# SelennLamson/AntsRL

Measured on AMD Instinct MI355X. Metric: ant-steps/sec (ants x envs x steps/s), 256^2 grid, higher is better.
Workload: dtype f64 ant kinematics / f32 grids

## Files before the change

### antsrl_amd/_lib.py

```python
from __future__ import annotations

import ctypes as C
import os

from .config import AntsCfg, AntsGen, AntsInit

LIB_PATH = os.environ.get("ANTSRL_LIB") or os.path.join(os.path.dirname(os.path.abspath(__file__)), "lib",
                                                        "libantsrl_hip.so")

EXPORTS = ("antsrl_abi_version", "antsrl_cfg_size", "antsrl_last_error", "antsrl_workspace_bytes", "antsrl_create",
           "antsrl_workspace_map",
           "antsrl_destroy", "antsrl_reset", "antsrl_generate", "antsrl_step", "antsrl_observe", "antsrl_update", "antsrl_flush",
           "antsrl_step_update", "antsrl_set_timing_events", "antsrl_set_activation", "antsrl_policy_mlp", "antsrl_read_state", "antsrl_state_bytes",
           "antsrl_set_obs_format", "antsrl_query", "antsrl_bench_copy", "antsrl_set_inloop_policy", "antsrl_set_obs_row_stride", "antsrl_set_perceive_path", "antsrl_mem_alloc", "antsrl_mem_free",
           "antsrl_mem_trim", "antsrl_mem_stats", "antsrl_update_phase",
           "antsrl_perceptive_field", "antsrl_memnet_packed_bytes", "antsrl_memnet_pack", "antsrl_policy_memory",
           "antsrl_memtrain_sizes", "antsrl_memtrain_init", "antsrl_memtrain_unpack", "antsrl_memtrain_copy",
           "antsrl_memtrain_grad", "antsrl_memtrain_apply", "antsrl_memnet_packed_bytes_ex", "antsrl_memnet_pack_ex",
           "antsrl_policy_memory_ex", "antsrl_agent_select", "antsrl_replay_record_pre", "antsrl_replay_record_post",
           "antsrl_policy_memory_tiles", "antsrl_agent_plan", "antsrl_agent_select_actions",
           "antsrl_replay_record_pre_plain", "antsrl_replay_record_post_plain", "antsrl_lintrain_sizes",
           "antsrl_lintrain_grad", "antsrl_lintrain_apply", "antsrl_lintrain_step", "antsrl_exptrain_sizes",
           "antsrl_exptrain_grad", "antsrl_exptrain_apply", "antsrl_exptrain_step", "antsrl_rework_collapsed_bytes",
           "antsrl_rework_collapse", "antsrl_policy_rework", "antsrl_reworktrain_sizes", "antsrl_reworktrain_grad",
           "antsrl_reworktrain_apply", "antsrl_reworktrain_step", "antsrl_policy_rework_select", "antsrl_monitor_sizes",
           "antsrl_monitor_init", "antsrl_monitor_step", "antsrl_monitor_end_episode", "antsrl_recorder_sizes",
           "antsrl_recorder_begin", "antsrl_recorder_frame", "antsrl_render_sizes", "antsrl_render_frames")

_lib = None


class AntsMemNetShape(C.Structure):
    _fields_ = [(n, C.c_int32) for n in ("n_features", "agent_dim", "mem_size", "h1", "h2", "h3", "n_rot", "n_ph")]


class AntsReworkShape(C.Structure):
    _fields_ = [(n, C.c_int32) for n in ("n_features", "agent_dim", "g1", "g2", "g3", "r1", "r2", "r3", "p1", "n_rot", "n_ph")]


class AntsRecordSpec(C.Structure):
    _fields_ = [(n, C.c_int32) for n in ("n_envs", "n_ants", "env_id_base", "n_features", "agent_dim", "mem_size", "n_rot",
                                         "obs_format", "obs_pitch", "reserved")] + [
        (n, C.c_int64) for n in ("K", "head", "max_len")] + [(n, C.c_uint64) for n in ("seed", "step")]


class AntsRenderOpts(C.Structure):
    _fields_ = [(n, C.c_int32) for n in ("zoom", "view_mask", "ant_radius", "layer_only")] + [
        ("phero_max_val", C.c_double), ("phero_colors", (C.c_uint8 * 3) * 4)]


class AntsWsArray(C.Structure):
    _fields_ = [("name", C.c_char * 24), ("block", C.c_int32), ("_pad", C.c_int32), ("offset", C.c_uint64), ("bytes", C.c_uint64)]


class AntsrlError(RuntimeError):
    pass


def load() -> C.CDLL:
    global _lib
    if _lib is not None:
        return _lib
    if not os.path.exists(LIB_PATH):
        raise AntsrlError(
            "libantsrl_hip.so is missing (%s): build it with `python -m antsrl_amd.build` "
            "(hipcc, gfx950).  There is no CPU fallback." % LIB_PATH)
    import torch
    lib = C.CDLL(LIB_PATH)
    vp, i32 = C.c_void_p, C.c_int
    lib.antsrl_abi_version.restype = i32
    lib.antsrl_last_error.restype = C.c_char_p
    lib.antsrl_workspace_bytes.argtypes = [C.POINTER(AntsCfg), C.POINTER(C.c_size_t)]
    lib.antsrl_create.argtypes = [C.POINTER(AntsCfg), vp, C.c_size_t, C.POINTER(vp)]
    lib.antsrl_workspace_bytes2.argtypes = [C.POINTER(AntsCfg), C.POINTER(C.c_size_t), C.POINTER(C.c_size_t)]
    lib.antsrl_create2.argtypes = [C.POINTER(AntsCfg), vp, C.c_size_t, vp, C.c_size_t, C.POINTER(vp)]
    lib.antsrl_workspace_map.argtypes = [C.POINTER(AntsCfg), i32, C.POINTER(AntsWsArray), C.c_int32, C.POINTER(C.c_int32)]
    lib.antsrl_destroy.argtypes = [vp]
    lib.antsrl_destroy.restype = None
    lib.antsrl_reset.argtypes = [vp, C.POINTER(AntsInit), vp]
    lib.antsrl_generate.argtypes = [vp, C.POINTER(AntsGen), C.c_uint64, vp]
    lib.antsrl_step.argtypes = [vp, vp, vp, vp, vp, vp, vp, vp]
    lib.antsrl_observe.argtypes = [vp, vp, vp, vp, vp]
    lib.antsrl_update.argtypes = [vp, vp, vp]
    lib.antsrl_flush.argtypes = [vp, vp]
    lib.antsrl_update_phase.argtypes = [vp, i32, vp, vp]
    lib.antsrl_perceptive_field.argtypes = [vp, vp, vp]
    lib.antsrl_step_update.argtypes = [vp, vp, vp, vp, vp, vp, vp, vp, vp]
    lib.antsrl_set_timing_events.argtypes = [vp, C.POINTER(vp)]
    lib.antsrl_set_activation.argtypes = [vp, vp, C.c_double, vp]
    lib.antsrl_policy_mlp.argtypes = [vp, vp, vp, C.c_int64, C.c_int32, vp, vp, vp, vp, vp, vp, vp, vp, vp, vp]
    lib.antsrl_read_state.argtypes = [vp, i32, vp, vp]
    lib.antsrl_state_bytes.argtypes = [vp, i32, C.POINTER(C.c_size_t)]
    lib.antsrl_query.argtypes = [vp, i32, C.POINTER(C.c_longlong)]
    lib.antsrl_set_inloop_policy.argtypes = [vp, i32] + [vp] * 9
    lib.antsrl_bench_copy.argtypes = [vp, vp, C.c_size_t, vp]
    lib.antsrl_set_obs_row_stride.argtypes = [vp, i32]
    lib.antsrl_set_perceive_path.argtypes = [vp, i32]
    lib.antsrl_mem_alloc.argtypes = [C.c_size_t, i32, C.POINTER(vp)]
    lib.antsrl_mem_free.argtypes = [vp]
    lib.antsrl_mem_trim.argtypes = []
    lib.antsrl_mem_stats.argtypes = [C.POINTER(C.c_size_t)] * 4
    lib.antsrl_memnet_packed_bytes.argtypes = [C.POINTER(AntsMemNetShape), C.POINTER(C.c_size_t)]
    lib.antsrl_memnet_pack.argtypes = [C.POINTER(AntsMemNetShape), C.POINTER(vp), vp, vp]
    lib.antsrl_policy_memory.argtypes = [C.POINTER(AntsMemNetShape), vp, vp, i32, vp, vp, C.c_int64, vp, vp, vp, vp, vp]
    lib.antsrl_memnet_packed_bytes_ex.argtypes = [C.POINTER(AntsMemNetShape), i32, C.POINTER(C.c_size_t)]
    lib.antsrl_memnet_pack_ex.argtypes = [C.POINTER(AntsMemNetShape), i32, C.POINTER(vp), vp, vp]
    lib.antsrl_policy_memory_ex.argtypes = [C.POINTER(AntsMemNetShape), i32, vp, vp, i32, vp, vp, C.c_int64, vp, vp, vp,
                                            vp, vp]
    lib.antsrl_policy_memory_tiles.argtypes = [C.POINTER(AntsMemNetShape), i32, vp, vp, i32, vp, vp, C.c_int64, vp, vp, vp,
                                               vp, vp, vp, vp]
    sz = C.POINTER(C.c_size_t)
    lib.antsrl_memtrain_sizes.argtypes = [C.POINTER(AntsMemNetShape), C.c_int64, sz, sz, sz, sz]
    lib.antsrl_memtrain_init.argtypes = [C.POINTER(AntsMemNetShape), C.POINTER(vp), vp, vp]
    lib.antsrl_memtrain_unpack.argtypes = [C.POINTER(AntsMemNetShape), vp, C.POINTER(vp), vp]
    lib.antsrl_memtrain_copy.argtypes = [C.POINTER(AntsMemNetShape), vp, vp, vp]
    lib.antsrl_memtrain_grad.argtypes = [C.POINTER(AntsMemNetShape), vp, vp, vp, vp, vp, vp, vp, vp, vp, vp, C.c_int64,
                                         C.c_float, vp, vp, vp, vp]
    lib.antsrl_memtrain_apply.argtypes = [C.POINTER(AntsMemNetShape), vp, vp, C.c_int64, C.c_double, C.c_double,
                                          C.c_double, C.c_double, vp]
    lib.antsrl_agent_select.argtypes = [C.c_uint64, C.c_uint64, i32, i32, i32, C.c_double, i32, i32, i32, vp, vp, vp, vp,
                                        vp, vp]
    lib.antsrl_agent_plan.argtypes = [C.c_uint64, C.c_uint64, i32, i32, i32, C.c_double, vp, vp, vp]
    lib.antsrl_replay_record_pre.argtypes = [C.POINTER(AntsRecordSpec)] + [vp] * 9
    lib.antsrl_replay_record_post.argtypes = [C.POINTER(AntsRecordSpec)] + [vp] * 10
    lib.antsrl_agent_select_actions.argtypes = [C.c_uint64, C.c_uint64, i32, i32, i32, C.c_double, i32, i32, vp, vp, vp, vp]
    lib.antsrl_replay_record_pre_plain.argtypes = [C.POINTER(AntsRecordSpec)] + [vp] * 8
    lib.antsrl_replay_record_post_plain.argtypes = [C.POINTER(AntsRecordSpec)] + [vp] * 9
    lib.antsrl_lintrain_sizes.argtypes = [i32, C.c_int64, sz, sz, C.POINTER(C.c_int32)]
    lib.antsrl_lintrain_grad.argtypes = [i32] + [vp] * 11 + [C.c_int64, vp, C.c_int64, C.c_float, vp, vp, vp, vp]
    lib.antsrl_lintrain_apply.argtypes = [vp, vp, vp, vp, C.c_int64, C.c_double, C.c_double, C.c_double, C.c_double, vp]
    lib.antsrl_lintrain_step.argtypes = [i32] + [vp] * 13 + [C.c_int64, vp, C.c_int64, C.c_float, C.c_int64, C.c_double,
                                                             C.c_double, C.c_double, C.c_double, vp, vp, vp, vp]
    lib.antsrl_exptrain_sizes.argtypes = [i32, C.c_int64, sz, sz, C.POINTER(C.c_int32)]
    lib.antsrl_exptrain_grad.argtypes = [i32] + [vp] * 9 + [C.c_int64, vp, C.c_int64, C.c_float, vp, vp, vp, vp]
    lib.antsrl_exptrain_apply.argtypes = [i32, vp, vp, vp, vp, C.c_int64, C.c_double, C.c_double, C.c_double, C.c_double, vp]
    lib.antsrl_exptrain_step.argtypes = [i32] + [vp] * 11 + [C.c_int64, vp, C.c_int64, C.c_float, C.c_int64, C.c_double,
                                                             C.c_double, C.c_double, C.c_double, vp, vp, vp, vp]
    lib.antsrl_rework_collapsed_bytes.argtypes = [C.POINTER(AntsReworkShape), sz]
    lib.antsrl_rework_collapse.argtypes = [C.POINTER(AntsReworkShape), C.POINTER(vp), vp, vp]
    lib.antsrl_policy_rework.argtypes = [C.POINTER(AntsReworkShape), vp, vp, i32, vp, C.c_int64, vp, vp, vp, vp]
    rs = C.POINTER(AntsReworkShape)
    lib.antsrl_policy_rework_select.argtypes = [rs, vp, vp, i32, vp, C.c_uint64, C.c_uint64, i32, i32, i32, C.c_double, vp, vp,
                                                vp, vp, vp]
    lib.antsrl_reworktrain_sizes.argtypes = [rs, C.c_int64, sz, sz, C.POINTER(C.c_int32)]
    lib.antsrl_reworktrain_grad.argtypes = [rs] + [vp] * 9 + [C.c_int64, vp, C.c_int64, C.c_float, vp, vp, vp, vp]
    lib.antsrl_reworktrain_apply.argtypes = [rs, vp, vp, vp, vp, C.c_int64, C.c_double, C.c_double, C.c_double, C.c_double, vp]
    lib.antsrl_reworktrain_step.argtypes = [rs] + [vp] * 11 + [C.c_int64, vp, C.c_int64, C.c_float, C.c_int64, C.c_double,
                                                               C.c_double, C.c_double, C.c_double, vp, vp, vp, vp]
    lib.antsrl_monitor_sizes.argtypes = [i32, i32, i32, i32, sz]
    lib.antsrl_monitor_init.argtypes = [vp, i32, i32, i32, i32, vp]
    lib.antsrl_monitor_step.argtypes = [vp, i32, i32, i32, i32, vp, vp, C.c_double, i32, i32, vp]
    lib.antsrl_monitor_end_episode.argtypes = [vp, i32, i32, i32, i32, i32, i32, vp]
    lib.antsrl_recorder_sizes.argtypes = [vp, i32, i32, i32, sz, sz, sz]
    lib.antsrl_recorder_begin.argtypes = [vp, vp, C.POINTER(C.c_int32), i32, i32, i32, vp]
    lib.antsrl_recorder_frame.argtypes = [vp, vp, C.POINTER(C.c_int32), i32, i32, i32, i32, vp]
    lib.antsrl_render_sizes.argtypes = [vp, i32, C.POINTER(AntsRenderOpts), sz, sz]
    lib.antsrl_render_frames.argtypes = [vp, vp, i32, i32, i32, i32, i32, C.POINTER(AntsRenderOpts), vp, vp, vp]
    for name in EXPORTS:
        getattr(lib, name)
    lib.antsrl_cfg_size.restype = C.c_size_t
    from .config import ABI_VERSION
    if lib.antsrl_abi_version() != ABI_VERSION:
        raise AntsrlError("ABI version mismatch: library %d, binding %d" % (lib.antsrl_abi_version(), ABI_VERSION))
    if lib.antsrl_cfg_size() != C.sizeof(AntsCfg):
        raise AntsrlError("AntsCfg layout mismatch: library %d bytes, binding %d" % (
            lib.antsrl_cfg_size(), C.sizeof(AntsCfg)))
    _lib = lib
    return lib


def hip_runtime() -> C.CDLL:
    load()
    for line in open("/proc/self/maps"):
        path = line.split()[-1]
        if "libamdhip64" in path:
            return C.CDLL(path)
    raise AntsrlError("no libamdhip64 mapped in this process")


def check(rc: int, what: str = "antsrl") -> None:
    if rc != 0:
        msg = load().antsrl_last_error().decode("utf-8", "replace")
        raise AntsrlError("%s failed (%d): %s" % (what, rc, msg))


def ptr(t):
    return None if t is None else C.c_void_p(t.data_ptr())


def stream(device):
    import torch
    return C.c_void_p(torch.cuda.current_stream(device).cuda_stream)


class HipEvents:

    def __init__(self, n):
        self.hip = hip_runtime()
        self.ev = []
        for _ in range(n):
            e = C.c_void_p()
            rc = self.hip.hipEventCreate(C.byref(e))
            assert rc == 0, "hipEventCreate failed: %d" % rc
            self.ev.append(e)

    def elapsed_ms(self, a, b):
        ms = C.c_float()
        rc = self.hip.hipEventElapsedTime(C.byref(ms), self.ev[a], self.ev[b])
        assert rc == 0, "hipEventElapsedTime failed: %d" % rc
        return ms.value

    def destroy(self):
        for e in self.ev:
            self.hip.hipEventDestroy(e)
```

### antsrl_amd/batched.py

```python
from __future__ import annotations

import ctypes as C
from typing import Dict, Optional

import numpy as np
import torch

from . import _lib
from . import config as cfgmod
from . import vmm
from .config import AntsCfg, AntsInit

_STATE_DTYPES = {
    cfgmod.S_ANTS_XYT: torch.float64, cfgmod.S_PREV_XY: torch.float64, cfgmod.S_HOLDING: torch.float32,
    cfgmod.S_MANDIBLES: torch.uint8, cfgmod.S_ACTIVATION: torch.float32, cfgmod.S_PHERO: torch.float32,
    cfgmod.S_FOOD: torch.float32, cfgmod.S_EXPLORED: torch.uint8, cfgmod.S_ANTHILL_FOOD: torch.float64,
    cfgmod.S_ROCK_CENTERS: torch.float64, cfgmod.S_TIMESTEP: torch.int32, cfgmod.S_REWARD_STATE: torch.uint8,
    cfgmod.S_WALLS: torch.uint8, cfgmod.S_ANTHILL_AREA: torch.uint8, cfgmod.S_SEED: torch.float32,
    cfgmod.S_ANTHILL_XYR: torch.int32, cfgmod.S_ROCK_RW: torch.float64,
    cfgmod.S_PHERO_C0: torch.float32, cfgmod.S_PHERO_C1: torch.float32, cfgmod.S_PHERO_C2: torch.float32,
    cfgmod.S_PHERO_C3: torch.float32,
}


import contextlib

_NULL_CTX = contextlib.nullcontext()
_RAW_STREAM = getattr(torch._C, "_cuda_getCurrentRawStream", None)


def _ptr(t: Optional[torch.Tensor]):
    return None if t is None else C.c_void_p(t.data_ptr())


def placement_levels_seen(times) -> bool:
    ok = [t for t in times if t < 1.25 * min(times)]
    return max(ok) >= 1.06 * min(ok)


class BatchedAntsEnv:
    def __init__(self, cfg: AntsCfg, device: Optional[torch.device] = None, obs_dtype: torch.dtype = torch.float32,
                 obs_row_stride=None, pieced_memory: bool = True, split_workspace: bool = True):
        if obs_dtype not in (torch.float32, torch.bfloat16):
            raise ValueError("obs_dtype must be torch.float32 or torch.bfloat16")
        if not torch.cuda.is_available():
            raise _lib.AntsrlError("BatchedAntsEnv needs an MI355X (torch.cuda.is_available() is False); "
                                   "there is no CPU fallback")
        self.lib = _lib.load()
        self.cfg = cfg.copy()
        self.device = torch.device(device if device is not None else "cuda:%d" % torch.cuda.current_device())
        self._dev_index = self.device.index if self.device.index is not None else torch.cuda.current_device()
        need = C.c_size_t()
        _lib.check(self.lib.antsrl_workspace_bytes(C.byref(self.cfg), C.byref(need)), "workspace_bytes")
        self.workspace_bytes = need.value
        nst, nrec = C.c_size_t(), C.c_size_t()
        _lib.check(self.lib.antsrl_workspace_bytes2(C.byref(self.cfg), C.byref(nst), C.byref(nrec)), "workspace_bytes2")
        self.state_bytes, self.record_bytes = nst.value, nrec.value
        self._split = bool(split_workspace)
        if not self._split:
            self.state_bytes, self.record_bytes = 0, self.workspace_bytes
        with torch.cuda.device(self.device):
            big = (lambda n: vmm.empty_u8(n, self.device)) if pieced_memory else (lambda n: torch.empty(n, dtype=torch.uint8, device=self.device))
            self._pieced = bool(pieced_memory)
            self._h = None
            self._state = None
            self._make_handle(torch.empty(self.record_bytes + 256, dtype=torch.uint8, device=self.device))
            E, N, P, K = cfg.n_envs, cfg.n_ants, cfg.pside, cfg.n_channels
            esz = 4 if obs_dtype == torch.float32 else 2
            row = P * P * K
            if obs_row_stride not in (None, "line"):
                raise ValueError("obs_row_stride must be None or 'line'")
            pitch = row if obs_row_stride is None else (row * esz + 127) // 128 * 128 // esz
            sizes = [("agent_state", E * N * 2 * 4), ("reward", E * N * 4), ("done", E), ("obs", E * N * pitch * esz)]
            offs, total = {}, 0
            for name, nbytes in sizes:
                offs[name] = total
                total += (nbytes + 255) // 256 * 256
            self._out_sizes, self._out_offs, self._out_total, self._small_bytes = sizes, offs, total, offs["obs"]
            self._obs_dtype, self._obs_pitch_row = obs_dtype, (pitch, row)
            if obs_dtype == torch.bfloat16:
                _lib.check(self.lib.antsrl_set_obs_format(self._h, 1), "set_obs_format")
            if pitch != row:
                _lib.check(self.lib.antsrl_set_obs_row_stride(self._h, pitch), "set_obs_row_stride")
            self.obs_row_pitch = pitch
            self._bind_outputs(big(total + 256).zero_())
        self._keep = None
        self._loaded = None
        self._host_out = None
        self._host_act = None
        self._act_event = None

    def __del__(self):
        h = getattr(self, "_h", None)
        if h:
            self.lib.antsrl_destroy(h)
            self._h = None

    def _bind_outputs(self, flat: torch.Tensor) -> None:
        c = self.cfg
        E, N, P, K = c.n_envs, c.n_ants, c.pside, c.n_channels
        sizes, offs, total = self._out_sizes, self._out_offs, self._out_total
        pitch, row = self._obs_pitch_row
        base = (-flat.data_ptr()) % 256
        self._out_flat = flat[base:base + total]

        def piece(name, nbytes, dtype, shape):
            return self._out_flat[offs[name]:offs[name] + nbytes].view(dtype).view(shape)
        if pitch == row:
            self.obs = piece("obs", sizes[3][1], self._obs_dtype, (E, N, P, P, K))
            self.obs_padded = None
        else:
            self.obs_padded = piece("obs", sizes[3][1], self._obs_dtype, (E, N, pitch))
            self.obs = self.obs_padded[..., :row].unflatten(-1, (P, P, K))
        self.agent_state = piece("agent_state", sizes[0][1], torch.float32, (E, N, 2))
        self.reward = piece("reward", sizes[1][1], torch.float32, (E, N))
        self.done = piece("done", sizes[2][1], torch.uint8, (E,))
        self._host_out = None

    def _make_handle(self, ws: torch.Tensor, state: Optional[torch.Tensor] = None) -> None:
        if getattr(self, "_h", None):
            self.lib.antsrl_destroy(self._h)
            self._h = None
        if ws.numel() < self.record_bytes + (-ws.data_ptr()) % 256:
            raise _lib.AntsrlError("record block too small: %d bytes for %d" % (ws.numel(), self.record_bytes))
        self._ws_ptr = ws.data_ptr() + (-ws.data_ptr()) % 256
        self._h = C.c_void_p()
        if not self._split:
            self._ws, self._state = ws, None
            _lib.check(self.lib.antsrl_create(C.byref(self.cfg), C.c_void_p(self._ws_ptr), self.workspace_bytes, C.byref(self._h)), "create")
        else:
            if state is None:
                state = self._state if self._state is not None else torch.empty(self.state_bytes + 256, dtype=torch.uint8, device=self.device)
            if state.numel() < self.state_bytes + (-state.data_ptr()) % 256:
                raise _lib.AntsrlError("state block too small: %d bytes for %d" % (state.numel(), self.state_bytes))
            self._ws, self._state = ws, state
            self._state_ptr = state.data_ptr() + (-state.data_ptr()) % 256
            _lib.check(self.lib.antsrl_create2(C.byref(self.cfg), C.c_void_p(self._state_ptr), self.state_bytes,
                                               C.c_void_p(self._ws_ptr), self.record_bytes, C.byref(self._h)), "create2")
        if getattr(self, "_obs_dtype", torch.float32) == torch.bfloat16:
            _lib.check(self.lib.antsrl_set_obs_format(self._h, 1), "set_obs_format")
        pitch, row = getattr(self, "_obs_pitch_row", (0, 0))
        if pitch != row:
            _lib.check(self.lib.antsrl_set_obs_row_stride(self._h, pitch), "set_obs_row_stride")

    def tune_placement(self, age: int = 150, steps: int = 30, verbose: bool = False, extra_outputs: int = 4,
                       walk_spacers: int = 3, spacer_gib: float = 24.0, force_walk: bool = False, state_stage: bool = True):
        if self._out_total < vmm.SMALL_BYTES:
            return None
        if self._loaded:
            raise _lib.AntsrlError("tune_placement() must run right after construction: this handle has already been %s" % self._loaded)
        c = self.cfg
        E, N = c.n_envs, c.n_ants
        dev = self.device

        def torch_u8(n):
            return torch.empty(n, dtype=torch.uint8, device=dev)
        with torch.cuda.device(dev):
            g = torch.Generator(device=dev)
            g.manual_seed(7)
            rot = torch.randint(-1, 2, (4, E, N), generator=g, device=dev, dtype=torch.int8)
            ph = torch.randint(0, 3, (4, E, N), generator=g, device=dev, dtype=torch.int8) if c.n_phero == 2 else [None] * 4
            e0, e1 = torch.cuda.Event(enable_timing=True), torch.cuda.Event(enable_timing=True)

            def scratch_episode():
                self.generate(cfgmod.make_gen(), episode_seed=0x7A11)
                for t in range(age):
                    self.step_update(rot[t % 4], ph[t % 4], None)

            NEV, PSTEPS, PSTEPS_STATE = cfgmod.TIMING_EVENTS, 8, 24
            evs = _lib.HipEvents(NEV * PSTEPS_STATE)
            prc_times = []
            upd_times = []

            def measure(psteps=PSTEPS):
                for t in range(4):
                    self.step_update(rot[t % 4], ph[t % 4], None)
                e0.record()
                for t in range(steps):
                    self.step_update(rot[t % 4], ph[t % 4], None)
                e1.record()
                for t in range(psteps):
                    self.set_timing_events([evs.ev[NEV * t + i].value for i in range(NEV)])
                    self.step_update(rot[t % 4], ph[t % 4], None)
                torch.cuda.current_stream(dev).synchronize()
                prc_times.append(float(np.mean([evs.elapsed_ms(NEV * t + 2, NEV * t + 3) for t in range(psteps)])))
                upd_times.append(float(np.mean([evs.elapsed_ms(NEV * t + 1, NEV * t + 2) for t in range(psteps)])))
                return e0.elapsed_time(e1) / steps
            own_ws, own_out, own_state = self._ws, self._out_flat, self._state
            n_ws, n_out, n_state = self.record_bytes + 256, self._out_total + 256, self.state_bytes + 256
            pairs, times = [], []
            for ws_kind in ("own", "other"):
                if ws_kind == "other":
                    self._make_handle(vmm.empty_u8(n_ws, dev))
                scratch_episode()
                for out_kind in ("own", "other"):
                    if out_kind == "other":
                        self._bind_outputs((torch_u8(n_out) if self._pieced else vmm.empty_u8(n_out, dev)).zero_())
                    elif ws_kind == "other":
                        self._bind_outputs(own_out)
                    pairs.append((self._ws, self._out_flat))
                    times.append(measure())
            labels = ["ws torch / out %s" % ("pieced" if self._pieced else "torch"),
                      "ws torch / out %s" % ("torch" if self._pieced else "pieced"),
                      "ws pieced / out %s" % ("pieced" if self._pieced else "torch"),
                      "ws pieced / out %s" % ("torch" if self._pieced else "pieced")]
            if extra_outputs > 0 and self._pieced:
                self._make_handle(own_ws)
                scratch_episode()
                for k in range(int(extra_outputs)):
                    self._bind_outputs(vmm.empty_u8(n_out, dev).zero_())
                    pairs.append((self._ws, self._out_flat))
                    times.append(measure())
                    labels.append("ws torch / out pieced (draw %d)" % (k + 2))
            spacers = []
            walked = 0
            both_levels = placement_levels_seen
            while self._pieced and walked < int(walk_spacers) and (force_walk or not both_levels(prc_times)):
                free_b = torch.cuda.mem_get_info(dev)[0]
                want = int(min(spacer_gib * 2 ** 30, free_b / 5))
                if want < (4 << 30):
                    break
                try:
                    spacers.append(torch_u8(want))
                    spacers.append(vmm.empty_u8(want, dev))
                except (RuntimeError, _lib.AntsrlError):
                    break
                walked += 1
                depth = sum(x.numel() for x in spacers) / 2 ** 30
                if self._ws.data_ptr() != own_ws.data_ptr():
                    self._make_handle(own_ws)
                scratch_episode()
                for kind, mk in (("pieced", lambda: vmm.empty_u8(n_out, dev)), ("torch", lambda: torch_u8(n_out))):
                    self._bind_outputs(mk().zero_())
                    pairs.append((self._ws, self._out_flat))
                    times.append(measure())
                    labels.append("ws torch / out %s (walk %d: +%.0f GiB)" % (kind, walked, depth))
                self._make_handle(torch_u8(n_ws))
                scratch_episode()
                self._bind_outputs(own_out)
                pairs.append((self._ws, self._out_flat))
                times.append(measure())
                labels.append("ws torch (walk %d: +%.0f GiB) / out %s" % (walked, depth, "pieced" if self._pieced else "torch"))
            best = min(range(len(times)), key=prc_times.__getitem__)
            if verbose:
                print("tune_placement: ms/step per (workspace, outputs) pair %s -> %d" % (["%.4f" % t for t in times], best))
            ws, out = pairs[best]
            n_stage1 = len(times)
            state_cands = [("state torch (default)", own_state)]
            if state_stage and self._split:
                try:
                    state_cands.append(("state pieced", vmm.pieced_u8(n_state, dev)))
                except _lib.AntsrlError:
                    pass
                seen = {ws.data_ptr()}
                for (w2, _o), lab in zip(pairs, labels):
                    if w2.data_ptr() not in seen and w2.numel() >= n_state and len(state_cands) < 4:
                        seen.add(w2.data_ptr())
                        state_cands.append(("state in spare record block (%s)" % lab.split(" / ")[0], w2[:n_state]))
            for lab, st in state_cands if len(state_cands) > 1 else []:
                self._make_handle(ws, st)
                self._bind_outputs(out)
                scratch_episode()
                times.append(measure(PSTEPS_STATE))
            evs.destroy()
            s_upd, s_prc = upd_times[n_stage1:], prc_times[n_stage1:]
            times, prc_times, upd_times = times[:n_stage1], prc_times[:n_stage1], upd_times[:n_stage1]
            s_best = 0
            if s_upd:
                def fast(k, by):
                    return s_upd[k] <= (1.0 - by) * s_upd[0] and s_upd[k] + s_prc[k] < s_upd[0] + s_prc[0]
                own = [k for k in range(1, len(s_upd)) if state_cands[k][0] == "state pieced" and fast(k, 0.03)]
                corners = [k for k in range(1, len(s_upd)) if state_cands[k][0] != "state pieced" and fast(k, 0.05)]
                if own or corners:
                    s_best = min(own or corners, key=s_upd.__getitem__)
            state = state_cands[s_best][1]
            state_labels = [lab for lab, _ in state_cands]
            del pairs, spacers, state_cands
            if ws.data_ptr() != self._ws.data_ptr() or (state is not None and state.data_ptr() != self._state.data_ptr()):
                self._make_handle(ws, state)
            self._bind_outputs(out)
            if walked:
                vmm.trim()
            torch.cuda.empty_cache()
            self._out_flat.zero_()
            del own_ws, own_out, own_state, ws, out, state
        self.placement_trials = dict(ms_per_step=[round(t, 5) for t in times], observation_kernel_ms=[round(t, 5) for t in prc_times],
                                     chosen=best, pairs=labels, both_levels_seen=bool(both_levels(prc_times)), walk_steps=walked,
                                     state_stage=dict(candidates=state_labels, update_move_kernel_ms=[round(t, 5) for t in s_upd],
                                                      observation_kernel_ms=[round(t, 5) for t in s_prc], chosen=s_best))
        self._loaded = None
        return times

    @property
    def _obs_buf(self):
        return self.obs if self.obs_padded is None else self.obs_padded

    def _stream(self):
        if _RAW_STREAM is not None:
            return C.c_void_p(_RAW_STREAM(self._dev_index))
        return C.c_void_p(torch.cuda.current_stream(self.device).cuda_stream)

    def _on_device(self):
        return _NULL_CTX if torch.cuda.current_device() == self._dev_index else torch.cuda.device(self.device)

    def _dev(self, a, dtype, shape=None):
        if a is None:
            return None
        t = torch.as_tensor(np.ascontiguousarray(a) if isinstance(a, np.ndarray) else a)
        t = t.to(device=self.device, dtype=dtype).contiguous()
        if shape is not None:
            assert tuple(t.shape) == tuple(shape), "expected shape %s, got %s" % (shape, tuple(t.shape))
        return t

    def reset(self, init: Dict[str, object]) -> None:
        c = self.cfg
        E, N, W, H, Cn, R = c.n_envs, c.n_ants, c.w, c.h, c.n_phero, c.n_rocks
        t = dict(
            ants_xyt=self._dev(init["ants_xyt"], torch.float64, (E, N, 3)),
            seed=self._dev(init["seed"], torch.float64, (E, N)),
            walls=self._dev(init["walls"], torch.uint8, (E, W, H)),
            food=self._dev(init["food"], torch.float32, (E, W, H)),
            anthill_xyr=self._dev(init["anthill_xyr"], torch.int32, (E, 3)),
            rocks=self._dev(init.get("rocks"), torch.float64, (E, R, 4)) if R > 0 else None,
            phero=self._dev(init.get("phero"), torch.float32, (E, Cn, W, H)),
        )
        ai = AntsInit(*[None if t[k] is None else t[k].data_ptr()
                        for k in ("ants_xyt", "seed", "walls", "food", "anthill_xyr", "rocks", "phero")])
        with torch.cuda.device(self.device):
            _lib.check(self.lib.antsrl_reset(self._h, C.byref(ai), self._stream()), "reset")
        self._loaded = "reset"
        self._keep = t

    def generate(self, gen=None, episode_seed: int = 0, walls=None) -> None:
        g = gen if gen is not None else cfgmod.make_gen()
        if walls is not None:
            c = self.cfg
            self._gen_walls = self._dev(np.asarray(walls).astype(np.uint8) if not torch.is_tensor(walls) else walls,
                                        torch.uint8, (c.n_envs, c.w, c.h))
            g.walls_input = self._gen_walls.data_ptr()
        with torch.cuda.device(self.device):
            _lib.check(self.lib.antsrl_generate(self._h, C.byref(g), int(episode_seed), self._stream()), "generate")
        self._loaded = "given an episode (generate)"

    def _actions(self, rotation, phero):
        c = self.cfg
        if isinstance(rotation, np.ndarray) and isinstance(phero, np.ndarray):
            n = c.n_envs * c.n_ants
            if self._host_act is None:
                self._host_act = torch.empty((2, c.n_envs, c.n_ants), dtype=torch.int8, pin_memory=True)
                self._dev_act = torch.empty((2, c.n_envs, c.n_ants), dtype=torch.int8, device=self.device)
                self._act_event = torch.cuda.Event()
            else:
                self._act_event.synchronize()
            assert rotation.size == n and phero.size == n, "expected %d actions per array" % n
            h = self._host_act.numpy()
            h[0] = self._integral(rotation, "rotation").reshape(c.n_envs, c.n_ants)
            h[1] = self._integral(phero, "pheromone").reshape(c.n_envs, c.n_ants)
            with torch.cuda.device(self.device):
                self._dev_act.copy_(self._host_act, non_blocking=True)
                self._act_event.record()
            return self._dev_act[0], self._dev_act[1]
        rot = self._dev(self._integral(rotation, "rotation"), torch.int8, (c.n_envs, c.n_ants))
        ph = self._dev(self._integral(phero, "pheromone"), torch.int8, (c.n_envs, c.n_ants))
        return rot, ph

    validate_actions = True

    def _integral(self, a, what):
        if a is None:
            return None
        if torch.is_tensor(a):
            if a.dtype == torch.int8 or a.numel() == 0:
                return a
            if self.validate_actions:
                fl = a.is_floating_point()
                frac = (a != a.round()).any() if fl else torch.zeros((), dtype=torch.bool, device=a.device)
                lo, hi, bad = torch.stack([a.min().to(torch.float64), a.max().to(torch.float64), frac.to(torch.float64)]).tolist()
                if bad:
                    raise ValueError("%s actions must be whole numbers (the kernels take them as int8)" % what)
                if lo < -128 or hi > 127:
                    raise ValueError("%s actions out of the int8 range" % what)
            return a.to(torch.int8) if a.is_floating_point() else a
        arr = np.asarray(a)
        if arr.dtype.kind == "f":
            if not np.array_equal(arr, np.rint(arr)):
                raise ValueError("%s actions must be whole numbers (the kernels take them as int8)" % what)
            arr = arr.astype(np.int64)
        if arr.size and (arr.min() < -128 or arr.max() > 127):
            raise ValueError("%s actions out of the int8 range" % what)
        return arr

    def outputs_to_host(self, want_obs: bool = True):
        if self.obs.dtype != torch.float32 and want_obs:
            raise _lib.AntsrlError("outputs_to_host: bfloat16 observations have no numpy dtype; use the device tensors")
        base, o = self._out_flat.data_ptr(), self._out_offs
        if any(t.data_ptr() != base + o[k] for k, t in (("obs", self._obs_buf), ("agent_state", self.agent_state),
                                                         ("reward", self.reward), ("done", self.done))):
            return (self.obs.cpu().numpy() if want_obs else None, self.agent_state.cpu().numpy(),
                    self.reward.cpu().numpy(), self.done.cpu().numpy())
        if self._host_out is None:
            self._host_out = torch.empty((self._out_flat.numel(),), dtype=torch.uint8, pin_memory=True)
        n = self._out_flat.numel() if want_obs else self._small_bytes
        with torch.cuda.device(self.device):
            self._host_out[:n].copy_(self._out_flat[:n], non_blocking=True)
            torch.cuda.current_stream(self.device).synchronize()
        hb, o = self._host_out.numpy(), self._out_offs

        def piece(name, t):
            nb = t.numel() * t.element_size()
            return hb[o[name]:o[name] + nb].view(np.float32 if t.dtype == torch.float32 else np.uint8).reshape(tuple(t.shape)).copy()
        obs_h = None
        if want_obs:
            obs_h = piece("obs", self._obs_buf)
            if self.obs_padded is not None:
                c = self.cfg
                obs_h = np.ascontiguousarray(obs_h[..., :c.pside * c.pside * c.n_channels]).reshape(tuple(self.obs.shape))
        return (obs_h, piece("agent_state", self.agent_state),
                piece("reward", self.reward), piece("done", self.done))

    def step(self, rotation, phero, want_obs: bool = True):
        rot, ph = self._actions(rotation, phero)
        with self._on_device():
            _lib.check(self.lib.antsrl_step(self._h, _ptr(rot), _ptr(ph), _ptr(self._obs_buf if want_obs else None),
                                            _ptr(self.agent_state), _ptr(self.reward), _ptr(self.done),
                                            self._stream()), "step")
        return self.obs, self.agent_state, self.reward, self.done

    def observe(self, want_obs: bool = True):
        with self._on_device():
            _lib.check(self.lib.antsrl_observe(self._h, _ptr(self._obs_buf if want_obs else None),
                                               _ptr(self.agent_state), _ptr(self.reward), self._stream()),
                       "observe")
        return self.obs, self.agent_state, self.reward

    def update(self, wall_jitter=None) -> None:
        c = self.cfg
        j = self._dev(wall_jitter, torch.float64, (c.n_envs, c.n_ants))
        with self._on_device():
            _lib.check(self.lib.antsrl_update(self._h, _ptr(j), self._stream()), "update")

    def update_phase(self, phase: int, wall_jitter=None) -> None:
        c = self.cfg
        j = self._dev(wall_jitter, torch.float64, (c.n_envs, c.n_ants)) if phase == cfgmod.PHASE_WALLS else None
        with self._on_device():
            _lib.check(self.lib.antsrl_update_phase(self._h, int(phase), _ptr(j), self._stream()), "update_phase")

    def flush(self) -> None:
        with self._on_device():
            _lib.check(self.lib.antsrl_flush(self._h, self._stream()), "flush")

    def step_update(self, rotation, phero, wall_jitter=None, want_obs: bool = True):
        c = self.cfg
        rot, ph = self._actions(rotation, phero)
        j = self._dev(wall_jitter, torch.float64, (c.n_envs, c.n_ants))
        with self._on_device():
            _lib.check(self.lib.antsrl_step_update(self._h, _ptr(rot), _ptr(ph), _ptr(j),
                                                   _ptr(self._obs_buf if want_obs else None), _ptr(self.agent_state),
                                                   _ptr(self.reward), _ptr(self.done), self._stream()),
                       "step_update")
        return self.obs, self.agent_state, self.reward, self.done

    def set_timing_events(self, events) -> None:
        if events is None:
            _lib.check(self.lib.antsrl_set_timing_events(self._h, None), "set_timing_events")
        else:
            n = cfgmod.TIMING_EVENTS
            assert len(events) == n, "antsrl_set_timing_events takes %d events" % n
            arr = (C.c_void_p * n)(*[C.c_void_p(int(e)) for e in events])
            _lib.check(self.lib.antsrl_set_timing_events(self._h, arr), "set_timing_events")

    def query(self, what: int) -> int:
        v = C.c_longlong()
        _lib.check(self.lib.antsrl_query(self._h, int(what), C.byref(v)), "query")
        return int(v.value)

    def set_perceive_path(self, path: int) -> None:
        _lib.check(self.lib.antsrl_set_perceive_path(self._h, int(path)), "set_perceive_path")

    def set_activation(self, act, new_deposit_strength: float = 0.0) -> None:
        c = self.cfg
        a = self._dev(act, torch.float32, (c.n_envs, c.n_ants, c.n_phero))
        with torch.cuda.device(self.device):
            _lib.check(self.lib.antsrl_set_activation(self._h, _ptr(a), float(new_deposit_strength),
                                                      self._stream()), "set_activation")
        self._loaded = "given an activation matrix"

    def perceptive_field(self) -> torch.Tensor:
        c = self.cfg
        out = torch.empty((c.n_envs, c.w, c.h), dtype=torch.uint8, device=self.device)
        with self._on_device():
            _lib.check(self.lib.antsrl_perceptive_field(self._h, _ptr(out), self._stream()), "perceptive_field")
        return out.to(torch.bool)

    def read_state(self, which: int) -> torch.Tensor:
        c = self.cfg
        E, N, W, H, Cn, R = c.n_envs, c.n_ants, c.w, c.h, c.n_phero, c.n_rocks
        shapes = {
            cfgmod.S_ANTS_XYT: (E, N, 3), cfgmod.S_PREV_XY: (E, N, 2), cfgmod.S_HOLDING: (E, N),
            cfgmod.S_MANDIBLES: (E, N), cfgmod.S_ACTIVATION: (E, N, Cn), cfgmod.S_PHERO: (E, Cn, W, H),
            cfgmod.S_FOOD: (E, W, H), cfgmod.S_EXPLORED: (E, W, H), cfgmod.S_ANTHILL_FOOD: (E,),
            cfgmod.S_ROCK_CENTERS: (E, R, 2), cfgmod.S_TIMESTEP: (E,), cfgmod.S_REWARD_STATE: (E, N),
            cfgmod.S_WALLS: (E, W, H), cfgmod.S_ANTHILL_AREA: (E, W, H), cfgmod.S_SEED: (E, N),
            cfgmod.S_ANTHILL_XYR: (E, 3), cfgmod.S_ROCK_RW: (E, R, 2),
            cfgmod.S_PHERO_C0: (E, W, H), cfgmod.S_PHERO_C1: (E, W, H), cfgmod.S_PHERO_C2: (E, W, H),
            cfgmod.S_PHERO_C3: (E, W, H),
        }
        if cfgmod.S_PHERO_C0 <= which <= cfgmod.S_PHERO_C3 and which - cfgmod.S_PHERO_C0 >= Cn:
            raise _lib.AntsrlError("pheromone channel %d of %d" % (which - cfgmod.S_PHERO_C0, Cn))
        out = torch.empty(shapes[which], dtype=_STATE_DTYPES[which], device=self.device)
        if out.numel():
            with torch.cuda.device(self.device):
                _lib.check(self.lib.antsrl_read_state(self._h, which, _ptr(out), self._stream()), "read_state")
        return out
```

### antsrl_amd/config.py

```python
from __future__ import annotations

import ctypes as C
import math
from typing import Optional, Sequence

import numpy as np

ABI_VERSION = 5
MAX_CHANNELS = 16
MAX_PSIDE = 15
MAX_PCELLS = MAX_PSIDE * MAX_PSIDE
MAX_FILTER_RADIUS = 3
MAX_FILTER_TAPS = 49
MAX_PHERO = 4

CH_ANTS, CH_PHERO, CH_ANTHILL, CH_WALLS, CH_FOOD, CH_ROCKS = range(6)
REWARD_NONE, REWARD_EXPLORATION, REWARD_FOOD, REWARD_ALL = range(4)
PHERO_AUTO, PHERO_EXPLICIT_SWEEP = 0, 1
ACT_AUTO, ACT_CELL_META, ACT_SINGLE_KERNEL = 0, 1, 2
TIMING_EVENTS = 5
Q_CELL_META, Q_SCALED_UNITS, Q_INTERLEAVED, Q_FILTER_SEPARABLE, Q_PERCEIVE_RUN, Q_TIMESTEP, Q_DEFERRED_UPDATE, Q_PERCEIVE_FAST = range(8)
PERCEIVE_AUTO, PERCEIVE_GENERIC = 0, 1

(S_ANTS_XYT, S_PREV_XY, S_HOLDING, S_MANDIBLES, S_ACTIVATION, S_PHERO, S_FOOD, S_EXPLORED,
 S_ANTHILL_FOOD, S_ROCK_CENTERS, S_TIMESTEP, S_REWARD_STATE, S_WALLS, S_ANTHILL_AREA,
 S_SEED, S_ANTHILL_XYR, S_ROCK_RW, S_PHERO_C0, S_PHERO_C1, S_PHERO_C2, S_PHERO_C3) = range(21)


class AntsCfg(C.Structure):
    _fields_ = [
        ("abi_version", C.c_int32),
        ("n_envs", C.c_int32),
        ("n_ants", C.c_int32),
        ("w", C.c_int32),
        ("h", C.c_int32),
        ("n_phero", C.c_int32),
        ("n_rocks", C.c_int32),
        ("max_time", C.c_int32),
        ("perception_radius", C.c_int32),
        ("n_channels", C.c_int32),
        ("channel_kind", C.c_int32 * MAX_CHANNELS),
        ("channel_arg", C.c_int32 * MAX_CHANNELS),
        ("has_mask", C.c_int32),
        ("mask", C.c_uint8 * MAX_PCELLS),
        ("_pad0", C.c_uint8 * 7),
        ("delta", C.c_double),
        ("fwd_delta", C.c_double),
        ("max_speed", C.c_double),
        ("max_rot_speed", C.c_double),
        ("carry_speed_reduction", C.c_double),
        ("backward_speed_reduction", C.c_double),
        ("max_hold", C.c_double),
        ("has_max_val", C.c_int32),
        ("filter_radius", C.c_int32),
        ("phero_max_val", C.c_double),
        ("deposit_strength", C.c_double),
        ("phero_threshold", C.c_double),
        ("filter", C.c_double * MAX_FILTER_TAPS),
        ("reward_kind", C.c_int32),
        ("phero_mode", C.c_int32),
        ("reward_threshold", C.c_double),
        ("fct_explore", C.c_double),
        ("fct_food", C.c_double),
        ("fct_anthill", C.c_double),
        ("fct_explore_holding", C.c_double),
        ("fct_headinganthill", C.c_double),
        ("rng_seed", C.c_uint64),
        ("act_path", C.c_int32),
        ("env_id_base", C.c_int32),
        ("n_envs_total", C.c_int32),
        ("_pad1", C.c_int32),
    ]

    @property
    def pside(self) -> int:
        return 2 * self.perception_radius + 1

    def copy(self) -> "AntsCfg":
        out = AntsCfg()
        C.memmove(C.byref(out), C.byref(self), C.sizeof(AntsCfg))
        return out

    def obs_shape(self):
        p = self.pside
        return (self.n_envs, self.n_ants, p, p, self.n_channels)


class AntsGen(C.Structure):
    _fields_ = [("wall_density", C.c_double), ("n_food_discs", C.c_int32), ("food_rmin", C.c_int32),
                ("food_rmax", C.c_int32), ("auto_reset", C.c_int32), ("wall_kind", C.c_int32),
                ("perlin_octaves", C.c_int32), ("perlin_scale", C.c_double), ("perlin_persistence", C.c_double),
                ("perlin_lacunarity", C.c_double), ("rng_kind", C.c_int32), ("_pad", C.c_int32),
                ("walls_input", C.c_void_p)]


WALLS_BERNOULLI, WALLS_PERLIN, WALLS_INPUT = 0, 1, 2
PHASE_WALLS, PHASE_ROCKS_PHEROMONE, PHASE_ANTS, PHASE_ANTHILL = 0, 1, 2, 3
RNG_COUNTER, RNG_REFERENCE = 0, 1


def make_gen(wall_density=0.05, n_food_discs=20, food_rmin=5, food_rmax=10, auto_reset=False, walls="bernoulli",
             perlin_scale=22.0, perlin_octaves=2, perlin_persistence=0.5, perlin_lacunarity=2.0, rng="counter",
             walls_input_ptr=None) -> AntsGen:
    kind = {"bernoulli": WALLS_BERNOULLI, "perlin": WALLS_PERLIN, "input": WALLS_INPUT}[walls]
    return AntsGen(wall_density, n_food_discs, food_rmin, food_rmax, 1 if auto_reset else 0, kind,
                   int(perlin_octaves), float(perlin_scale), float(perlin_persistence), float(perlin_lacunarity),
                   {"counter": RNG_COUNTER, "reference": RNG_REFERENCE}[rng], 0, walls_input_ptr)


class AntsInit(C.Structure):
    _fields_ = [
        ("ants_xyt", C.c_void_p),
        ("seed", C.c_void_p),
        ("walls", C.c_void_p),
        ("food", C.c_void_p),
        ("anthill_xyr", C.c_void_p),
        ("rocks", C.c_void_p),
        ("phero", C.c_void_p),
    ]


DEFAULT_MASK = np.array([[0, 0, 1, 1, 1, 0, 0],
                         [0, 1, 1, 1, 1, 1, 0],
                         [1, 1, 1, 1, 1, 1, 1],
                         [1, 1, 1, 1, 1, 1, 1],
                         [1, 1, 1, 1, 1, 1, 1],
                         [0, 1, 1, 1, 1, 1, 0],
                         [0, 0, 1, 1, 1, 0, 0]], dtype=np.uint8)


def diffuse_filter(diffuse_factor: float = 0.0, evap_factor: float = 0.001) -> np.ndarray:
    f = np.ones((3, 3)) * diffuse_factor
    f[1, 1] = 1 - 8 * diffuse_factor
    f *= 1 - evap_factor
    return f


def default_channels(n_phero: int, n_rocks: int):
    kinds = [CH_ANTS] + [CH_PHERO] * n_phero + [CH_ANTHILL, CH_WALLS, CH_FOOD]
    args = [0] + list(range(n_phero)) + [0, 0, 0]
    if n_rocks > 0:
        kinds.append(CH_ROCKS)
        args.append(0)
    return kinds, args


def make_cfg(n_envs: int, n_ants: int, w: int, h: int, *, n_phero: int = 2, n_rocks: int = 0,
             max_time: int = 2000, mask: Optional[np.ndarray] = DEFAULT_MASK,
             perception_radius: Optional[int] = None, fwd_delta: float = 4.0, delta: float = 1.1,
             channels: Optional[Sequence] = None,
             max_speed: float = 1.0, max_rot_speed: float = 40 / 180 * np.pi,
             carry_speed_reduction: float = 0.05, backward_speed_reduction: float = 0.5,
             max_hold: float = 5.0, phero_max_val: Optional[float] = 255.0,
             deposit_strength: float = 1.0, phero_threshold: float = 0.01,
             filt: Optional[np.ndarray] = None, reward_kind: int = REWARD_EXPLORATION,
             reward_threshold: float = 1.0, fct_explore: float = 1.0, fct_food: float = 1.0,
             fct_anthill: float = 5.0, fct_explore_holding: float = 0.0,
             fct_headinganthill: float = 1.0, rng_seed: int = 0x5EED,
             phero_mode: int = PHERO_AUTO, act_path: int = ACT_AUTO, env_id_base: int = 0,
             n_envs_total: int = 0) -> AntsCfg:
    c = AntsCfg()
    c.abi_version = ABI_VERSION
    c.n_envs, c.n_ants, c.w, c.h = n_envs, n_ants, w, h
    c.n_phero, c.n_rocks, c.max_time = n_phero, n_rocks, max_time
    if mask is not None:
        mask = np.asarray(mask)
        assert mask.ndim == 2 and mask.shape[0] == mask.shape[1] and mask.shape[0] % 2 == 1
        r = mask.shape[0] // 2 if perception_radius is None else perception_radius
        assert mask.shape[0] == 2 * r + 1
        c.has_mask = 1
        flat = mask.astype(np.uint8).reshape(-1)
        for i, v in enumerate(flat):
            c.mask[i] = int(v)
    else:
        r = 3 if perception_radius is None else perception_radius
        c.has_mask = 0
    assert 2 * r + 1 <= MAX_PSIDE
    c.perception_radius = r
    if channels is None:
        kinds, args = default_channels(n_phero, n_rocks)
    else:
        kinds = [k if isinstance(k, int) else k[0] for k in channels]
        args = [0 if isinstance(k, int) else k[1] for k in channels]
    assert len(kinds) <= MAX_CHANNELS
    c.n_channels = len(kinds)
    for i, (k, a) in enumerate(zip(kinds, args)):
        c.channel_kind[i] = k
        c.channel_arg[i] = a
    c.delta, c.fwd_delta = delta, fwd_delta
    c.max_speed, c.max_rot_speed = max_speed, max_rot_speed
    c.carry_speed_reduction, c.backward_speed_reduction = carry_speed_reduction, backward_speed_reduction
    c.max_hold = max_hold
    c.has_max_val = 0 if phero_max_val is None else 1
    c.phero_max_val = 0.0 if phero_max_val is None else phero_max_val
    c.deposit_strength = deposit_strength
    c.phero_threshold = phero_threshold
    if filt is None:
        filt = diffuse_filter()
    filt = np.asarray(filt, dtype=np.float64)
    assert filt.ndim == 2 and filt.shape[0] == filt.shape[1] and filt.shape[0] % 2 == 1
    fr = filt.shape[0] // 2
    off = filt.copy()
    off[fr, fr] = 0.0
    if not off.any():
        filt = filt[fr:fr + 1, fr:fr + 1]
        fr = 0
    assert fr <= MAX_FILTER_RADIUS
    c.filter_radius = fr
    for i, v in enumerate(filt.reshape(-1)):
        c.filter[i] = float(v)
    c.reward_kind = reward_kind
    c.reward_threshold = reward_threshold
    c.fct_explore, c.fct_food, c.fct_anthill = fct_explore, fct_food, fct_anthill
    c.fct_explore_holding, c.fct_headinganthill = fct_explore_holding, fct_headinganthill
    c.rng_seed = rng_seed
    c.phero_mode = phero_mode
    c.act_path = act_path
    c.env_id_base = env_id_base
    c.n_envs_total = n_envs_total
    return c


def mask_array(cfg: AntsCfg) -> Optional[np.ndarray]:
    if not cfg.has_mask:
        return None
    p = cfg.pside
    return np.array(list(cfg.mask[: p * p]), dtype=bool).reshape(p, p)


__all__ = [n for n in dir() if n.isupper() or n in (
    "AntsCfg", "AntsInit", "AntsGen", "make_gen", "make_cfg", "diffuse_filter", "default_channels", "mask_array")]
_ = math


def uses_scaled_units(cfg: AntsCfg) -> bool:
    return (cfg.phero_mode == PHERO_AUTO and cfg.filter_radius == 0 and 0.5 < cfg.filter[0] <= 1.0
            and cfg.phero_threshold >= 0.0)
```

### antsrl_amd/csrc/antsrl_capi.hip

```cpp
#include <hip/hip_runtime.h>
#include <stdarg.h>
#include <stdio.h>
#include <math.h>
#include <stdlib.h>
#include <string.h>
#include <new>

#include "antsrl_device.h"
#include "antsrl_fail.h"
#include "antsrl_recorder.h"
#include "antsrl_render.h"

hipError_t antsrl_launch_act(const KP &p, const int8_t *rot, const int8_t *ph, int cur, float *obs,
                             float *agent_state, float *reward, uint8_t *done, int flags, hipStream_t st);
bool antsrl_act_fits(const KP &p);
bool antsrl_act_needs_hbm_maps(const KP &p);
hipError_t antsrl_launch_sweep(const KP &p, int cur, hipStream_t st);
hipError_t antsrl_launch_update(const KP &p, const double *jitter, int out_buf, hipStream_t st, int phases = 15);
hipError_t antsrl_launch_collect_full(const KP &p, hipStream_t st);
hipError_t antsrl_launch_reset(const KP &p, const AntsInit *in, hipStream_t st);
hipError_t antsrl_launch_set_activation(const KP &p, const float *act, hipStream_t st);
hipError_t antsrl_launch_read_state(const KP &p, int which, int cur, void *dst, hipStream_t st);
hipError_t antsrl_launch_perceptive_field(const KP &p, uint8_t *dst, hipStream_t st);
hipError_t antsrl_launch_generate(const KP &p, const AntsGen &g, uint64_t seed, hipStream_t st);
hipError_t antsrl_launch_phero_wall_clear(const KP &p, hipStream_t st, int buf = 0);
hipError_t antsrl_launch_phero_renorm(const KP &p, hipStream_t st);
bool antsrl_meta_supported(const KP &p);
hipError_t antsrl_launch_move(const KP &p, const int8_t *rot, const int8_t *ph, uint8_t *done, int do_step, uint32_t seq,
                              hipStream_t st);
hipError_t antsrl_launch_perceive(const KP &p, int cur, float *obs, float *agent_state, float *reward, int flags,
                                  uint32_t seq, hipStream_t st, const PolArgs *pol, uint32_t obs_pitch, bool generic);
bool antsrl_perceive_fast(const KP &p);
bool antsrl_inloop_policy_supported(const KP &p);
hipError_t antsrl_launch_policy_pack(unsigned char *pack, const float *w1, const float *b1, const float *w2, const float *b2,
                                     const float *w3, const float *b3, int F, hipStream_t st);
hipError_t antsrl_launch_meta_rebase(const KP &p, hipStream_t st);
bool antsrl_update_move_supported(const KP &p);
hipError_t antsrl_launch_update_move(const KP &p, int out_buf, double g_dep, double inv_g_dep, const int8_t *rot,
                                     const int8_t *ph, uint8_t *done, uint32_t seq, hipStream_t st, bool with_frames);
int antsrl_perceive_run(const KP &p);
hipError_t antsrl_launch_copy16(void *dst, const void *src, size_t bytes, hipStream_t st);

struct AntsHandle {
    AntsCfg cfg;
    KP p;
    int cur;
    int steps_since_update;
    bool need_full_collect;
    bool is_reset;
    bool episode_over;
    size_t ws_bytes[2];
    AntsGen gen;
    bool has_gen;
    uint64_t episode_seed;
    int host_timestep;
    long long sweeps;
    bool obs_bf16;
    uint32_t obs_pitch;
    bool prc_generic;
    bool need_wall_clear;
    hipEvent_t ev[ANTSRL_TIMING_EVENTS];
    bool ev_armed;
    uint32_t obs_seq;
    PolArgs pol;
    bool pend_update;
    KP pend_p;
    int pend_out_buf;
    int phase_next;
};

static thread_local char g_err[512] = "";

int fail(int code, const char *fmt, ...)
{
    va_list ap;
    va_start(ap, fmt);
    vsnprintf(g_err, sizeof(g_err), fmt, ap);
    va_end(ap);
    return code;
}

int hip_fail(hipError_t e, const char *what)
{
    return fail(ANTSRL_E_DEVICE, "%s: %s", what, hipGetErrorString(e));
}

extern "C" int antsrl_abi_version(void) { return ANTSRL_ABI_VERSION; }
extern "C" size_t antsrl_cfg_size(void) { return sizeof(AntsCfg); }
extern "C" const char *antsrl_last_error(void) { return g_err; }

static void fill_kp(const AntsCfg *c, KP *p);

static int validate(const AntsCfg *c)
{
    if (!c) return fail(ANTSRL_E_INVALID, "cfg is NULL");
    if (c->abi_version != ANTSRL_ABI_VERSION)
        return fail(ANTSRL_E_INVALID, "AntsCfg.abi_version %d != library %d", c->abi_version, ANTSRL_ABI_VERSION);
    if (c->n_envs < 1 || c->n_ants < 1 || c->w < 1 || c->h < 1)
        return fail(ANTSRL_E_INVALID, "n_envs, n_ants, w, h must be >= 1");
    if ((long long)c->w * c->h > (1ll << 30)) return fail(ANTSRL_E_INVALID, "grid too large");
    if (c->n_envs > 65535)
        return fail(ANTSRL_E_INVALID, "n_envs must be <= 65535 per handle (shard larger batches over handles / GPUs)");
    if (c->n_phero < 1 || c->n_phero > ANTSRL_MAX_PHERO)
        return fail(ANTSRL_E_INVALID, "n_phero must be in 1..%d", ANTSRL_MAX_PHERO);
    if (c->n_rocks < 0 || c->n_rocks > 32) return fail(ANTSRL_E_INVALID, "n_rocks must be in 0..32");
    if (c->perception_radius < 0 || 2 * c->perception_radius + 1 > ANTSRL_MAX_PSIDE)
        return fail(ANTSRL_E_INVALID, "perception side must be <= %d", ANTSRL_MAX_PSIDE);
    if (c->n_channels < 1 || c->n_channels > ANTSRL_MAX_CHANNELS)
        return fail(ANTSRL_E_INVALID, "n_channels must be in 1..%d", ANTSRL_MAX_CHANNELS);
    for (int k = 0; k < c->n_channels; ++k) {
        const int kind = c->channel_kind[k];
        if (kind < ANTSRL_CH_ANTS || kind > ANTSRL_CH_ROCKS) return fail(ANTSRL_E_INVALID, "bad channel kind");
        if (kind == ANTSRL_CH_PHERO && (c->channel_arg[k] < 0 || c->channel_arg[k] >= c->n_phero))
            return fail(ANTSRL_E_INVALID, "pheromone channel index out of range");
        if (kind == ANTSRL_CH_PHERO && !c->has_max_val)
            return fail(ANTSRL_E_INVALID, "a perceived pheromone needs max_val (RL_api.py:125 divides by it)");
        if (kind == ANTSRL_CH_ROCKS && c->n_rocks == 0)
            return fail(ANTSRL_E_INVALID, "rocks perceived but n_rocks == 0");
    }
    if (c->filter_radius < 0 || c->filter_radius > ANTSRL_MAX_FILTER_RADIUS)
        return fail(ANTSRL_E_INVALID, "filter_radius must be in 0..%d", ANTSRL_MAX_FILTER_RADIUS);
    if (c->reward_kind < ANTSRL_REWARD_NONE || c->reward_kind > ANTSRL_REWARD_ALL)
        return fail(ANTSRL_E_INVALID, "bad reward_kind");
    if (c->has_max_val && !(c->phero_max_val > 0)) return fail(ANTSRL_E_INVALID, "phero_max_val must be > 0");
    if (c->act_path < ANTSRL_ACT_AUTO || c->act_path > ANTSRL_ACT_SINGLE_KERNEL) return fail(ANTSRL_E_INVALID, "bad act_path");
    if (c->env_id_base < 0 || (long long)c->env_id_base + c->n_envs > 0x7fffffffll)
        return fail(ANTSRL_E_INVALID, "env_id_base must be >= 0 and env_id_base + n_envs must fit 31 bits");
    if (c->n_envs_total != 0 && (long long)c->n_envs_total < (long long)c->env_id_base + c->n_envs)
        return fail(ANTSRL_E_INVALID, "n_envs_total %d < env_id_base + n_envs = %lld (0 = that sum)", c->n_envs_total,
                    (long long)c->env_id_base + c->n_envs);
    if (c->act_path == ANTSRL_ACT_CELL_META) {
        KP kp;
        fill_kp(c, &kp);
        if (!kp.meta)
            return fail(ANTSRL_E_UNSUPPORTED, "ANTSRL_ACT_CELL_META needs 2 pheromone channels, the generator's channel order "
                                              "([Ants, Phero0, Phero1, Anthill, Walls, Food(, Rocks)]), a perception of 128..368 values "
                                              "per ant over at most 64 cells, and at most 4096 ants per env");
    }
    return ANTSRL_OK;
}

static bool use_scaled(const AntsCfg *c)
{
    return c->phero_mode == ANTSRL_PHERO_AUTO && c->filter_radius == 0 && c->filter[0] > 0.5 &&
           c->filter[0] <= 1.0 && c->phero_threshold >= 0.0;
}

static bool use_interleaved(const AntsCfg *c)
{
    return use_scaled(c) && c->n_phero == 2;
}

static void carve(const AntsCfg *c, DState *s, unsigned char *base, unsigned char *rec_base, bool split, size_t bytes[2],
                  AntsWsArray *map = nullptr, int32_t cap = 0, int32_t *count = nullptr)
{
    const size_t E = c->n_envs, N = c->n_ants, G = (size_t)c->w * c->h, Cn = c->n_phero, R = c->n_rocks;
    const size_t words = (G + 31) / 32;
    size_t off[2] = {0, 0};
    int32_t n_arrays = 0;
    auto take_from = [&](int block, const char *name, size_t nbytes) -> unsigned char * {
        unsigned char *b = block ? rec_base : base;
        size_t &o = off[split ? block : 0];
        unsigned char *ptr = b ? b + o : nullptr;
        if (map && n_arrays < cap) {
            AntsWsArray &a = map[n_arrays];
            memset(&a, 0, sizeof(a));
            strncpy(a.name, name, sizeof(a.name) - 1);
            a.block = split ? block : 0; a.offset = o; a.bytes = nbytes;
        }
        ++n_arrays;
        o = (o + nbytes + 255) / 256 * 256;
        return ptr;
    };
    auto take = [&](const char *name, size_t nbytes) { return take_from(0, name, nbytes); };
    auto take_rec = [&](const char *name, size_t nbytes) { return take_from(1, name, nbytes); };
    KP kp;
    fill_kp(c, &kp);
    DState d;
    d.x = (double *)take("x", 8 * E * N); d.y = (double *)take("y", 8 * E * N); d.theta = (double *)take("theta", 8 * E * N);
    d.prev_x = (double *)take("prev_x", 8 * E * N); d.prev_y = (double *)take("prev_y", 8 * E * N);
    d.prev_dist = (double *)take("prev_dist", 8 * E * N);
    d.holding = (float *)take("holding", 4 * E * N); d.seed = (float *)take("seed", 4 * E * N);
    d.prev_holding = (float *)take("prev_holding", 4 * E * N);
    d.activation = (float *)take("activation", 4 * E * N * Cn);
    d.mandibles = (uint8_t *)take("mandibles", E * N); d.reward_state = (uint8_t *)take("reward_state", E * N);
    d.dirty_cell = (int32_t *)take("dirty_cell", 4 * E * N);
    d.walldep_cell = (int32_t *)take("walldep_cell", 4 * E * N);
    if (use_interleaved(c)) {
        d.phero[0] = d.phero[1] = (float *)take_rec("records", 16 * E * G);
        d.food = d.phero[0] ? d.phero[0] + 2 : nullptr;
    } else {
        d.phero[0] = (float *)take_rec("phero0", 4 * E * G * Cn);
        d.phero[1] = use_scaled(c) ? d.phero[0] : (float *)take_rec("phero1", 4 * E * G * Cn);
        d.food = (float *)take_rec("food", 4 * E * G * (size_t)kp.fs);
    }
    d.walls_bits = (uint32_t *)take("walls_bits", 4 * E * words); d.area_bits = (uint32_t *)take("area_bits", 4 * E * words);
    d.explored_bits = (uint32_t *)take("explored_bits", 4 * E * words);
    d.big_pres = d.big_old = nullptr;
    if (!kp.meta && antsrl_act_needs_hbm_maps(kp)) {
        d.big_pres = (uint32_t *)take("big_pres", 4 * E * words);
        d.big_old = (uint32_t *)take("big_old", 4 * E * words);
    }
    d.primed_cur = kp.meta ? (uint8_t *)take("primed_cur", E) : nullptr;
    d.frames = kp.meta ? (AntFrame *)take("frames", sizeof(AntFrame) * E * N) : nullptr;
    d.anthill_xyr = (int32_t *)take("anthill_xyr", 4 * E * 3);
    d.anthill_food = (double *)take("anthill_food", 8 * E);
    d.rock_cx = (double *)take("rock_cx", 8 * E * (R ? R : 1)); d.rock_cy = (double *)take("rock_cy", 8 * E * (R ? R : 1));
    d.rock_r = (double *)take("rock_r", 8 * E * (R ? R : 1)); d.rock_w = (double *)take("rock_w", 8 * E * (R ? R : 1));
    d.timestep = (int32_t *)take("timestep", 4 * E);
    d.reward_primed = (uint8_t *)take("reward_primed", E);
    d.gen_discs = (int32_t *)take("gen_discs", 4 * E * ANTSRL_MAX_FOOD_DISCS * 3);
    d.gen_perlin = (int32_t *)take("gen_perlin", 4 * E * 2);
    d.pol_pack = (unsigned char *)take("pol_pack", ANTSRL_POL_PACK_BYTES);
    if (s) *s = d;
    if (count) *count = n_arrays;
    bytes[0] = off[0]; bytes[1] = off[1];
}

static void fill_kp(const AntsCfg *c, KP *p)
{
    memset(p, 0, sizeof(*p));
    p->E = c->n_envs; p->N = c->n_ants; p->W = c->w; p->H = c->h; p->C = c->n_phero; p->R = c->n_rocks;
    p->K = c->n_channels; p->r = c->perception_radius; p->P = 2 * p->r + 1; p->PP = p->P * p->P;
    p->words = (int)(((size_t)c->w * c->h + 31) / 32);
    int ht = 64;
    while (ht < 2 * c->n_ants) ht <<= 1;
    p->HT = ht;
    p->has_mask = c->has_mask; p->has_max_val = c->has_max_val; p->reward_kind = c->reward_kind;
    p->max_time = c->max_time; p->filter_radius = c->filter_radius;
    p->explore_on = c->reward_kind == ANTSRL_REWARD_EXPLORATION ||
                    (c->reward_kind == ANTSRL_REWARD_ALL &&
                     (c->fct_explore != 0.0 || c->fct_explore_holding != 0.0));
    for (int k = 0; k < ANTSRL_MAX_CHANNELS; ++k) {
        p->ch_kind[k] = c->channel_kind[k];
        p->ch_arg[k] = c->channel_arg[k];
    }
    p->mand_first = p->mand_last = 0;
    for (int k = 0; k < c->n_channels; ++k) {
        const int op = c->channel_kind[k] == ANTSRL_CH_FOOD ? 1 : c->channel_kind[k] == ANTSRL_CH_ANTHILL ? 2 : 0;
        if (op && op != p->mand_last) {
            p->mand_first = p->mand_last;
            p->mand_last = op;
        }
    }
    memcpy(p->mask, c->mask, ANTSRL_MAX_PCELLS);
    p->delta = c->delta; p->fwd_delta = c->fwd_delta; p->max_speed = c->max_speed;
    p->max_rot_speed = c->max_rot_speed; p->carry = c->carry_speed_reduction;
    p->backward = c->backward_speed_reduction; p->max_hold = c->max_hold;
    p->max_val = c->phero_max_val; p->deposit_strength = c->deposit_strength;
    p->threshold = c->phero_threshold; p->reward_threshold = c->reward_threshold;
    p->fct_explore = c->fct_explore; p->fct_food = c->fct_food; p->fct_anthill = c->fct_anthill;
    p->fct_explore_holding = c->fct_explore_holding; p->fct_heading = c->fct_headinganthill;
    memcpy(p->filter, c->filter, sizeof(p->filter));
    {
        const int S = 2 * c->filter_radius + 1;
        for (int a = 0; a < S; ++a)
            for (int b = 0; b < S; ++b) {
                const double f = c->filter[a * S + b];
                const float hi = (float)f;
                p->ftap[(b * S + a) * 2 + 0] = hi;
                p->ftap[(b * S + a) * 2 + 1] = (float)(f - (double)hi);
            }
    }
    {
        const int S = 2 * c->filter_radius + 1;
        p->filter_sep = 0;
        if (S > 1) {
            int i0 = 0, j0 = 0;
            double big = 0.0;
            for (int a = 0; a < S; ++a)
                for (int b = 0; b < S; ++b)
                    if (fabs(c->filter[a * S + b]) > big) { big = fabs(c->filter[a * S + b]); i0 = a; j0 = b; }
            bool sep = big > 0.0;
            double u[2 * ANTSRL_MAX_FILTER_RADIUS + 1], v[2 * ANTSRL_MAX_FILTER_RADIUS + 1];
            for (int a = 0; a < S && sep; ++a) u[a] = c->filter[a * S + j0];
            for (int b = 0; b < S && sep; ++b) v[b] = c->filter[i0 * S + b] / c->filter[i0 * S + j0];
            for (int a = 0; a < S && sep; ++a)
                for (int b = 0; b < S; ++b)
                    if (fabs(u[a] * v[b] - c->filter[a * S + b]) > 1e-15 * big) sep = false;
            if (sep) {
                p->filter_sep = 1;
                for (int k = 0; k < S; ++k) {
                    const float uh = (float)u[k], vh = (float)v[k];
                    p->fsep_u[2 * k] = uh; p->fsep_u[2 * k + 1] = (float)(u[k] - (double)uh);
                    p->fsep_v[2 * k] = vh; p->fsep_v[2 * k + 1] = (float)(v[k] - (double)vh);
                }
            }
        }
    }
    p->rng_seed = c->rng_seed;
    p->env_id_base = (uint32_t)c->env_id_base;
    p->scaled = use_scaled(c) ? 1 : 0;
    p->ps = use_interleaved(c) ? 4 : c->n_phero;
    p->fs = use_interleaved(c) ? 4 : 1;
    p->g_now = p->g_dep = p->inv_g_dep = 1.0;
    p->meta = antsrl_meta_supported(*p) && c->act_path != ANTSRL_ACT_SINGLE_KERNEL ? 1 : 0;
    if (p->meta && p->fs == 1) p->fs = 2;
    p->tiled = (p->meta && p->ps == 4 && p->fs == 4 && (c->w & 1) == 0 && (c->h & 3) == 0) ? 1 : 0;
    p->ftile = (p->meta && p->fs == 2 && (c->w & 3) == 0 && (c->h & 3) == 0) ? 1 : 0;
}

static void set_decay(AntsHandle *h)
{
    if (!h->p.scaled) return;
    const double f0 = h->cfg.filter[0];
    h->p.g_now = pow(f0, (double)h->sweeps);
    h->p.g_dep = pow(f0, (double)(h->sweeps + 1));
    h->p.inv_g_dep = 1.0 / h->p.g_dep;
}

extern "C" int antsrl_workspace_bytes(const AntsCfg *cfg, size_t *bytes)
{
    int rc = validate(cfg);
    if (rc) return rc;
    if (!bytes) return fail(ANTSRL_E_INVALID, "bytes is NULL");
    size_t b[2];
    carve(cfg, nullptr, nullptr, nullptr, false, b);
    *bytes = b[0];
    return ANTSRL_OK;
}

extern "C" int antsrl_workspace_bytes2(const AntsCfg *cfg, size_t *state_bytes, size_t *record_bytes)
{
    int rc = validate(cfg);
    if (rc) return rc;
    size_t b[2];
    carve(cfg, nullptr, nullptr, nullptr, true, b);
    if (state_bytes) *state_bytes = b[0];
    if (record_bytes) *record_bytes = b[1];
    return ANTSRL_OK;
}

extern "C" int antsrl_workspace_map(const AntsCfg *cfg, int split, AntsWsArray *entries, int32_t cap, int32_t *count)
{
    int rc = validate(cfg);
    if (rc) return rc;
    if (!count) return fail(ANTSRL_E_INVALID, "count is NULL");
    if (cap < 0 || (cap > 0 && !entries)) return fail(ANTSRL_E_INVALID, "entries is NULL or cap < 0");
    size_t b[2];
    carve(cfg, nullptr, nullptr, nullptr, split != 0, b, entries, cap, count);
    return ANTSRL_OK;
}

static int create_handle(const AntsCfg *cfg, void *state_ws, void *record_ws, bool split, const size_t need[2], AntsHandle **out)
{
    AntsHandle *h = new (std::nothrow) AntsHandle();
    if (!h) return fail(ANTSRL_E_NOMEM, "out of host memory");
    h->cfg = *cfg;
    fill_kp(cfg, &h->p);
    size_t b[2];
    carve(cfg, &h->p.s, (unsigned char *)state_ws, (unsigned char *)record_ws, split, b);
    h->cur = 0; h->steps_since_update = 0; h->need_full_collect = true; h->is_reset = false; h->episode_over = false; h->pend_update = false;
    h->phase_next = 0;
    h->pol = PolArgs{};
    h->sweeps = 0; h->need_wall_clear = false;
    h->has_gen = false; h->episode_seed = 0; h->host_timestep = 1; h->obs_bf16 = false; h->obs_pitch = 0;
    h->prc_generic = false;
    h->ws_bytes[0] = need[0]; h->ws_bytes[1] = need[1];
    h->ev_armed = false;
    h->obs_seq = 0;
    if (!h->p.meta && !antsrl_act_fits(h->p)) {
        delete h;
        return fail(ANTSRL_E_UNSUPPORTED,
                    "%d ants with a %dx%d perception need more than 160 KiB of LDS per workgroup "
                    "(per-ant frames, the collision hash and the row staging are kept in LDS)", cfg->n_ants,
                    2 * cfg->perception_radius + 1, 2 * cfg->perception_radius + 1);
    }
    *out = h;
    return ANTSRL_OK;
}

extern "C" int antsrl_create(const AntsCfg *cfg, void *workspace, size_t workspace_bytes, AntsHandle **out)
{
    int rc = validate(cfg);
    if (rc) return rc;
    if (!out) return fail(ANTSRL_E_INVALID, "out is NULL");
    if (!workspace) return fail(ANTSRL_E_INVALID, "workspace is NULL");
    if (((uintptr_t)workspace & 255) != 0) return fail(ANTSRL_E_INVALID, "workspace must be 256-byte aligned");
    size_t need[2];
    carve(cfg, nullptr, nullptr, nullptr, false, need);
    if (workspace_bytes < need[0])
        return fail(ANTSRL_E_NOMEM, "workspace too small: %zu < %zu bytes", workspace_bytes, need[0]);
    return create_handle(cfg, workspace, workspace, false, need, out);
}

extern "C" int antsrl_create2(const AntsCfg *cfg, void *state_ws, size_t state_bytes, void *record_ws, size_t record_bytes,
                              AntsHandle **out)
{
    int rc = validate(cfg);
    if (rc) return rc;
    if (!out) return fail(ANTSRL_E_INVALID, "out is NULL");
    if (!state_ws || !record_ws) return fail(ANTSRL_E_INVALID, "state_ws or record_ws is NULL");
    if ((((uintptr_t)state_ws | (uintptr_t)record_ws) & 255) != 0)
        return fail(ANTSRL_E_INVALID, "state_ws and record_ws must be 256-byte aligned");
    size_t need[2];
    carve(cfg, nullptr, nullptr, nullptr, true, need);
    if (state_bytes < need[0])
        return fail(ANTSRL_E_NOMEM, "state block too small: %zu < %zu bytes", state_bytes, need[0]);
    if (record_bytes < need[1])
        return fail(ANTSRL_E_NOMEM, "record block too small: %zu < %zu bytes", record_bytes, need[1]);
    const uintptr_t s0 = (uintptr_t)state_ws, r0 = (uintptr_t)record_ws;
    if (s0 < r0 + need[1] && r0 < s0 + need[0])
        return fail(ANTSRL_E_INVALID, "the state block and the record block overlap");
    return create_handle(cfg, state_ws, record_ws, true, need, out);
}

extern "C" void antsrl_destroy(AntsHandle *h) { delete h; }

extern "C" int antsrl_reset(AntsHandle *h, const AntsInit *init, void *stream)
{
    if (!h || !init) return fail(ANTSRL_E_INVALID, "NULL handle or init");
    if (!init->ants_xyt || !init->seed || !init->walls || !init->food || !init->anthill_xyr)
        return fail(ANTSRL_E_INVALID, "AntsInit: ants_xyt, seed, walls, food, anthill_xyr are required");
    if (h->p.R > 0 && !init->rocks) return fail(ANTSRL_E_INVALID, "AntsInit.rocks is NULL but n_rocks > 0");
    h->pend_update = false;
    h->phase_next = 0;
    hipError_t e = antsrl_launch_reset(h->p, init, (hipStream_t)stream);
    if (e != hipSuccess) return hip_fail(e, "reset");
    h->p.deposit_strength = h->cfg.deposit_strength;
    h->cur = 0; h->steps_since_update = 0; h->need_full_collect = true; h->is_reset = true; h->episode_over = false;
    h->sweeps = 0; h->need_wall_clear = h->p.scaled && init->phero != nullptr;
    h->host_timestep = 1; h->obs_seq = 0;
    set_decay(h);
    return ANTSRL_OK;
}

static int check_gen_seed(const AntsHandle *h, const AntsGen &g, uint64_t seed)
{
    const uint64_t top = (uint64_t)h->p.env_id_base + (uint64_t)h->p.E;
    const uint64_t lim = 0xFFFFFFFFull / 5u;
    if (g.rng_kind == ANTSRL_RNG_REFERENCE && (top > lim || seed > lim - top))
        return fail(ANTSRL_E_INVALID, "ANTSRL_RNG_REFERENCE: (episode_seed + env_id_base + n_envs) * 5 must stay below 2^32 (np.random.seed)");
    return ANTSRL_OK;
}

static int do_generate(AntsHandle *h, uint64_t seed, hipStream_t st)
{
    int rc = check_gen_seed(h, h->gen, seed);
    if (rc) return rc;
    h->pend_update = false;
    h->phase_next = 0;
    hipError_t e = antsrl_launch_generate(h->p, h->gen, seed, st);
    if (e != hipSuccess) return hip_fail(e, "generate");
    h->p.deposit_strength = h->cfg.deposit_strength;
    h->cur = 0; h->steps_since_update = 0; h->need_full_collect = true; h->is_reset = true; h->episode_over = false;
    h->sweeps = 0; h->need_wall_clear = false; h->host_timestep = 1; h->obs_seq = 0;
    h->episode_seed = seed;
    set_decay(h);
    return ANTSRL_OK;
}

extern "C" int antsrl_generate(AntsHandle *h, const AntsGen *gen, uint64_t episode_seed, void *stream)
{
    if (!h || !gen) return fail(ANTSRL_E_INVALID, "NULL handle or gen");
    if (gen->n_food_discs < 0 || gen->n_food_discs > ANTSRL_MAX_FOOD_DISCS)
        return fail(ANTSRL_E_INVALID, "n_food_discs must be in 0..%d", ANTSRL_MAX_FOOD_DISCS);
    if (gen->food_rmin < 0 || gen->food_rmax < gen->food_rmin) return fail(ANTSRL_E_INVALID, "bad food radii");
    if (gen->wall_kind == ANTSRL_WALLS_BERNOULLI) {
        if (!(gen->wall_density >= 0.0 && gen->wall_density <= 1.0)) return fail(ANTSRL_E_INVALID, "bad wall_density");
    } else if (gen->wall_kind == ANTSRL_WALLS_PERLIN) {
        if (!(gen->wall_density >= -1.0 && gen->wall_density <= 1.0) || gen->perlin_octaves < 1 || gen->perlin_octaves > 8 ||
            !(gen->perlin_scale > 0.0) || !(gen->perlin_persistence > 0.0) || !(gen->perlin_lacunarity > 0.0))
            return fail(ANTSRL_E_INVALID, "bad Perlin wall parameters (density in [-1, 1], 1..8 octaves, positive "
                                          "scale / persistence / lacunarity)");
    } else if (gen->wall_kind == ANTSRL_WALLS_INPUT) {
        if (!gen->walls_input) return fail(ANTSRL_E_INVALID, "ANTSRL_WALLS_INPUT needs AntsGen.walls_input");
    } else {
        return fail(ANTSRL_E_INVALID, "bad wall_kind %d", gen->wall_kind);
    }
    if (gen->rng_kind != ANTSRL_RNG_COUNTER && gen->rng_kind != ANTSRL_RNG_REFERENCE)
        return fail(ANTSRL_E_INVALID, "bad rng_kind %d", gen->rng_kind);
    if (gen->rng_kind == ANTSRL_RNG_REFERENCE) {
        if (gen->wall_kind == ANTSRL_WALLS_BERNOULLI && gen->wall_density != 0.0)
            return fail(ANTSRL_E_UNSUPPORTED, "the reference has no Bernoulli walls generator: with ANTSRL_RNG_REFERENCE use "
                                              "ANTSRL_WALLS_PERLIN, ANTSRL_WALLS_INPUT or wall_density 0");
    }
    int rc = check_gen_seed(h, *gen, episode_seed);
    if (rc) return rc;
    h->gen = *gen;
    h->has_gen = true;
    return do_generate(h, episode_seed, (hipStream_t)stream);
}

static int bf16_unsupported()
{
    return fail(ANTSRL_E_UNSUPPORTED, "bfloat16 observations on the single-kernel path (k_act) need 2 pheromone channels, the "
                                      "generator's channel order ([Ants, Phero0, Phero1, Anthill, Walls, Food(, Rocks)]), a perception of "
                                      "at most 64 cells and a grid whose bit maps fit LDS (up to ~600k cells); the cell-meta path "
                                      "(ANTSRL_Q_CELL_META) has no grid limit");
}

extern "C" int antsrl_set_obs_format(AntsHandle *h, int format)
{
    if (!h) return fail(ANTSRL_E_INVALID, "NULL handle");
    if (format != ANTSRL_OBS_F32 && format != ANTSRL_OBS_BF16) return fail(ANTSRL_E_INVALID, "bad observation format %d", format);
    if ((format == ANTSRL_OBS_BF16) != h->obs_bf16) h->obs_pitch = 0;
    h->obs_bf16 = format == ANTSRL_OBS_BF16;
    if (!h->obs_bf16) h->pol = PolArgs{};
    return ANTSRL_OK;
}

extern "C" int antsrl_set_obs_row_stride(AntsHandle *h, int32_t stride_elems)
{
    if (!h) return fail(ANTSRL_E_INVALID, "NULL handle");
    const int32_t row = h->p.PP * h->p.K, esz = h->obs_bf16 ? 2 : 4;
    if (stride_elems == 0 || stride_elems == row) {
        h->obs_pitch = 0;
        return ANTSRL_OK;
    }
    if (stride_elems < row || ((long long)stride_elems * esz) % 128 != 0 || stride_elems > row + 128 / esz)
        return fail(ANTSRL_E_INVALID, "obs row stride %d: 0 (dense) or the row's %d elements rounded up to whole 128-byte lines (%d)",
                    stride_elems, row, (row * esz + 127) / 128 * 128 / esz);
    if (!h->p.meta) return fail(ANTSRL_E_UNSUPPORTED, "antsrl_set_obs_row_stride needs the cell-meta path (ANTSRL_Q_CELL_META)");
    if (h->pol.pack)
        return fail(ANTSRL_E_UNSUPPORTED, "a padded observation row stride and the in-loop policy exclude each other (the net reads a "
                                          "dense tile image): switch the policy off first (antsrl_set_inloop_policy with w1 == NULL)");
    h->obs_pitch = (uint32_t)stride_elems;
    return ANTSRL_OK;
}

extern "C" int antsrl_set_perceive_path(AntsHandle *h, int path)
{
    if (!h) return fail(ANTSRL_E_INVALID, "NULL handle");
    if (path != ANTSRL_PERCEIVE_AUTO && path != ANTSRL_PERCEIVE_GENERIC) return fail(ANTSRL_E_INVALID, "bad perceive path %d", path);
    h->prc_generic = path == ANTSRL_PERCEIVE_GENERIC;
    return ANTSRL_OK;
}

static int flush_pending(AntsHandle *h, hipStream_t st)
{
    if (!h->pend_update) return ANTSRL_OK;
    h->pend_update = false;
    hipError_t e = antsrl_launch_update(h->pend_p, nullptr, h->pend_out_buf, st);
    if (e != hipSuccess) return hip_fail(e, "deferred update");
    return ANTSRL_OK;
}

static int not_reset(const AntsHandle *h)
{
    if (h->episode_over)
        return fail(ANTSRL_E_INVALID, "the episode is over and its auto-reset was refused (episode seed past np.random.seed's 32 bits): "
                                      "call antsrl_reset or antsrl_generate");
    return fail(ANTSRL_E_INVALID, "antsrl_reset has not been called on this handle");
}

static int mid_update(const AntsHandle *h)
{
    return fail(ANTSRL_E_INVALID, "an Environment.update is in progress (antsrl_update_phase %d of 4 is next): finish it first", h->phase_next);
}

static int meta_observe(AntsHandle *h, const int8_t *rot, const int8_t *ph, float *obs, float *agent_state,
                        float *reward, uint8_t *done, bool stepping, hipStream_t st, bool timed)
{
    hipError_t e;
    if (obs && h->obs_pitch != 0 && h->obs_pitch != (uint32_t)(h->p.PP * h->p.K) && h->pol.pack && h->obs_bf16)
        return fail(ANTSRL_E_UNSUPPORTED, "a padded observation row stride and the in-loop policy exclude each other");
    if (h->obs_seq >= META_NEVER - 2) {
        e = antsrl_launch_meta_rebase(h->p, st);
        if (e != hipSuccess) return hip_fail(e, "explored-stamp rebase");
        h->obs_seq = 0;
    }
    h->obs_seq++;
    bool frames = false;
    if (h->pend_update && stepping) {
        h->pend_update = false;
        frames = h->pol.pack != nullptr;
        e = antsrl_launch_update_move(h->p, h->pend_out_buf, h->pend_p.g_dep, h->pend_p.inv_g_dep, rot, ph, done, h->obs_seq, st, frames);
        if (e != hipSuccess) return hip_fail(e, "update + move");
    } else {
        int rc = flush_pending(h, st);
        if (rc) return rc;
        e = antsrl_launch_move(h->p, rot, ph, done, stepping ? 1 : 0, h->obs_seq, st);
        if (e != hipSuccess) return hip_fail(e, "move");
    }
    if (timed) (void)hipEventRecord(h->ev[2], st);
    e = antsrl_launch_perceive(h->p, h->cur, obs, agent_state, reward,
                               (stepping ? ACT_STEP : 0) | (obs ? ACT_HAS_OBS : 0) | (frames ? ACT_FRAMES : 0) |
                                   ((obs || h->pol.pack) && h->obs_bf16 ? ACT_OBS_BF16 : 0),
                               h->obs_seq, st, &h->pol, h->obs_pitch, h->prc_generic);
    if (e == hipErrorNotSupported)
        return fail(ANTSRL_E_UNSUPPORTED, "a padded observation row stride and the in-loop policy exclude each other (the net reads a dense tile image)");
    if (e != hipSuccess) return hip_fail(e, "perceive");
    return ANTSRL_OK;
}

static int do_step(AntsHandle *h, const int8_t *rot, const int8_t *ph, float *obs, float *agent_state,
                   float *reward, uint8_t *done, hipStream_t st, bool timed = false)
{
    if (ph && h->p.C != 2)
        return fail(ANTSRL_E_INVALID, "pheromone actions need exactly 2 pheromone channels (ants.py:89-96)");
    if (h->steps_since_update > 0) h->need_full_collect = true;
    if (h->p.meta) {
        int rc = meta_observe(h, rot, ph, obs, agent_state, reward, done, true, st, timed);
        if (rc) return rc;
        h->steps_since_update++;
        return ANTSRL_OK;
    }
    if (obs && h->obs_pitch) return fail(ANTSRL_E_UNSUPPORTED, "antsrl_set_obs_row_stride needs the cell-meta path (ANTSRL_Q_CELL_META)");
    if (timed) (void)hipEventRecord(h->ev[2], st);
    hipError_t e = antsrl_launch_act(h->p, rot, ph, h->cur, obs, agent_state, reward, done,
                                     ACT_STEP | (obs ? ACT_HAS_OBS : 0) | (obs && h->obs_bf16 ? ACT_OBS_BF16 : 0), st);
    if (e == hipErrorNotSupported) return bf16_unsupported();
    if (e != hipSuccess) return hip_fail(e, "step");
    h->steps_since_update++;
    return ANTSRL_OK;
}

static int do_update(AntsHandle *h, const double *jitter, hipStream_t st, bool sweep_done, bool may_defer)
{
    hipError_t e;
    int frc = flush_pending(h, st);
    if (frc) return frc;
    if (h->p.scaled) {
        if (h->p.g_dep < 1e-20) {
            e = antsrl_launch_phero_renorm(h->p, st);
            if (e != hipSuccess) return hip_fail(e, "pheromone renorm");
            h->sweeps = 0;
            set_decay(h);
        }
        if (h->need_wall_clear) {
            e = antsrl_launch_phero_wall_clear(h->p, st);
            if (e != hipSuccess) return hip_fail(e, "pheromone wall clear");
            h->need_wall_clear = false;
        }
    } else if (!sweep_done) {
        e = antsrl_launch_sweep(h->p, h->cur, st);
        if (e != hipSuccess) return hip_fail(e, "pheromone sweep");
    }
    if (may_defer && !jitter && !h->need_full_collect && antsrl_update_move_supported(h->p)) {
        h->pend_update = true;
        h->pend_p = h->p;
        h->pend_out_buf = h->p.scaled ? 0 : h->cur ^ 1;
    } else {
        e = antsrl_launch_update(h->p, jitter, h->p.scaled ? 0 : h->cur ^ 1, st);
        if (e != hipSuccess) return hip_fail(e, "update");
    }
    if (h->p.scaled) {
        h->sweeps++;
        set_decay(h);
    }
    if (h->need_full_collect) {
        e = antsrl_launch_collect_full(h->p, st);
        if (e != hipSuccess) return hip_fail(e, "anthill collect");
        h->need_full_collect = false;
    }
    if (!h->p.scaled) h->cur ^= 1;
    h->steps_since_update = 0;
    h->host_timestep++;
    return ANTSRL_OK;
}

extern "C" int antsrl_step(AntsHandle *h, const int8_t *rotation, const int8_t *phero, float *obs,
                           float *agent_state, float *reward, uint8_t *done, void *stream)
{
    if (!h) return fail(ANTSRL_E_INVALID, "NULL handle");
    if (!h->is_reset) return not_reset(h);
    if (h->phase_next) return mid_update(h);
    if (!agent_state || !reward || !done) return fail(ANTSRL_E_INVALID, "agent_state, reward, done are required");
    return do_step(h, rotation, phero, obs, agent_state, reward, done, (hipStream_t)stream);
}

extern "C" int antsrl_observe(AntsHandle *h, float *obs, float *agent_state, float *reward, void *stream)
{
    if (!h) return fail(ANTSRL_E_INVALID, "NULL handle");
    if (!h->is_reset) return not_reset(h);
    if (h->phase_next) return mid_update(h);
    if (h->p.meta)
        return meta_observe(h, nullptr, nullptr, obs, agent_state, reward, nullptr, false, (hipStream_t)stream, false);
    if (obs && h->obs_pitch) return fail(ANTSRL_E_UNSUPPORTED, "antsrl_set_obs_row_stride needs the cell-meta path (ANTSRL_Q_CELL_META)");
    hipError_t e = antsrl_launch_act(h->p, nullptr, nullptr, h->cur, obs, agent_state, reward, nullptr,
                                     obs ? ACT_HAS_OBS | (h->obs_bf16 ? ACT_OBS_BF16 : 0) : 0, (hipStream_t)stream);
    if (e == hipErrorNotSupported) return bf16_unsupported();
    if (e != hipSuccess) return hip_fail(e, "observe");
    return ANTSRL_OK;
}

extern "C" int antsrl_update(AntsHandle *h, const double *wall_jitter, void *stream)
{
    if (!h) return fail(ANTSRL_E_INVALID, "NULL handle");
    if (!h->is_reset) return not_reset(h);
    if (h->phase_next) return mid_update(h);
    return do_update(h, wall_jitter, (hipStream_t)stream, false, true);
}

extern "C" int antsrl_update_phase(AntsHandle *h, int phase, const double *wall_jitter, void *stream)
{
    if (!h) return fail(ANTSRL_E_INVALID, "NULL handle");
    if (!h->is_reset) return not_reset(h);
    if (phase < ANTSRL_PHASE_WALLS || phase > ANTSRL_PHASE_ANTHILL) return fail(ANTSRL_E_INVALID, "bad phase %d", phase);
    if (phase != h->phase_next)
        return fail(ANTSRL_E_INVALID, "antsrl_update_phase: phase %d is next, got %d (WALLS, ROCKS_PHEROMONE, ANTS, ANTHILL in order)", h->phase_next, phase);
    hipStream_t st = (hipStream_t)stream;
    hipError_t e;
    if (phase == ANTSRL_PHASE_WALLS) {
        int frc = flush_pending(h, st);
        if (frc) return frc;
        if (h->p.scaled) {
            if (h->p.g_dep < 1e-20) {
                e = antsrl_launch_phero_renorm(h->p, st);
                if (e != hipSuccess) return hip_fail(e, "pheromone renorm");
                h->sweeps = 0;
                set_decay(h);
            }
            if (h->need_wall_clear) {
                e = antsrl_launch_phero_wall_clear(h->p, st);
                if (e != hipSuccess) return hip_fail(e, "pheromone wall clear");
                h->need_wall_clear = false;
            }
        } else {
            e = antsrl_launch_phero_wall_clear(h->p, st, h->cur);
            if (e != hipSuccess) return hip_fail(e, "pheromone wall clear");
        }
        e = antsrl_launch_update(h->p, wall_jitter, h->p.scaled ? 0 : h->cur, st, 1 );
        if (e != hipSuccess) return hip_fail(e, "update: walls");
    } else if (phase == ANTSRL_PHASE_ROCKS_PHEROMONE) {
        e = antsrl_launch_update(h->p, nullptr, h->p.scaled ? 0 : h->cur, st, 2 );
        if (e != hipSuccess) return hip_fail(e, "update: rocks");
        if (h->p.scaled) {
            h->sweeps++;
            set_decay(h);
        } else {
            e = antsrl_launch_sweep(h->p, h->cur, st);
            if (e != hipSuccess) return hip_fail(e, "pheromone sweep");
            h->cur ^= 1;
        }
    } else if (phase == ANTSRL_PHASE_ANTS) {
        KP kp = h->p;
        if (kp.scaled) {
            kp.g_dep = kp.g_now;
            kp.inv_g_dep = 1.0 / kp.g_dep;
        }
        e = antsrl_launch_update(kp, nullptr, kp.scaled ? 0 : h->cur, st, 4 );
        if (e != hipSuccess) return hip_fail(e, "update: ants");
    } else {
        e = antsrl_launch_update(h->p, nullptr, h->p.scaled ? 0 : h->cur, st, 8 );
        if (e != hipSuccess) return hip_fail(e, "update: anthill");
        if (h->need_full_collect) {
            e = antsrl_launch_collect_full(h->p, st);
            if (e != hipSuccess) return hip_fail(e, "anthill collect");
            h->need_full_collect = false;
        }
        h->steps_since_update = 0;
        h->host_timestep++;
    }
    h->phase_next = (phase + 1) % 4;
    return ANTSRL_OK;
}

extern "C" int antsrl_flush(AntsHandle *h, void *stream)
{
    if (!h) return fail(ANTSRL_E_INVALID, "NULL handle");
    return flush_pending(h, (hipStream_t)stream);
}

extern "C" int antsrl_step_update(AntsHandle *h, const int8_t *rotation, const int8_t *phero,
                                  const double *wall_jitter, float *obs, float *agent_state, float *reward,
                                  uint8_t *done, void *stream)
{
    if (!h) return fail(ANTSRL_E_INVALID, "NULL handle");
    if (!h->is_reset) return not_reset(h);
    if (h->phase_next) return mid_update(h);
    if (!agent_state || !reward || !done) return fail(ANTSRL_E_INVALID, "agent_state, reward, done are required");
    hipStream_t st = (hipStream_t)stream;
    const bool timed = h->ev_armed;
    h->ev_armed = false;
    if (timed) (void)hipEventRecord(h->ev[0], st);
    const bool sweep_late = !h->p.scaled && h->pend_update;
    if (!h->p.scaled && !sweep_late) {
        hipError_t e = antsrl_launch_sweep(h->p, h->cur, st);
        if (e != hipSuccess) return hip_fail(e, "pheromone sweep");
    }
    if (timed) (void)hipEventRecord(h->ev[1], st);
    int rc = do_step(h, rotation, phero, obs, agent_state, reward, done, st, timed);
    if (rc) return rc;
    if (timed) (void)hipEventRecord(h->ev[3], st);
    if (sweep_late) {
        hipError_t e = antsrl_launch_sweep(h->p, h->cur, st);
        if (e != hipSuccess) return hip_fail(e, "pheromone sweep");
    }
    const bool was_done = h->host_timestep == h->cfg.max_time;
    const bool regen = was_done && h->has_gen && h->gen.auto_reset;
    rc = do_update(h, wall_jitter, st, true, !regen);
    if (timed) (void)hipEventRecord(h->ev[4], st);
    if (rc == ANTSRL_OK && regen) {
        const uint64_t total = h->cfg.n_envs_total ? (uint64_t)h->cfg.n_envs_total : (uint64_t)h->p.env_id_base + (uint64_t)h->p.E;
        rc = do_generate(h, h->episode_seed + (h->gen.rng_kind == ANTSRL_RNG_REFERENCE ? total : 1u), st);
        if (rc != ANTSRL_OK) {
            h->is_reset = false;
            h->episode_over = true;
        }
    }
    return rc;
}

extern "C" int antsrl_query(const AntsHandle *h, int what, long long *value)
{
    if (!h || !value) return fail(ANTSRL_E_INVALID, "NULL handle or value");
    switch (what) {
    case ANTSRL_Q_CELL_META: *value = h->p.meta; break;
    case ANTSRL_Q_SCALED_UNITS: *value = h->p.scaled; break;
    case ANTSRL_Q_INTERLEAVED: *value = h->p.ps == 4 && h->p.fs == 4; break;
    case ANTSRL_Q_FILTER_SEPARABLE: *value = h->p.filter_sep; break;
    case ANTSRL_Q_PERCEIVE_RUN: *value = h->p.meta ? antsrl_perceive_run(h->p) : 0; break;
    case ANTSRL_Q_TIMESTEP: *value = h->host_timestep; break;
    case ANTSRL_Q_DEFERRED_UPDATE: *value = antsrl_update_move_supported(h->p); break;
    case ANTSRL_Q_PERCEIVE_FAST: *value = h->p.meta && !h->prc_generic && antsrl_perceive_fast(h->p); break;
    default: return fail(ANTSRL_E_INVALID, "bad query selector %d", what);
    }
    return ANTSRL_OK;
}

extern "C" int antsrl_bench_copy(void *dst, const void *src, size_t bytes, void *stream)
{
    if (!dst || !src || (bytes & 15) || ((uintptr_t)dst & 15) || ((uintptr_t)src & 15))
        return fail(ANTSRL_E_INVALID, "bench_copy: 16-byte aligned pointers and a multiple of 16 bytes");
    hipError_t e = antsrl_launch_copy16(dst, src, bytes, (hipStream_t)stream);
    if (e != hipSuccess) return hip_fail(e, "bench_copy");
    return ANTSRL_OK;
}

extern "C" int antsrl_set_timing_events(AntsHandle *h, void *const *events)
{
    if (!h) return fail(ANTSRL_E_INVALID, "NULL handle");
    h->ev_armed = events != nullptr;
    if (events)
        for (int i = 0; i < ANTSRL_TIMING_EVENTS; ++i) h->ev[i] = (hipEvent_t)events[i];
    return ANTSRL_OK;
}

extern "C" int antsrl_set_activation(AntsHandle *h, const float *act, double new_deposit_strength, void *stream)
{
    if (!h || !act) return fail(ANTSRL_E_INVALID, "NULL handle or act");
    if (!h->is_reset) return not_reset(h);
    if (h->phase_next) return mid_update(h);
    int frc = flush_pending(h, (hipStream_t)stream);
    if (frc) return frc;
    hipError_t e = antsrl_launch_set_activation(h->p, act, (hipStream_t)stream);
    if (e != hipSuccess) return hip_fail(e, "set_activation");
    if (new_deposit_strength > 0) h->p.deposit_strength = new_deposit_strength;
    return ANTSRL_OK;
}

hipError_t antsrl_launch_policy(const float *obs, const float *agent_state, const float *w1, const float *b1,
                                const float *w2, const float *b2, const float *w3, const float *b3, int8_t *rot,
                                int8_t *ph, float *logits, int M, int F, hipStream_t st, bool obs_bf16);

extern "C" int antsrl_policy_mlp(AntsHandle *h, const float *obs, const float *agent_state, int64_t n_ants,
                                 int32_t n_features, const float *w1, const float *b1, const float *w2,
                                 const float *b2, const float *w3, const float *b3, int8_t *rotation,
                                 int8_t *pheromone, float *logits, void *stream)
{
    if (!obs || !agent_state || !w1 || !b1 || !w2 || !b2 || !rotation)
        return fail(ANTSRL_E_INVALID, "policy_mlp: obs, agent_state, w1, b1, w2, b2, rotation are required");
    if ((w3 == nullptr) != (b3 == nullptr) || (pheromone && !w3))
        return fail(ANTSRL_E_INVALID, "policy_mlp: w3/b3 go together and are needed for a pheromone output");
    if (n_ants < 1 || n_ants > 0x7fffffff || n_features < 1 || n_features + 2 > 1024)
        return fail(ANTSRL_E_INVALID, "policy_mlp: n_ants >= 1 and 1 <= n_features <= 1022");
    hipError_t e = antsrl_launch_policy(obs, agent_state, w1, b1, w2, b2, w3, b3, rotation, pheromone, logits,
                                        (int)n_ants, n_features, (hipStream_t)stream, h && h->obs_bf16);
    if (e != hipSuccess) return hip_fail(e, "policy_mlp");
    return ANTSRL_OK;
}

extern "C" int antsrl_set_inloop_policy(AntsHandle *h, int32_t n_features, const float *w1, const float *b1, const float *w2,
                                        const float *b2, const float *w3, const float *b3, int8_t *rotation_next,
                                        int8_t *pheromone_next, void *stream)
{
    if (!h) return fail(ANTSRL_E_INVALID, "NULL handle");
    if (!w1) {
        h->pol = PolArgs{};
        return ANTSRL_OK;
    }
    if (!b1 || !w2 || !b2 || !rotation_next)
        return fail(ANTSRL_E_INVALID, "inloop_policy: w1, b1, w2, b2, rotation_next are required");
    if ((w3 == nullptr) != (b3 == nullptr) || (pheromone_next && !w3))
        return fail(ANTSRL_E_INVALID, "inloop_policy: w3/b3 go together and are needed for a pheromone output");
    if (n_features != h->p.PP * h->p.K)
        return fail(ANTSRL_E_INVALID, "inloop_policy: n_features must be P*P*K = %d", h->p.PP * h->p.K);
    if (!h->obs_bf16 || !antsrl_inloop_policy_supported(h->p))
        return fail(ANTSRL_E_UNSUPPORTED, "inloop_policy needs the cell-meta path (ANTSRL_Q_CELL_META) with bfloat16 "
                                          "observations (antsrl_set_obs_format) — use antsrl_policy_mlp otherwise");
    if (h->obs_pitch != 0 && h->obs_pitch != (uint32_t)(h->p.PP * h->p.K))
        return fail(ANTSRL_E_UNSUPPORTED, "the in-loop policy and a padded observation row stride exclude each other (the net reads a "
                                          "dense tile image): antsrl_set_obs_row_stride(h, 0) first");
    hipError_t e = antsrl_launch_policy_pack(h->p.s.pol_pack, w1, b1, w2, b2, w3, b3, n_features, (hipStream_t)stream);
    if (e != hipSuccess) return hip_fail(e, "inloop_policy pack");
    h->pol.pack = h->p.s.pol_pack;
    h->pol.rot = rotation_next;
    h->pol.ph = pheromone_next;
    h->pol.ks = (n_features + 15) / 16;
    return ANTSRL_OK;
}

static size_t state_bytes(const AntsHandle *h, int which)
{
    const size_t E = h->p.E, N = h->p.N, G = (size_t)h->p.W * h->p.H, C = h->p.C, R = h->p.R;
    switch (which) {
    case ANTSRL_S_ANTS_XYT: return 8 * E * N * 3;
    case ANTSRL_S_PREV_XY: return 8 * E * N * 2;
    case ANTSRL_S_HOLDING: case ANTSRL_S_SEED: return 4 * E * N;
    case ANTSRL_S_MANDIBLES: case ANTSRL_S_REWARD_STATE: return E * N;
    case ANTSRL_S_ACTIVATION: return 4 * E * N * C;
    case ANTSRL_S_PHERO: return 4 * E * C * G;
    case ANTSRL_S_FOOD: return 4 * E * G;
    case ANTSRL_S_EXPLORED: case ANTSRL_S_WALLS: case ANTSRL_S_ANTHILL_AREA: return E * G;
    case ANTSRL_S_ANTHILL_FOOD: return 8 * E;
    case ANTSRL_S_ROCK_CENTERS: return 8 * E * R * 2;
    case ANTSRL_S_TIMESTEP: return 4 * E;
    case ANTSRL_S_ANTHILL_XYR: return 4 * E * 3;
    case ANTSRL_S_ROCK_RW: return 8 * E * R * 2;
    case ANTSRL_S_PHERO_C0: case ANTSRL_S_PHERO_C1: case ANTSRL_S_PHERO_C2: case ANTSRL_S_PHERO_C3:
        return (size_t)(which - ANTSRL_S_PHERO_C0) < C ? 4 * E * G : 0;
    default: return 0;
    }
}

extern "C" int antsrl_state_bytes(const AntsHandle *h, int which, size_t *bytes)
{
    if (!h || !bytes) return fail(ANTSRL_E_INVALID, "NULL handle or bytes");
    if (which < 0 || which >= ANTSRL_S_COUNT_) return fail(ANTSRL_E_INVALID, "bad state selector %d", which);
    *bytes = state_bytes(h, which);
    return ANTSRL_OK;
}

extern "C" int antsrl_perceptive_field(AntsHandle *h, uint8_t *dst, void *stream)
{
    if (!h || !dst) return fail(ANTSRL_E_INVALID, "NULL handle or dst");
    if (!h->is_reset) return not_reset(h);
    hipError_t e = antsrl_launch_perceptive_field(h->p, dst, (hipStream_t)stream);
    if (e != hipSuccess) return hip_fail(e, "perceptive_field");
    return ANTSRL_OK;
}

static int recorder_layout(const char *who, const AntsHandle *h, int32_t n_sel, int32_t max_frames, int32_t with_heatmap,
                           RecorderLayout *L)
{
    if (!h) return fail(ANTSRL_E_INVALID, "%s: NULL handle", who);
    if (n_sel < 1 || n_sel > ANTSRL_RECORDER_MAX_ENVS)
        return fail(ANTSRL_E_INVALID, "%s: n_sel %d is not in 1..%d", who, n_sel, ANTSRL_RECORDER_MAX_ENVS);
    if (max_frames < 1) return fail(ANTSRL_E_INVALID, "%s: max_frames must be >= 1 (%d)", who, max_frames);
    const bool keeps_map = h->cfg.reward_kind == ANTSRL_REWARD_EXPLORATION || h->cfg.reward_kind == ANTSRL_REWARD_ALL;
    *L = antsrl_recorder_layout(n_sel, h->p.N, h->p.R, h->p.C, (size_t)h->p.W * h->p.H, with_heatmap && keeps_map ? 1 : 0);
    return ANTSRL_OK;
}

static int recorder_check(const char *who, const AntsHandle *h, const void *block, const int32_t *env_indices, int32_t n_sel,
                          int32_t max_frames, int32_t with_heatmap, bool has_frame, int32_t frame, RecorderLayout *L, RecorderSel *sel)
{
    int rc = recorder_layout(who, h, n_sel, max_frames, with_heatmap, L);
    if (rc) return rc;
    if (!block) return fail(ANTSRL_E_INVALID, "%s: NULL block", who);
    if ((uintptr_t)block & 15) return fail(ANTSRL_E_INVALID, "%s: block must be 16-byte aligned", who);
    if (!env_indices) return fail(ANTSRL_E_INVALID, "%s: NULL env_indices", who);
    memset(sel, 0, sizeof(*sel));
    for (int s = 0; s < n_sel; ++s) {
        const int32_t e = env_indices[s];
        if (e < 0 || e >= h->p.E)
            return fail(ANTSRL_E_INVALID, "%s: env_indices[%d] = %d is not in [0, n_envs = %d)", who, s, e, h->p.E);
        for (int t = 0; t < s; ++t)
            if (sel->env[t] == e) return fail(ANTSRL_E_INVALID, "%s: env_indices[%d] repeats environment %d", who, s, e);
        sel->env[s] = e;
    }
    if (has_frame && (frame < 0 || frame >= max_frames))
        return fail(ANTSRL_E_INVALID, "%s: frame %d is not in [0, max_frames = %d)", who, frame, max_frames);
    if (!h->is_reset) return not_reset(h);
    if (h->phase_next) return mid_update(h);
    return ANTSRL_OK;
}

extern "C" int antsrl_recorder_sizes(const AntsHandle *h, int32_t n_sel, int32_t max_frames, int32_t with_heatmap,
                                     size_t *static_bytes, size_t *frame_bytes, size_t *bytes)
{
    RecorderLayout L;
    int rc = recorder_layout("recorder_sizes", h, n_sel, max_frames, with_heatmap, &L);
    if (rc) return rc;
    if (static_bytes) *static_bytes = L.static_bytes;
    if (frame_bytes) *frame_bytes = L.frame_bytes;
    if (bytes) *bytes = L.static_bytes + (size_t)max_frames * L.frame_bytes;
    return ANTSRL_OK;
}

extern "C" int antsrl_recorder_begin(AntsHandle *h, void *block, const int32_t *env_indices, int32_t n_sel,
                                     int32_t max_frames, int32_t with_heatmap, void *stream)
{
    RecorderLayout L;
    RecorderSel sel;
    int rc = recorder_check("recorder_begin", h, block, env_indices, n_sel, max_frames, with_heatmap, false, 0, &L, &sel);
    if (rc) return rc;
    rc = flush_pending(h, (hipStream_t)stream);
    if (rc) return rc;
    hipError_t e = antsrl_launch_record_static(h->p, L, sel, (unsigned char *)block, (hipStream_t)stream);
    if (e != hipSuccess) return hip_fail(e, "recorder_begin");
    return ANTSRL_OK;
}

extern "C" int antsrl_recorder_frame(AntsHandle *h, void *block, const int32_t *env_indices, int32_t n_sel,
                                     int32_t max_frames, int32_t with_heatmap, int32_t frame, void *stream)
{
    RecorderLayout L;
    RecorderSel sel;
    int rc = recorder_check("recorder_frame", h, block, env_indices, n_sel, max_frames, with_heatmap, true, frame, &L, &sel);
    if (rc) return rc;
    rc = flush_pending(h, (hipStream_t)stream);
    if (rc) return rc;
    hipError_t e = antsrl_launch_record_frame(h->p, h->cur, L, sel,
                                              (unsigned char *)block + L.static_bytes + (size_t)frame * L.frame_bytes,
                                              (hipStream_t)stream);
    if (e != hipSuccess) return hip_fail(e, "recorder_frame");
    return ANTSRL_OK;
}

static int render_opts(const char *who, const AntsHandle *h, int32_t n_sel, const AntsRenderOpts *o)
{
    if (!h) return fail(ANTSRL_E_INVALID, "%s: NULL handle", who);
    if (!o) return fail(ANTSRL_E_INVALID, "%s: NULL opts", who);
    if (n_sel < 1 || n_sel > ANTSRL_RECORDER_MAX_ENVS)
        return fail(ANTSRL_E_INVALID, "%s: n_sel %d is not in 1..%d", who, n_sel, ANTSRL_RECORDER_MAX_ENVS);
    if (o->zoom < 1 || o->zoom > ANTSRL_RENDER_MAX_ZOOM)
        return fail(ANTSRL_E_INVALID, "%s: zoom %d is not in 1..%d", who, o->zoom, ANTSRL_RENDER_MAX_ZOOM);
    if (o->ant_radius < 0 || o->ant_radius > ANTSRL_RENDER_MAX_ANT_RADIUS)
        return fail(ANTSRL_E_INVALID, "%s: ant_radius %d is not in 0..%d", who, o->ant_radius, ANTSRL_RENDER_MAX_ANT_RADIUS);
    if (!(o->phero_max_val > 0.0)) return fail(ANTSRL_E_INVALID, "%s: phero_max_val must be > 0 (%g)", who, o->phero_max_val);
    if (o->view_mask & ~ANTSRL_RENDER_VIEW_ALL)
        return fail(ANTSRL_E_INVALID, "%s: view_mask 0x%x has bits outside 0x%x", who, (unsigned)o->view_mask, ANTSRL_RENDER_VIEW_ALL);
    return ANTSRL_OK;
}

extern "C" int antsrl_render_sizes(const AntsHandle *h, int32_t n_sel, const AntsRenderOpts *o, size_t *frame_env_bytes,
                                   size_t *scratch_bytes_per_frame)
{
    int rc = render_opts("render_sizes", h, n_sel, o);
    if (rc) return rc;
    const size_t W = (size_t)h->p.W, H = (size_t)h->p.H, Z = (size_t)o->zoom;
    if (frame_env_bytes) *frame_env_bytes = o->layer_only ? 4 * W * H : 3 * (W * Z) * (H * Z);
    if (scratch_bytes_per_frame) *scratch_bytes_per_frame = 4 * (size_t)n_sel;
    return ANTSRL_OK;
}

extern "C" int antsrl_render_frames(AntsHandle *h, const void *block, int32_t n_sel, int32_t max_frames, int32_t with_heatmap,
                                    int32_t first, int32_t count, const AntsRenderOpts *o, void *out, void *scratch, void *stream)
{
    const char *who = "render_frames";
    int rc = render_opts(who, h, n_sel, o);
    if (rc) return rc;
    RenderArgs a;
    memset(&a, 0, sizeof(a));
    rc = recorder_layout(who, h, n_sel, max_frames, with_heatmap, &a.L);
    if (rc) return rc;
    if (!block) return fail(ANTSRL_E_INVALID, "%s: NULL block", who);
    if (!out) return fail(ANTSRL_E_INVALID, "%s: NULL out", who);
    if (!scratch) return fail(ANTSRL_E_INVALID, "%s: NULL scratch", who);
    if ((uintptr_t)block & 15) return fail(ANTSRL_E_INVALID, "%s: block must be 16-byte aligned", who);
    if ((uintptr_t)out & 15) return fail(ANTSRL_E_INVALID, "%s: out must be 16-byte aligned", who);
    if ((uintptr_t)scratch & 15) return fail(ANTSRL_E_INVALID, "%s: scratch must be 16-byte aligned", who);
    if (first < 0 || count < 1 || (long long)first + count > max_frames)
        return fail(ANTSRL_E_INVALID, "%s: frames %d .. %d + %d are not inside [0, max_frames = %d)", who, first, first, count, max_frames);
    const size_t groups = o->layer_only ? render_layer_groups(a.L.G) : render_tiles(h->p.W, h->p.H, o->zoom);
    if (count > 65535 || groups * (size_t)n_sel * (size_t)count >= ANTSRL_RENDER_MAX_GROUPS)
        return fail(ANTSRL_E_INVALID, "%s: count %d is past the launch limits (65535 frames, %zu workgroups per frame of 2^24): split the call",
                    who, count, groups * (size_t)n_sel);
    if (!h->is_reset) return not_reset(h);
    a.block = (const unsigned char *)block;
    a.out = (unsigned char *)out;
    a.fmax = (int32_t *)scratch;
    a.W = h->p.W; a.H = h->p.H; a.Z = o->zoom; a.TY = render_ty(o->zoom); a.view = o->view_mask; a.ra = o->ant_radius; a.first = first; a.count = count;
    a.phero_den = o->phero_max_val + 0.0001;
    memcpy(a.col, o->phero_colors, sizeof(a.col));
    hipError_t e = antsrl_launch_render(a, o->layer_only != 0, (hipStream_t)stream);
    if (e != hipSuccess) return hip_fail(e, who);
    return ANTSRL_OK;
}

extern "C" int antsrl_read_state(AntsHandle *h, int which, void *dst, void *stream)
{
    if (!h || !dst) return fail(ANTSRL_E_INVALID, "NULL handle or dst");
    if (!h->is_reset) return not_reset(h);
    if (which < 0 || which >= ANTSRL_S_COUNT_) return fail(ANTSRL_E_INVALID, "bad state selector %d", which);
    if (state_bytes(h, which) == 0) return ANTSRL_OK;
    int frc = flush_pending(h, (hipStream_t)stream);
    if (frc) return frc;
    hipError_t e = antsrl_launch_read_state(h->p, which, h->cur, dst, (hipStream_t)stream);
    if (e != hipSuccess) return hip_fail(e, "read_state");
    return ANTSRL_OK;
}
```

### antsrl_amd/csrc/antsrl_device.h

```cpp
#pragma once
#include <stdint.h>
#include "../../include/antsrl.h"

#define META_PRES_MASK 0xFFFFu
#define META_WALL 0x10000u
#define META_AREA 0x20000u
#define META_STAMP_SHIFT 18
#define META_NEVER 0x3FFFu

struct __align__(16) AntFrame { double cx, cy, ct, st; };
#define UMFWD_WIN 0x100
struct UmFwd {
    double x, y, th;
    double th_new, sn, cs;
    float food, hold;
    uint32_t meta;
    int m, rot, pa;
    int rec;
    int pre;
    int has_rot;
    int ts;
    uint8_t primed;
    uint32_t frm_off;
};

struct DState {
    double *x, *y, *theta, *prev_x, *prev_y;
    double *prev_dist;
    float *holding, *seed, *prev_holding;
    float *activation;
    uint8_t *mandibles, *reward_state;
    int32_t *dirty_cell;
    int32_t *walldep_cell;
    float *phero[2];
    float *food;
    uint32_t *walls_bits, *area_bits, *explored_bits;
    uint32_t *big_pres, *big_old;
    int32_t *anthill_xyr;
    double *anthill_food;
    double *rock_cx, *rock_cy, *rock_r, *rock_w;
    int32_t *timestep;
    uint8_t *reward_primed;
    int32_t *gen_discs;
    int32_t *gen_perlin;
    uint8_t *primed_cur;
    AntFrame *frames;
    unsigned char *pol_pack;
};

#define ANTSRL_POL_MAX_KSTEPS 64
#define ANTSRL_POL_WPACK_BYTES (ANTSRL_POL_MAX_KSTEPS * 64 * 16)
#define ANTSRL_POL_A2PACK_BYTES (2 * 64 * 16)
#define ANTSRL_POL_LANEPACK_FLOATS (48 * 64 + 8)
#define ANTSRL_POL_PACK_BYTES (ANTSRL_POL_WPACK_BYTES + ANTSRL_POL_A2PACK_BYTES + 4 * ANTSRL_POL_LANEPACK_FLOATS)
struct PolArgs {
    const unsigned char *pack;
    int8_t *rot, *ph;
    int ks;
    int _pad;
};

struct KP {
    DState s;
    int32_t E, N, W, H, C, R, K, P, PP, r, words;
    int32_t HT;
    int32_t has_mask, has_max_val, reward_kind, max_time, filter_radius, explore_on;
    int32_t ch_kind[ANTSRL_MAX_CHANNELS], ch_arg[ANTSRL_MAX_CHANNELS];
    int32_t mand_first, mand_last;
    uint8_t mask[ANTSRL_MAX_PCELLS + 7];
    double delta, fwd_delta, max_speed, max_rot_speed, carry, backward, max_hold;
    double max_val, deposit_strength, threshold, reward_threshold;
    double fct_explore, fct_food, fct_anthill, fct_explore_holding, fct_heading;
    double filter[ANTSRL_MAX_FILTER_TAPS];
    uint64_t rng_seed;
    uint32_t env_id_base, _pad0;
    int32_t scaled, _pad;
    int32_t ps, fs;
    int32_t meta;
    int32_t tiled;
    int32_t ftile;
    int32_t _pad3;
    double g_now;
    double g_dep;
    double inv_g_dep;
    float ftap[2 * ANTSRL_MAX_FILTER_TAPS];
    int32_t filter_sep, _pad2;
    float fsep_u[2 * (2 * ANTSRL_MAX_FILTER_RADIUS + 1)], fsep_v[2 * (2 * ANTSRL_MAX_FILTER_RADIUS + 1)];
};

#define ACT_STEP 1
#define ACT_HAS_OBS 2
#define ACT_OBS_BF16 8
#define ACT_FRAMES 16
```

### antsrl_amd/csrc/antsrl_perceive.hip

```cpp
#include "antsrl_util.h"
#include "antsrl_flush.h"
#include "antsrl_update_one.h"
#include <type_traits>

#define PRC_UNROLL 2

#define PLAYOUT_DEFAULT 1
#define PLAYOUT_DEFAULT_ROCKS 2

__host__ __device__ inline size_t move_lds_bytes(int HT, int N)
{
    return align_up(8 * (size_t)HT + 12 * (size_t)N, 16);
}

template <int C>
__device__ __forceinline__ void move_body(const KP &p, const int e, const int8_t *__restrict__ rotation,
                                          const int8_t *__restrict__ phero_act, uint8_t *__restrict__ done, const int do_step,
                                          const uint32_t seq, unsigned char *smem, const UmFwd *fw = nullptr)
{
    const int tid = threadIdx.x, T = blockDim.x;
    const int N = p.N, W = p.W, H = p.H;
    const size_t G = (size_t)W * H, eN = (size_t)e * N;
    uint32_t *hkeys = (uint32_t *)smem, *hvals = hkeys + p.HT;
    float *tmp_q = (float *)(hvals + p.HT), *tmp_d = tmp_q + N;
    uint32_t *cprevs = (uint32_t *)(tmp_d + N);

    const uint32_t *area = p.s.area_bits + (size_t)e * p.words;
    const FoodView food{p.s.food + (size_t)e * G * p.fs, p.fs};
    uint16_t *pres = reinterpret_cast<uint16_t *>(p.s.food + (size_t)e * G * p.fs) + 2;
    const size_t FS2 = 2 * (size_t)p.fs;

    const bool one = fw ? true : N <= T;
    const size_t a1 = eN + (tid < N ? tid : 0);
    double h_x = 0.0, h_y = 0.0, h_th = 0.0;
    float h_hold = 0.0f, h_q = 0.0f;
    int h_m = 0, h_rot = 0, h_pa = 0;
    uint32_t h_cprev = 0u;
    if (one) {
        if (fw) {
            h_x = fw->x; h_y = fw->y; h_th = fw->th;
            h_hold = fw->hold; h_m = fw->m & 1; h_rot = fw->rot; h_pa = fw->pa;
            h_cprev = frec_xy(p, (int)fw->x, (int)fw->y);
            if (fw->rec) h_q = (fw->meta & META_AREA) ? 0.0f : fw->food;
            else h_q = food[h_cprev];
        } else {
            h_x = p.s.x[a1]; h_y = p.s.y[a1]; h_th = p.s.theta[a1];
            h_hold = p.s.holding[a1];
            if (do_step) {
                const double ppx = STP_LD(p.s.prev_x[a1]), ppy = STP_LD(p.s.prev_y[a1]);
                h_m = STP_LD(p.s.mandibles[a1]);
                if (rotation) h_rot = STP_LD(rotation[a1]);
                if (phero_act) h_pa = STP_LD(phero_act[a1]);
                h_cprev = frec_xy(p, (int)ppx, (int)ppy);
                h_q = food[h_cprev];
            }
        }
    }
    if (do_step && !fw)
        for (int h = tid; h < p.HT; h += T) {
            hkeys[h] = HASH_EMPTY;
            hvals[h] = 0u;
        }
    if (tid == 0) {
        if (p.reward_kind != ANTSRL_REWARD_NONE) {
            p.s.primed_cur[e] = fw ? fw->primed : p.s.reward_primed[e];
            p.s.reward_primed[e] = 1;
        }
        if (do_step && done) done[e] = (uint8_t)(p.max_time == (fw ? fw->ts : p.s.timestep[e]));
    }
    if (!fw) __syncthreads();
    else __builtin_amdgcn_sched_barrier(0);

    if (do_step) {
        for (int i = tid; i < N; i += T) {
            double x, y;
            uint32_t cprev;
            float q, hold;
            int old_m;
            if (one) {
                x = h_x; y = h_y; cprev = h_cprev; q = h_q; old_m = h_m; hold = h_hold;
            } else {
                x = p.s.x[eN + i]; y = p.s.y[eN + i];
                cprev = frec_xy(p, (int)p.s.prev_x[eN + i], (int)p.s.prev_y[eN + i]);
                q = food[cprev];
                old_m = p.s.mandibles[eN + i];
                hold = p.s.holding[eN + i];
            }
            const uint32_t ccur = (uint32_t)((int)x * H + (int)y);
            int m = old_m;
            {
                const int set = q > 0.0f;
                const int keep = 1 - (int)((fw && fw->rec) ? (fw->meta & META_AREA) != 0 : test_bit(area, ccur));
                if (p.mand_first == 1) m |= set;
                else if (p.mand_first == 2) m &= keep;
                if (p.mand_last == 1) m |= set;
                else if (p.mand_last == 2) m &= keep;
            }
            const int closing = m & (1 - old_m), opening = (1 - m) & old_m;
            const float taken = fminf((float)p.max_hold, fmaxf(0.0f, q)) * (float)closing;
            const float dropped = hold * (float)opening;
            h_hold = hold + (taken - dropped);
            p.s.holding[eN + i] = h_hold;
            STP_ST(p.s.mandibles[eN + i], (uint8_t)m);
            cprevs[i] = cprev;
            tmp_q[i] = q;
            tmp_d[i] = dropped - taken;
            if (fw) break;
            lww_insert(hkeys, hvals, (uint32_t)p.HT - 1, cprev, (uint32_t)i);
        }
        if (!fw) __syncthreads();
        else __builtin_amdgcn_sched_barrier(0);
        for (int i = tid; i < N; i += T) {
            const uint32_t cprev = cprevs[i];
            const float delta = tmp_d[i];
            int32_t dirty = -1;
            if (delta != 0.0f && (fw ? (fw->m & UMFWD_WIN) != 0 : lww_winner(hkeys, hvals, (uint32_t)p.HT - 1, cprev) == (uint32_t)i)) {
                food[cprev] = tmp_q[i] + delta;
                if (__float_as_uint((&food[cprev])[1]) & META_AREA) dirty = (int32_t)cprev;
            }
            STP_ST(p.s.dirty_cell[eN + i], dirty);
            if (fw) break;
        }
    }

    for (int i = tid; i < N; i += T) {
        double x, y, th;
        if (one) {
            x = h_x; y = h_y; th = h_th;
        } else {
            x = p.s.x[eN + i]; y = p.s.y[eN + i]; th = p.s.theta[eN + i];
        }
        if (do_step) {
            if (phero_act) {
                const int a = one ? h_pa : (int)phero_act[eN + i];
                float a0 = 0.0f, a1 = 0.0f;
                if (a == 1) a0 = (float)p.deposit_strength;
                else if (a != 0) a1 = (float)p.deposit_strength;
                STP_ST(p.s.activation[(eN + i) * C + 0], a0);
                if (C > 1) STP_ST(p.s.activation[(eN + i) * C + 1], a1);
            }
            double sn, cs;
            if (fw && fw->pre) {
                th = fw->th_new; sn = fw->sn; cs = fw->cs;
            } else {
                if (rotation)
                    th = np_mod_d(th + (double)(one ? h_rot : (int)rotation[eN + i]) * p.max_rot_speed, 2 * PI_D);
                sincos(th, &sn, &cs);
            }
            double fwd = 1.0 * p.max_speed * (1 - (double)(one ? h_hold : p.s.holding[eN + i]) * p.carry);
            if (fwd < 0) fwd *= p.backward;
            x = warp_coord(x + cs * fwd, (double)W);
            y = warp_coord(y + sn * fwd, (double)H);
            p.s.x[eN + i] = x;
            p.s.y[eN + i] = y;
            p.s.theta[eN + i] = th;
        }
        const uint32_t cell = frec_xy(p, wrap_index((int)x, W), wrap_index((int)y, H));
        pres[(size_t)cell * FS2] = (uint16_t)seq;
        if (fw && fw->frm_off) {
            const double *fs = reinterpret_cast<const double *>(smem + fw->frm_off) + 2 * i;
            AntFrame f;
            const bool shifted = p.fwd_delta != 0.0;
            f.cx = shifted ? x + fw->cs * p.fwd_delta : x;
            f.cy = shifted ? y + fw->sn * p.fwd_delta : y;
            f.ct = fs[0];
            f.st = fs[1];
            p.s.frames[eN + i] = f;
        }
        if (fw) break;
    }
}

template <int C>
__global__ void __launch_bounds__(1024)
k_move(const KP p, const int8_t *__restrict__ rotation, const int8_t *__restrict__ phero_act,
       uint8_t *__restrict__ done, const int do_step, const uint32_t seq)
{
    extern __shared__ __align__(16) unsigned char smem[];
    move_body<C>(p, env_of_block(blockIdx.x, p.E, seq), rotation, phero_act, done, do_step, seq, smem);
}

template <int C, bool ILV>
__global__ void __launch_bounds__(1024, 8)
k_update_move(const KP p, const int out_buf, const double g_dep, const double inv_g_dep, const int8_t *__restrict__ rotation,
              const int8_t *__restrict__ phero_act, uint8_t *__restrict__ done, const uint32_t seq, const int with_frames)
{
    extern __shared__ __align__(16) unsigned char smem[];
    const int e = env_of_block(blockIdx.x, p.E, seq);
    UmFwd fw = {};
    {
        const size_t a = (size_t)e * p.N + (threadIdx.x < (unsigned)p.N ? threadIdx.x : 0);
        fw.hold = p.s.holding[a];
        fw.m = STP_LD(p.s.mandibles[a]);
        if (rotation) fw.rot = STP_LD(rotation[a]);
        if (phero_act) fw.pa = STP_LD(phero_act[a]);
        fw.has_rot = rotation != nullptr;
        fw.primed = p.s.reward_primed[e];
    }
    fw.rec = (ILV && C == 2) ? 1 : 0;
    fw.frm_off = with_frames ? (uint32_t)align_up(max(update_one_lds_bytes(p.HT, p.R, (int)(blockDim.x >> 6), p.N), move_lds_bytes(p.HT, p.N)), 16) : 0u;
    update_one_body<C, ILV>(p, e, nullptr, out_buf, smem, g_dep, inv_g_dep, &fw);
    __syncthreads();
    move_body<C>(p, e, rotation, phero_act, done, 1, seq, smem, &fw);
}

struct PrcOff {
    uint32_t rock, wave0, frame, rm, stage, per_wave, stride;
    size_t total;
};

__host__ __device__ __forceinline__ PrcOff prc_offsets(int run, int PP, int K, int R, int nwaves, bool no_stage = false, uint32_t pitch = 0,
                                                       bool rock_reg = false)
{
    PrcOff o;
    o.rock = 0;
    o.wave0 = (uint32_t)(32 * (size_t)(R > 0 ? R : 1));
    o.frame = 0;
    o.rm = (uint32_t)(sizeof(AntFrame) * (size_t)run);
    o.stage = (uint32_t)align_up(o.rm + ((R > 0 && !rock_reg) ? 4 * (size_t)run : 0), 16);
    const size_t rowf = (size_t)PP * K;
    o.stride = (uint32_t)((2 * rowf + 32 + 3) / 4 * 4);
    if (2 * pitch > o.stride) o.stride = 2 * pitch;
    o.per_wave = (uint32_t)align_up(o.stage + (no_stage ? 0 : 4 * (size_t)o.stride), 16);
    o.total = o.wave0 + (size_t)nwaves * o.per_wave;
    return o;
}

__host__ __device__ __forceinline__ uint32_t prc_policy_img_elems(int row) { return (uint32_t)((32 * row + 8 + 32 + 7) / 8 * 8); }

#define PRC_TPB 256

__device__ __forceinline__ int prc_tile_ant(const int w, const int j, const int run, const int nwaves)
{
    (void)nwaves;
    return w * run + j;
}

typedef __attribute__((ext_vector_type(8))) __bf16 prc_bf16x8;
typedef __attribute__((ext_vector_type(16))) float prc_f32x16;
typedef __attribute__((ext_vector_type(4))) uint32_t prc_u4;

__device__ __forceinline__ void policy_tile(const PolArgs &pol, const uint16_t *img, const uint32_t img_shift, const float *as_lds,
                                            const int F, const int rows, const size_t ant0, const int lane)
{
    const int r = lane & 31, h = lane >> 5;
    const prc_u4 *wpack = reinterpret_cast<const prc_u4 *>(pol.pack);
    const prc_u4 *a2pack = reinterpret_cast<const prc_u4 *>(pol.pack + ANTSRL_POL_WPACK_BYTES);
    const float *lanepack = reinterpret_cast<const float *>(pol.pack + ANTSRL_POL_WPACK_BYTES + ANTSRL_POL_A2PACK_BYTES);
    const int rc = min(r, rows - 1);
    const float as0 = (float)(__bf16)as_lds[2 * rc], as1 = (float)(__bf16)as_lds[2 * rc + 1];
    prc_f32x16 acc;
#pragma unroll
    for (int g = 0; g < 16; ++g) acc[g] = 0.0f;
    const uint32_t off0 = img_shift + (uint32_t)r * (uint32_t)F + 8u * h;
    const int ks = pol.ks;
    constexpr int POL_AHEAD = 6;
    prc_u4 a[POL_AHEAD];
#pragma unroll
    for (int i = 0; i < POL_AHEAD; ++i) a[i] = wpack[min(i, ks - 1) * 64 + lane];
    for (int s0 = 0; s0 < ks; s0 += POL_AHEAD) {
#pragma unroll
        for (int i = 0; i < POL_AHEAD; ++i) {
            const int s = s0 + i;
            const prc_u4 a_s = a[i];
            a[i] = wpack[min(s + POL_AHEAD, ks - 1) * 64 + lane];
            if (s < ks) {
                const uint32_t off = off0 + 16u * s, sh = (off & 1u) * 16u;
                const uint32_t *d = reinterpret_cast<const uint32_t *>(img) + (off >> 1);
                const uint32_t d0 = d[0], d1 = d[1], d2 = d[2], d3 = d[3], d4 = d[4];
                const prc_u4 packed = {__builtin_amdgcn_alignbit(d1, d0, sh), __builtin_amdgcn_alignbit(d2, d1, sh),
                                       __builtin_amdgcn_alignbit(d3, d2, sh), __builtin_amdgcn_alignbit(d4, d3, sh)};
                acc = __builtin_amdgcn_mfma_f32_32x32x16_bf16(__builtin_bit_cast(prc_bf16x8, a_s),
                                                              __builtin_bit_cast(prc_bf16x8, packed), acc, 0, 0, 0);
            }
        }
    }
    prc_f32x16 acc2;
#pragma unroll
    for (int g = 0; g < 16; ++g) acc2[g] = 0.0f;
#pragma unroll
    for (int s = 0; s < 2; ++s) {
        prc_bf16x8 hfrag;
#pragma unroll
        for (int j = 0; j < 8; ++j) {
            const int g = 8 * s + j;
            const float bias1 = lanepack[g * 64 + lane], was0 = lanepack[(16 + g) * 64 + lane], was1 = lanepack[(32 + g) * 64 + lane];
            hfrag[j] = (__bf16)(acc[g] + (as0 * was0 + as1 * was1) + bias1);
        }
        acc2 = __builtin_amdgcn_mfma_f32_32x32x16_bf16(__builtin_bit_cast(prc_bf16x8, a2pack[s * 64 + lane]), hfrag, acc2, 0, 0, 0);
    }
    float lg[6];
    lg[0] = acc2[0]; lg[1] = acc2[1]; lg[2] = acc2[2]; lg[3] = acc2[3];
    lg[4] = __shfl(acc2[0], r + 32); lg[5] = __shfl(acc2[1], r + 32);
#pragma unroll
    for (int o = 0; o < 6; ++o) lg[o] += lanepack[48 * 64 + o];
    if (h == 0 && r < rows) {
        int ar = 0, ap = 0;
        if (lg[1] > lg[ar]) ar = 1;
        if (lg[2] > lg[ar]) ar = 2;
        if (lg[4] > lg[3 + ap]) ap = 1;
        if (lg[5] > lg[3 + ap]) ap = 2;
        pol.rot[ant0 + r] = (int8_t)(ar - 1);
        if (pol.ph) pol.ph[ant0 + r] = (int8_t)ap;
    }
}

#ifndef PRC_SGPR_CAP
#define PRC_SGPR_CAP 96
#endif
#ifndef PRC_MIN_WAVES
#define PRC_MIN_WAVES 7
#endif
#define PRC_SGPR_ATTR __attribute__((amdgpu_num_sgpr(PRC_SGPR_CAP)))
template <int LAYOUT, bool OBS16, bool ILV, bool HAS_OBS, bool POLICY = false, bool PAD = false, bool FAST = false>
__global__ void __launch_bounds__(PRC_TPB, PRC_MIN_WAVES) PRC_SGPR_ATTR
k_perceive(const KP p, const float *__restrict__ cells, float *__restrict__ obs, float *__restrict__ agent_state,
           float *__restrict__ reward, const int flags, const uint32_t seq, const int run, const int nseg, const PolArgs pol,
           const uint32_t pitch_arg)
{
    static_assert(!POLICY || OBS16, "the in-loop policy reads bfloat16 rows");
    static_assert(!PAD || (HAS_OBS && !POLICY), "padded rows: an observation tensor, no in-loop policy image");
    static_assert(!FAST || ILV, "the fast path reads interleaved records");
    extern __shared__ __align__(16) unsigned char smem[];
    constexpr int C = 2;
    const int tid = threadIdx.x;
    const int lane = tid & 63, wave = __builtin_amdgcn_readfirstlane(tid >> 6);
    constexpr int nwaves = PRC_TPB / 64;
    const int N = p.N, W = p.W, H = p.H, K = p.K, P = p.P, PP = p.PP, R = p.R;
    const size_t G = (size_t)W * H;
    int e, seg;
    {
        const int b = blockIdx.x;
        if ((p.E & 7) == 0) {
            const int j = b >> 3;
            e = (j / nseg) * 8 + (b & 7);
            seg = j % nseg;
        } else {
            e = b / nseg;
            seg = b % nseg;
        }
        e = env_of_block(e, p.E, seq);
    }
    const PrcOff lo = prc_offsets(run, PP, K, R, nwaves, POLICY, PAD ? pitch_arg : 0u, FAST);
    double *rock = (double *)(smem + lo.rock);
    unsigned char *wbase = smem + lo.wave0 + (size_t)wave * lo.per_wave;
    AntFrame *frames = (AntFrame *)(wbase + lo.frame);
    uint32_t *rmask = (uint32_t *)(wbase + lo.rm);
    (void)rmask;
    float *stage = (float *)(wbase + lo.stage);
    uint16_t *pol_img = reinterpret_cast<uint16_t *>(smem + align_up(lo.total, 16));
    float *pol_as = reinterpret_cast<float *>(pol_img + prc_policy_img_elems(PP * K));
    const size_t tile_elem0 = ((size_t)e * N + (size_t)(seg * nwaves * run)) * (size_t)(PP * K);
    uint16_t *tile0 = pol_img + (uint32_t)((((uintptr_t)obs >> 1) + tile_elem0) & 7);
    (void)tile0;
    if constexpr (POLICY) {
        const uint32_t rowe = (uint32_t)PP * (uint32_t)K, n_img = prc_policy_img_elems(PP * K);
        const int t0_ = seg * nwaves * run;
        for (int j = 0; j < run; ++j) {
            if (t0_ + wave * run + j < N) continue;
            uint16_t *rz = tile0 + (uint32_t)(wave * run + j) * rowe;
            for (uint32_t i = lane; i < rowe; i += 64) rz[i] = 0;
        }
        if (wave == 0) {
            const uint32_t sh = (uint32_t)(tile0 - pol_img), tail0 = sh + (uint32_t)(nwaves * run) * rowe;
            if ((uint32_t)lane < sh) pol_img[lane] = 0;
            for (uint32_t i = tail0 + lane; i < n_img; i += 64) pol_img[i] = 0;
        }
    }

    const size_t eN = (size_t)e * N;
    const int t_begin = seg * nwaves * run;
    int n_run = 0;
    for (int j = 0; j < run; ++j) n_run += (t_begin + prc_tile_ant(wave, j, run, nwaves) < N) ? 1 : 0;
#define PRC_ANT(j) (t_begin + prc_tile_ant(wave, (j), run, nwaves))

    const size_t a_pre = eN + (size_t)min(PRC_ANT(min(lane, max(n_run, 1) - 1)), N - 1);
    const float pre_hold = p.s.holding[a_pre];
    const float pre_seed = (agent_state || POLICY) ? p.s.seed[a_pre] : 0.0f;
    uint32_t rm_lane = 0u;
    {
        const uint32_t wsel = (blockIdx.x >> 3) + (blockIdx.x >> 8);
        const int w_pro = (POLICY && nwaves > 1) ? 1 + (int)(wsel % (nwaves > 1 ? nwaves - 1 : 1)) : (int)(wsel % nwaves);
        const int w_rock = (w_pro + 1) % nwaves;
        const bool have_frames = (flags & ACT_FRAMES) != 0;
        if (have_frames && lane < n_run) frames[lane] = p.s.frames[eN + (size_t)PRC_ANT(lane)];
        if (wave == w_rock) {
            for (int q = lane; q < R; q += 64) {
                const double rad = p.s.rock_r[(size_t)e * R + q];
                rock[4 * q + 0] = p.s.rock_cx[(size_t)e * R + q];
                rock[4 * q + 1] = p.s.rock_cy[(size_t)e * R + q];
                rock[4 * q + 2] = rad;
                rock[4 * q + 3] = sqrt_lt_threshold(rad);
            }
        }
        if (wave == w_pro && !have_frames) {
            const bool fwd = p.fwd_delta != 0.0;
            const int n_slot = nwaves * run, n_task = fwd ? 2 * n_slot : n_slot;
            for (int t = lane; t < n_task; t += 64) {
                const int which = t >= n_slot ? 1 : 0;
                const int sl = which ? t - n_slot : t, w2 = sl / run, j2 = sl - w2 * run;
                const int ant = t_begin + prc_tile_ant(w2, j2, run, nwaves);
                if (ant < N) {
                    const size_t a = eN + (size_t)ant;
                    AntFrame *fr = reinterpret_cast<AntFrame *>(smem + lo.wave0 + (size_t)w2 * lo.per_wave + lo.frame) + j2;
                    const double th = p.s.theta[a], x = p.s.x[a], y = p.s.y[a];
                    double sn, cs;
                    sincos(which ? th : th + PI_D * 0.5, &sn, &cs);
                    if (which) {
                        fr->cx = x + cs * p.fwd_delta;
                        fr->cy = y + sn * p.fwd_delta;
                    } else {
                        fr->ct = cs;
                        fr->st = sn;
                        if (!fwd) {
                            fr->cx = x;
                            fr->cy = y;
                        }
                    }
                }
            }
        }
        if (!have_frames || R > 0) __syncthreads();
        else wave_lds_sync();
        if (lane < n_run) {
            uint32_t rm = 0u;
            if (R > 0) {
                const double xf = frames[lane].cx, yf = frames[lane].cy;
                const double margin = (double)p.r * p.delta * 1.4142135623730951 + 1.5;
                const bool border = xf - margin < 0 || yf - margin < 0 || xf + margin >= W || yf + margin >= H;
                for (int q = 0; q < R; ++q) {
                    const double dx = rock[4 * q + 0] - xf, dy = rock[4 * q + 1] - yf;
                    const double rr = rock[4 * q + 2] + margin;
                    if (border || dx * dx + dy * dy < rr * rr) rm |= 1u << q;
                }
            }
            if constexpr (FAST) rm_lane = rm;
            else if (R > 0) rmask[lane] = rm;
        }
    }
    const bool wave_rocks = FAST && LAYOUT == PLAYOUT_DEFAULT_ROCKS && __ballot(rm_lane != 0u) != 0ull;
    (void)wave_rocks;
    wave_lds_sync();
    if (n_run <= 0) {
        if constexpr (POLICY) __syncthreads();
        return;
    }

    const float *ph = cells + (size_t)e * G * (size_t)p.ps;
    const float *fm = p.s.food + (size_t)e * G * p.fs;
    uint32_t *metaw = reinterpret_cast<uint32_t *>(p.s.food + (size_t)e * G * p.fs) + 1;
    const size_t FS = (size_t)p.fs;
    const bool explore = p.explore_on != 0;
    constexpr bool has_obs = HAS_OBS;
    constexpr bool has_rows = HAS_OBS || POLICY;
    const float inv_max = 1.0f / (float)p.max_val;
    const float g_now = (float)p.g_now;
    const float cut = p.scaled ? (float)p.threshold : 0.0f;
    const uint32_t row = (uint32_t)PP * (uint32_t)K;
    const bool wrap_fast = !FAST && W > 4 * (p.r + 4) && H > 4 * (p.r + 4) && p.fwd_delta < W / 4 && p.fwd_delta < H / 4 &&
                           p.fwd_delta > -W / 4 && p.fwd_delta > -H / 4 && p.delta < 2.0;
    const bool wrap_pow2 = FAST || ((W & (W - 1)) == 0 && (H & (H - 1)) == 0);

    const int q = lane < PP ? lane : PP - 1;
    const double of_px = (double)(q % P - p.r) * p.delta;
    const double of_py = (double)(q / P - p.r) * p.delta;
    const bool mask_q = p.has_mask ? p.mask[q] != 0 : true;
    const uint32_t qK = (uint32_t)q * K;
    const bool own = mask_q || explore;
    const unsigned long long need_mask = __ballot(own);
    const int src_lane = own ? lane : (need_mask ? __builtin_ctzll(need_mask) : 0);

    const bool tiled = FAST || p.tiled != 0, ftile = !FAST && p.ftile != 0;
#define PRC_SLOT(ix, iy) (tiled ? tiled_slot((ix), (iy), H) : ftile ? tiled44_slot((ix), (iy), H) : (uint32_t)((ix) * H + (iy)))
#define PRC_LOAD4(ptr) (*reinterpret_cast<const stream_f4 *>(ptr))
#define PRC_FETCH(G0, GRP, PERM)                                                                            \
    {                                                                                                    \
        _Pragma("unroll") for (int u = 0; u < PRC_UNROLL; ++u)                                           \
        {                                                                                                \
            const int j_ = min((G0) + u, n_run - 1);                                                     \
            const AntFrame fr = frames[j_];                     \
            const double rx = fr.ct * of_px - fr.st * of_py;                      \
            const double ry = fr.st * of_px + fr.ct * of_py;                                             \
            int ix = (int)rint(rx + fr.cx);                                   \
            int iy = (int)rint(ry + fr.cy);                                                              \
            if (wrap_pow2) {     \
                ix &= W - 1; iy &= H - 1;                                                                \
            } else if (wrap_fast) {            \
                ix = (int)min(min((uint32_t)ix, (uint32_t)(ix + W)), (uint32_t)(ix - W));                \
                iy = (int)min(min((uint32_t)iy, (uint32_t)(iy + H)), (uint32_t)(iy - H));                \
            } else {                                                                                     \
                ix = wrap_index(ix, W); iy = wrap_index(iy, H);                                          \
            }                                                                                            \
            GRP.cell[u] = PRC_SLOT(ix, iy);                                                              \
            if (!ILV) GRP.pc[u] = (uint32_t)(ix * H + iy);   \
        }                                                                                                \
        _Pragma("unroll") for (int u = 0; u < PRC_UNROLL; ++u)                                           \
        {                                                                                                \
            const uint32_t gc_ = (PERM) ? (uint32_t)__shfl((int)GRP.cell[u], src_lane) : GRP.cell[u]; \
            if (ILV) {      \
                const stream_f4 t = PRC_LOAD4(ph + (size_t)gc_ * 4);                                     \
                GRP.pv[u][0] = t.x; GRP.pv[u][1] = t.y; GRP.fd[u] = t.z; GRP.mt[u] = __float_as_uint(t.w); \
            } else {                                                                                     \
                const uint32_t pc_ = (PERM) ? (uint32_t)__shfl((int)GRP.pc[u], src_lane) : GRP.pc[u];  \
                const float2 t = *reinterpret_cast<const float2 *>(ph + (size_t)pc_ * 2);                \
                const float2 f = *reinterpret_cast<const float2 *>(fm + (size_t)gc_ * 2);                \
                GRP.pv[u][0] = t.x; GRP.pv[u][1] = t.y; GRP.fd[u] = f.x; GRP.mt[u] = __float_as_uint(f.y); \
            }                                                                                            \
        }                                                                                                \
    }
    struct PrcGrp {
        uint32_t cell[PRC_UNROLL], mt[PRC_UNROLL], pc[ILV ? 1 : PRC_UNROLL];
        float pv[PRC_UNROLL][C], fd[PRC_UNROLL];
    };
    PrcGrp gA, gB, gC;
    uint32_t cntv = 0u;
    constexpr uint32_t LINE = OBS16 ? 64u : 32u, VEC = OBS16 ? 8u : 4u, ESZ = OBS16 ? 2u : 4u;
    const uint32_t pitch = PAD ? pitch_arg : row;
    unsigned char *run0 = reinterpret_cast<unsigned char *>(obs) + ((size_t)e * N + (size_t)PRC_ANT(0)) * pitch * ESZ;
    uint32_t carry = (has_obs && !PAD) ? (uint32_t)(((uintptr_t)run0 & 15) / ESZ) : 0u;
    (void)LINE; (void)VEC;
    if constexpr (PAD) {
        const uint32_t npad = pitch - row;
        if ((uint32_t)lane < npad) {
            if (OBS16) {
                reinterpret_cast<uint16_t *>(stage)[row + lane] = 0;
                reinterpret_cast<uint16_t *>(stage)[pitch + row + lane] = 0;
            } else {
                stage[row + lane] = 0.0f;
                stage[pitch + row + lane] = 0.0f;
            }
        }
    }
    auto process = [&](const PrcGrp &g, const int j0, auto rk) __attribute__((always_inline)) {
        constexpr bool WAVE_ROCKS = decltype(rk)::value;
        (void)WAVE_ROCKS;
#pragma unroll
        for (int u = 0; u < PRC_UNROLL; ++u) {
            const int j = min(j0 + u, n_run - 1);
            const bool real = (j0 + u < n_run) && lane < PP;
            const uint32_t mt = g.mt[u];
            const bool unexp = real && explore && (mt >> META_STAMP_SHIFT) >= seq;
            const uint32_t n_un = (uint32_t)__popcll(__ballot(unexp));
            cntv = (lane == j0 + u) ? n_un : cntv;
            if (unexp)
                reinterpret_cast<uint16_t *>(metaw)[(size_t)g.cell[u] * FS * 2 + 1] = (uint16_t)((seq << 2) | ((mt >> 16) & 3u));
            if (has_rows) {
                float pvs[C];
#pragma unroll
                for (int c = 0; c < C; ++c) {
                    float v = g.pv[u][c];
                    if (p.scaled) {
                        v *= g_now;
                        v = v < cut ? 0.0f : v;
                    }
                    pvs[c] = v * inv_max;
                }
                const float v_ants = (mt & META_PRES_MASK) == seq ? 1.0f : 0.0f;
                const float v_area = (mt & META_AREA) ? 1.0f : 0.0f;
                const float v_wall = (mt & META_WALL) ? 1.0f : 0.0f;
                float v_rock = 0.0f;
                if (LAYOUT == PLAYOUT_DEFAULT_ROCKS) {
                    uint32_t rm = 0u;
                    if constexpr (!FAST) rm = mask_q ? rmask[j] : 0u;
                    else if constexpr (WAVE_ROCKS)
                        rm = mask_q ? (uint32_t)__builtin_amdgcn_readlane((int)rm_lane, j) : 0u;
                    bool any = false;
                    if (rm) {
                        const AntFrame fr = frames[j];
                        int ix = (int)rint((fr.ct * of_px - fr.st * of_py) + fr.cx);
                        int iy = (int)rint((fr.st * of_px + fr.ct * of_py) + fr.cy);
                        if (wrap_pow2) {
                            ix &= W - 1; iy &= H - 1;
                        } else if (wrap_fast) {
                            ix = (int)min(min((uint32_t)ix, (uint32_t)(ix + W)), (uint32_t)(ix - W));
                            iy = (int)min(min((uint32_t)iy, (uint32_t)(iy + H)), (uint32_t)(iy - H));
                        } else {
                            ix = wrap_index(ix, W); iy = wrap_index(iy, H);
                        }
                        while (rm) {
                            const int r = __builtin_ctz(rm);
                            rm &= rm - 1;
                            const double vx = (double)ix - rock[4 * r + 0];
                            const double vy = (double)iy - rock[4 * r + 1];
                            any |= vx * vx + vy * vy < rock[4 * r + 3];
                        }
                    }
                    v_rock = any ? 1.0f : 0.0f;
                }
                const bool m = mask_q;
                if (OBS16) {
                    uint16_t *o16 = POLICY ? tile0 + (uint32_t)prc_tile_ant(wave, min(j0 + u, n_run - 1), run, nwaves) * row + qK
                                           : reinterpret_cast<uint16_t *>(stage) + carry + (uint32_t)u * pitch + qK;
                    o16[0] = bf16_bits(m ? v_ants : -1.0f); o16[1] = bf16_bits(m ? pvs[0] : -1.0f);
                    o16[2] = bf16_bits(m ? pvs[1] : -1.0f); o16[3] = bf16_bits(m ? v_area : -1.0f);
                    o16[4] = bf16_bits(m ? v_wall : -1.0f); o16[5] = bf16_bits(m ? g.fd[u] : -1.0f);
                    if (LAYOUT == PLAYOUT_DEFAULT_ROCKS) o16[6] = bf16_bits(m ? v_rock : -1.0f);
                } else {
                    float *o = stage + carry + (uint32_t)u * pitch + qK;
                    o[0] = m ? v_ants : -1.0f; o[1] = m ? pvs[0] : -1.0f; o[2] = m ? pvs[1] : -1.0f;
                    o[3] = m ? v_area : -1.0f; o[4] = m ? v_wall : -1.0f; o[5] = m ? g.fd[u] : -1.0f;
                    if (LAYOUT == PLAYOUT_DEFAULT_ROCKS) o[6] = m ? v_rock : -1.0f;
                }
            }
        }
        if (has_obs) {
            wave_lds_sync();
            const uint32_t rowp = (j0 + 1 < n_run) ? 2u * row : row;
            if constexpr (PAD) {
                const uint32_t n16 = ((j0 + 1 < n_run) ? 2u : 1u) * pitch / VEC, last = n16 - 1u;
                uint4 *d = reinterpret_cast<uint4 *>(reinterpret_cast<unsigned char *>(obs) + ((size_t)e * N + (size_t)PRC_ANT(j0)) * pitch * ESZ);
                const uint4 *sp = reinterpret_cast<const uint4 *>(stage);
                const uint32_t i1 = min((uint32_t)lane, last), i2 = min((uint32_t)lane + 64u, last), i3 = min((uint32_t)lane + 128u, last);
                const uint4 w1 = sp[i1], w2 = sp[i2];
                uint4 w3 = w2;
                if (!OBS16) w3 = sp[i3];
                store_stream(d + i1, w1);
                store_stream(d + i2, w2);
                if (!OBS16) store_stream(d + i3, w3);
            } else if (OBS16) {
                uint16_t *dst16 = reinterpret_cast<uint16_t *>(obs) + ((size_t)e * N + (size_t)PRC_ANT(j0)) * row;
                const uint32_t mis16 = (uint32_t)(((uintptr_t)dst16 >> 1) & 7);
                uint16_t *d_al = dst16 - mis16;
                uint16_t *st16 = POLICY ? tile0 + (uint32_t)prc_tile_ant(wave, j0, run, nwaves) * row - mis16 : reinterpret_cast<uint16_t *>(stage);
                const FlushPlanB16 f = flush_plan_b16((uint32_t)lane, mis16, rowp, (uint32_t)((uintptr_t)d_al >> 4) & 7u);
                const uint4 w1 = reinterpret_cast<const uint4 *>(st16)[f.g1];
                const uint4 w2 = reinterpret_cast<const uint4 *>(st16)[f.g2];
                const uint16_t we = st16[f.fe];
                store_stream(reinterpret_cast<uint4 *>(d_al) + f.g1, w1);
                store_stream(reinterpret_cast<uint4 *>(d_al) + f.g2, w2);
                store_stream(d_al + f.fe, we);
                carry = (uint32_t)(((uintptr_t)(reinterpret_cast<uint16_t *>(obs) + ((size_t)e * N + (size_t)PRC_ANT(j0 + 2)) * row) >> 1) & 7);
            } else {
                float *dst = reinterpret_cast<float *>(obs) + ((size_t)e * N + (size_t)PRC_ANT(j0)) * row;
                const uint32_t mis = (uint32_t)(((uintptr_t)dst >> 2) & 3);
                float *dst_al = dst - mis;
                const FlushPlanF32 f = flush_plan_f32((uint32_t)lane, mis, rowp, (uint32_t)((uintptr_t)dst_al >> 4) & 7u);
                const float4 v1 = reinterpret_cast<const float4 *>(stage)[f.j1];
                const float4 v2 = reinterpret_cast<const float4 *>(stage)[f.j2];
                const float4 v3 = reinterpret_cast<const float4 *>(stage)[f.j3];
                const float ve = stage[f.fe];
                store_stream(reinterpret_cast<float4 *>(dst_al) + f.j1, v1);
                store_stream(reinterpret_cast<float4 *>(dst_al) + f.j2, v2);
                store_stream(reinterpret_cast<float4 *>(dst_al) + f.j3, v3);
                store_stream(dst_al + f.fe, ve);
                carry = (uint32_t)(((uintptr_t)(reinterpret_cast<float *>(obs) + ((size_t)e * N + (size_t)PRC_ANT(j0 + 2)) * row) >> 2) & 3);
            }
            wave_lds_sync();
        }
    };
#define PRC_CHUNKS(PERM, RK)                                                                  \
    for (int c0 = 0; c0 < n_run; c0 += 4 * PRC_UNROLL) {                                      \
        constexpr std::integral_constant<bool, (RK)> rk_{};                                   \
        PRC_FETCH(min(c0, n_run - 1), gA, PERM)                                               \
        PRC_FETCH(min(c0 + PRC_UNROLL, n_run - 1), gB, PERM)                                  \
        __builtin_amdgcn_s_waitcnt(0x0F70);         \
        PRC_FETCH(min(c0 + 2 * PRC_UNROLL, n_run - 1), gC, PERM)                              \
        process(gA, c0, rk_);                                                                 \
        if (c0 + PRC_UNROLL < n_run) {                                                        \
            PRC_FETCH(min(c0 + 3 * PRC_UNROLL, n_run - 1), gA, PERM)                          \
            process(gB, c0 + PRC_UNROLL, rk_);                                                \
            if (c0 + 2 * PRC_UNROLL < n_run) {                                                \
                process(gC, c0 + 2 * PRC_UNROLL, rk_);                                        \
                if (c0 + 3 * PRC_UNROLL < n_run) {                                            \
                    process(gA, c0 + 3 * PRC_UNROLL, rk_);                                    \
                }                                                                             \
            }                                                                                 \
        }                                                                                     \
    }
#define PRC_CHUNKS_RK(PERM)                                                                   \
    if (LAYOUT == PLAYOUT_DEFAULT_ROCKS && wave_rocks) PRC_CHUNKS(PERM, true)                 \
    else PRC_CHUNKS(PERM, false)
    if constexpr (FAST) {
        if (need_mask == ~0ull) {
            PRC_CHUNKS_RK(false)
        } else {
            PRC_CHUNKS_RK(true)
        }
    } else {
        PRC_CHUNKS(true, false)
    }
#undef PRC_CHUNKS_RK
#undef PRC_CHUNKS
#undef PRC_FETCH

    if (lane < n_run) {
        const size_t a = eN + (size_t)PRC_ANT(lane);
        const float hold = pre_hold, seed = pre_seed;
        if (agent_state) {
            store_stream(agent_state + a * 2 + 0, hold);
            store_stream(agent_state + a * 2 + 1, seed);
        }
        if constexpr (POLICY) {
            pol_as[2 * prc_tile_ant(wave, lane, run, nwaves)] = hold;
            pol_as[2 * prc_tile_ant(wave, lane, run, nwaves) + 1] = seed;
        }
        double rw = 0.0;
        if (p.reward_kind == ANTSRL_REWARD_EXPLORATION) {
            rw = (double)cntv / 10.0;
        } else if (p.reward_kind != ANTSRL_REWARD_NONE) {
            const float prev_h = p.s.primed_cur[e] ? p.s.prev_holding[a] : hold;
            const double dh = (double)hold - (double)prev_h;
            if (p.reward_kind == ANTSRL_REWARD_FOOD) {
                rw = dh < 0 ? 10.0 : dh;
                p.s.prev_holding[a] = hold;
            } else {
                const double r_food = dh < 0 ? 0.0 : dh;
                const double r_anthill = dh < 0 ? 1.0 : 0.0;
                p.s.prev_holding[a] = hold;
                if (explore) {
                    double re = (double)cntv / 10.0;
                    re = (hold == 0.0f) ? re * p.fct_explore : re * p.fct_explore_holding;
                    rw += re;
                }
                const double dx = p.s.x[a] - (double)p.s.anthill_xyr[3 * e + 0];
                const double dy = p.s.y[a] - (double)p.s.anthill_xyr[3 * e + 1];
                const double nd = sqrt(dx * dx + dy * dy);
                const double heading = (double)((p.s.prev_dist[a] > nd) && (hold > 0.0f)) * 0.1;
                p.s.prev_dist[a] = nd;
                rw += r_food * p.fct_food + r_anthill * p.fct_anthill + heading * p.fct_heading;
            }
        }
        if (reward) store_stream(reward + a, (float)rw);
        if ((flags & ACT_STEP) && rw - p.reward_threshold > 0) p.s.reward_state[a] = 255;
    }
#undef PRC_ANT
    if constexpr (POLICY) {
        __syncthreads();
        const int t0 = seg * nwaves * run;
        if (wave == 0) {
            policy_tile(pol, pol_img, (uint32_t)(tile0 - pol_img), pol_as, (int)row, min(nwaves * run, N - t0), eN + (size_t)t0, lane);
        }
    }
}

__global__ void k_meta_rebase(const KP p)
{
    const size_t n = (size_t)p.E * p.W * p.H;
    uint32_t *m = reinterpret_cast<uint32_t *>(p.s.food) + 1;
    for (size_t i = (size_t)blockIdx.x * blockDim.x + threadIdx.x; i < n; i += (size_t)gridDim.x * blockDim.x) {
        const uint32_t v = m[i * p.fs];
        m[i * p.fs] = (v & (META_WALL | META_AREA)) | ((v >> META_STAMP_SHIFT) != META_NEVER ? 0u : META_NEVER << META_STAMP_SHIFT);
    }
}

static int prc_layout(const KP &p)
{
    static const int def[7] = {ANTSRL_CH_ANTS, ANTSRL_CH_PHERO, ANTSRL_CH_PHERO, ANTSRL_CH_ANTHILL,
                               ANTSRL_CH_WALLS, ANTSRL_CH_FOOD, ANTSRL_CH_ROCKS};
    if (p.C != 2 || (p.K != 6 && p.K != 7)) return 0;
    for (int k = 0; k < p.K; ++k)
        if (p.ch_kind[k] != def[k]) return 0;
    if (p.ch_arg[1] != 0 || p.ch_arg[2] != 1) return 0;
    return p.K == 6 ? PLAYOUT_DEFAULT : PLAYOUT_DEFAULT_ROCKS;
}

bool antsrl_meta_supported(const KP &p)
{
    const uint32_t row = (uint32_t)p.PP * p.K;
    return prc_layout(p) != 0 && p.PP <= 64 && row >= 128 && row <= 368 && p.N <= 4096 &&
           move_lds_bytes(p.HT, p.N) <= 160 * 1024;
}

static int n_cus()
{
    static int n[ANTSRL_MAX_DEVICES] = {};
    int dev = 0;
    if (hipGetDevice(&dev) != hipSuccess || dev < 0 || dev >= ANTSRL_MAX_DEVICES) return 256;
    if (!n[dev] && hipDeviceGetAttribute(&n[dev], hipDeviceAttributeMultiprocessorCount, dev) != hipSuccess) n[dev] = 256;
    return n[dev] > 0 ? n[dev] : 256;
}

static int pick_run(const KP &p)
{
    const long total = (long)p.E * p.N, slots = (long)n_cus() * 16;
    int run = 8;
    while (run > 2 && total / run < slots) run >>= 1;
    return run;
}

int antsrl_perceive_run(const KP &p) { return pick_run(p); }

hipError_t antsrl_launch_move(const KP &p, const int8_t *rot, const int8_t *ph, uint8_t *done, int do_step,
                              uint32_t seq, hipStream_t st)
{
    const int T = p.N <= 1024 ? (p.N + 63) / 64 * 64 : 1024;
    const size_t lds = move_lds_bytes(p.HT, p.N);
    static size_t seen[ANTSRL_MAX_DEVICES] = {};
    int dev = 0;
    if (hipGetDevice(&dev) != hipSuccess || dev < 0 || dev >= ANTSRL_MAX_DEVICES) return hipErrorInvalidDevice;
    if (lds > 64 * 1024 && lds > seen[dev]) {
        hipError_t err = hipFuncSetAttribute((const void *)k_move<2>, hipFuncAttributeMaxDynamicSharedMemorySize, (int)lds);
        if (err != hipSuccess) return err;
        seen[dev] = lds;
    }
    hipLaunchKernelGGL((k_move<2>), dim3(p.E), dim3(T), lds, st, p, rot, ph, done, do_step, seq);
    return hipGetLastError();
}

bool antsrl_update_move_supported(const KP &p)
{
    return p.meta && p.C == 2 && p.N <= 1024;
}

hipError_t antsrl_launch_update_move(const KP &p, int out_buf, double g_dep, double inv_g_dep, const int8_t *rot,
                                     const int8_t *ph, uint8_t *done, uint32_t seq, hipStream_t st, bool with_frames)
{
    const int T = (p.N + 63) / 64 * 64;
    const size_t lds = align_up(std::max(update_one_lds_bytes(p.HT, p.R, T / 64, p.N), move_lds_bytes(p.HT, p.N)), 16) +
                 16 * (size_t)T;
    static size_t seen[ANTSRL_MAX_DEVICES] = {};
    int dev = 0;
    if (hipGetDevice(&dev) != hipSuccess || dev < 0 || dev >= ANTSRL_MAX_DEVICES) return hipErrorInvalidDevice;
    const bool ilv = p.ps == 4;
    if (lds > 64 * 1024 && lds > seen[dev]) {
        hipError_t err = hipFuncSetAttribute((const void *)k_update_move<2, true>, hipFuncAttributeMaxDynamicSharedMemorySize, (int)lds);
        if (err == hipSuccess)
            err = hipFuncSetAttribute((const void *)k_update_move<2, false>, hipFuncAttributeMaxDynamicSharedMemorySize, (int)lds);
        if (err != hipSuccess) return err;
        seen[dev] = lds;
    }
    const int wf = with_frames ? 1 : 0;
    if (ilv) hipLaunchKernelGGL((k_update_move<2, true>), dim3(p.E), dim3(T), lds, st, p, out_buf, g_dep, inv_g_dep, rot, ph, done, seq, wf);
    else hipLaunchKernelGGL((k_update_move<2, false>), dim3(p.E), dim3(T), lds, st, p, out_buf, g_dep, inv_g_dep, rot, ph, done, seq, wf);
    return hipGetLastError();
}

template <int LAYOUT, bool OBS16, bool ILV, bool HAS_OBS, bool POLICY = false, bool PAD = false, bool FAST = false>
static hipError_t launch_perceive_t(const KP &p, const float *cells, float *obs, float *agent_state, float *reward,
                                    int flags, uint32_t seq, hipStream_t st, const PolArgs &pol = PolArgs{}, uint32_t pitch = 0)
{
    const int run = pick_run(p), nwaves = PRC_TPB / 64;
    if (POLICY && run * nwaves > 32) return hipErrorInvalidValue;
    const int nseg = (p.N + run * nwaves - 1) / (run * nwaves);
    const PrcOff lo = prc_offsets(run, p.PP, p.K, p.R, nwaves, POLICY, PAD ? pitch : 0u, FAST);
    const size_t lds = POLICY ? align_up(lo.total, 16) + 2 * (size_t)prc_policy_img_elems(p.PP * p.K) + 4 * 64 : lo.total;
    if (lds > 64 * 1024) return hipErrorInvalidValue;
    hipLaunchKernelGGL((k_perceive<LAYOUT, OBS16, ILV, HAS_OBS, POLICY, PAD, FAST>), dim3((unsigned)((size_t)p.E * nseg)), dim3(PRC_TPB), lds, st, p,
                       cells, obs, agent_state, reward, flags, seq, run, nseg, pol, pitch);
    return hipGetLastError();
}

bool antsrl_inloop_policy_supported(const KP &p) { return p.meta && pick_run(p) * (PRC_TPB / 64) <= 32; }

bool antsrl_perceive_fast(const KP &p)
{
    return (p.W & (p.W - 1)) == 0 && (p.H & (p.H - 1)) == 0 && p.tiled != 0 && p.ftile == 0 && p.ps == 4 && p.fs == 4 &&
           p.has_mask != 0;
}

hipError_t antsrl_launch_perceive(const KP &p, int cur, float *obs, float *agent_state, float *reward, int flags,
                                  uint32_t seq, hipStream_t st, const PolArgs *pol, uint32_t obs_pitch, bool generic)
{
    const int layout = prc_layout(p);
    const bool o16 = (flags & ACT_OBS_BF16) != 0, ilv = p.ps == 4 && p.fs == 4;
    const bool fast = !generic && antsrl_perceive_fast(p);
    const float *cells = p.s.phero[cur];
    const bool with_pol = pol && pol->pack && o16;
    const bool padded = obs && obs_pitch != 0 && obs_pitch != (uint32_t)(p.PP * p.K);
    if (padded && with_pol) return hipErrorNotSupported;
#define PRC_GO(LY)                                                                                             \
    {                                                                                                          \
        if (padded && o16) return launch_perceive_t<LY, true, ILVV, true, false, true, FASTV>(p, cells, obs, agent_state, reward, flags, seq, st, PolArgs{}, obs_pitch); \
        if (padded) return launch_perceive_t<LY, false, ILVV, true, false, true, FASTV>(p, cells, obs, agent_state, reward, flags, seq, st, PolArgs{}, obs_pitch); \
        if (with_pol && !obs) return launch_perceive_t<LY, true, ILVV, false, true, false, FASTV>(p, cells, obs, agent_state, reward, flags, seq, st, *pol); \
        if (!obs) return launch_perceive_t<LY, false, ILVV, false, false, false, FASTV>(p, cells, obs, agent_state, reward, flags, seq, st); \
        if (with_pol) return launch_perceive_t<LY, true, ILVV, true, true, false, FASTV>(p, cells, obs, agent_state, reward, flags, seq, st, *pol); \
        if (o16) return launch_perceive_t<LY, true, ILVV, true, false, false, FASTV>(p, cells, obs, agent_state, reward, flags, seq, st);    \
        return launch_perceive_t<LY, false, ILVV, true, false, false, FASTV>(p, cells, obs, agent_state, reward, flags, seq, st);            \
    }
#define PRC_GO2(LY)                                                                           \
    {                                                                                         \
        if (ilv && fast) { constexpr bool ILVV = true, FASTV = true; PRC_GO(LY) }             \
        else if (ilv) { constexpr bool ILVV = true, FASTV = false; PRC_GO(LY) }               \
        else { constexpr bool ILVV = false, FASTV = false; PRC_GO(LY) }                       \
    }
    if (layout == PLAYOUT_DEFAULT) PRC_GO2(PLAYOUT_DEFAULT)
    if (layout == PLAYOUT_DEFAULT_ROCKS) PRC_GO2(PLAYOUT_DEFAULT_ROCKS)
#undef PRC_GO2
#undef PRC_GO
    return hipErrorInvalidValue;
}

hipError_t antsrl_launch_meta_rebase(const KP &p, hipStream_t st)
{
    hipLaunchKernelGGL(k_meta_rebase, dim3(grid_for((size_t)p.E * p.W * p.H)), dim3(256), 0, st, p);
    return hipGetLastError();
}
```

### include/antsrl.h

```cpp
#ifndef ANTSRL_H
#define ANTSRL_H

#include <stddef.h>
#include <stdint.h>

#ifdef __cplusplus
extern "C" {
#endif

#define ANTSRL_ABI_VERSION 5

#define ANTSRL_MAX_CHANNELS 16
#define ANTSRL_MAX_PSIDE 15
#define ANTSRL_MAX_PCELLS (ANTSRL_MAX_PSIDE * ANTSRL_MAX_PSIDE)
#define ANTSRL_MAX_FILTER_RADIUS 3
#define ANTSRL_MAX_FILTER_TAPS 49
#define ANTSRL_MAX_PHERO 4

#define ANTSRL_OK 0
#define ANTSRL_E_INVALID (-1)
#define ANTSRL_E_NOMEM (-2)
#define ANTSRL_E_DEVICE (-3)
#define ANTSRL_E_UNSUPPORTED (-4)

enum {
    ANTSRL_CH_ANTS = 0,
    ANTSRL_CH_PHERO = 1,
    ANTSRL_CH_ANTHILL = 2,
    ANTSRL_CH_WALLS = 3,
    ANTSRL_CH_FOOD = 4,
    ANTSRL_CH_ROCKS = 5
};

enum { ANTSRL_PHERO_AUTO = 0, ANTSRL_PHERO_EXPLICIT_SWEEP = 1 };

enum { ANTSRL_ACT_AUTO = 0, ANTSRL_ACT_CELL_META = 1, ANTSRL_ACT_SINGLE_KERNEL = 2 };

enum {
    ANTSRL_REWARD_NONE = 0,
    ANTSRL_REWARD_EXPLORATION = 1,
    ANTSRL_REWARD_FOOD = 2,
    ANTSRL_REWARD_ALL = 3
};

typedef struct AntsCfg {
    int32_t abi_version;
    int32_t n_envs;
    int32_t n_ants;
    int32_t w, h;
    int32_t n_phero;
    int32_t n_rocks;
    int32_t max_time;

    int32_t perception_radius;
    int32_t n_channels;
    int32_t channel_kind[ANTSRL_MAX_CHANNELS];
    int32_t channel_arg[ANTSRL_MAX_CHANNELS];
    int32_t has_mask;
    uint8_t mask[ANTSRL_MAX_PCELLS];
    uint8_t _pad0[7];
    double delta;
    double fwd_delta;

    double max_speed, max_rot_speed, carry_speed_reduction, backward_speed_reduction;
    double max_hold;

    int32_t has_max_val;
    int32_t filter_radius;
    double phero_max_val;
    double deposit_strength;
    double phero_threshold;
    double filter[ANTSRL_MAX_FILTER_TAPS];

    int32_t reward_kind;
    int32_t phero_mode;
    double reward_threshold;
    double fct_explore, fct_food, fct_anthill, fct_explore_holding, fct_headinganthill;

    uint64_t rng_seed;

    int32_t act_path;

    int32_t env_id_base;
    int32_t n_envs_total;
    int32_t _pad1;
} AntsCfg;

typedef struct AntsInit {
    const double *ants_xyt;
    const double *seed;
    const uint8_t *walls;
    const float *food;
    const int32_t *anthill_xyr;
    const double *rocks;
    const float *phero;
} AntsInit;

#define ANTSRL_MAX_FOOD_DISCS 64
#define ANTSRL_WALLS_BERNOULLI 0
#define ANTSRL_WALLS_PERLIN 1
#define ANTSRL_WALLS_INPUT 2
#define ANTSRL_RNG_COUNTER 0
#define ANTSRL_RNG_REFERENCE 1
typedef struct AntsGen {
    double wall_density;
    int32_t n_food_discs;
    int32_t food_rmin, food_rmax;
    int32_t auto_reset;
    int32_t wall_kind;
    int32_t perlin_octaves;
    double perlin_scale;
    double perlin_persistence;
    double perlin_lacunarity;
    int32_t rng_kind;
    int32_t _pad;
    const uint8_t *walls_input;
} AntsGen;

typedef struct AntsHandle AntsHandle;

enum {
    ANTSRL_S_ANTS_XYT = 0,
    ANTSRL_S_PREV_XY = 1,
    ANTSRL_S_HOLDING = 2,
    ANTSRL_S_MANDIBLES = 3,
    ANTSRL_S_ACTIVATION = 4,
    ANTSRL_S_PHERO = 5,
    ANTSRL_S_FOOD = 6,
    ANTSRL_S_EXPLORED = 7,
    ANTSRL_S_ANTHILL_FOOD = 8,
    ANTSRL_S_ROCK_CENTERS = 9,
    ANTSRL_S_TIMESTEP = 10,
    ANTSRL_S_REWARD_STATE = 11,
    ANTSRL_S_WALLS = 12,
    ANTSRL_S_ANTHILL_AREA = 13,
    ANTSRL_S_SEED = 14,
    ANTSRL_S_ANTHILL_XYR = 15,
    ANTSRL_S_ROCK_RW = 16,
    ANTSRL_S_PHERO_C0 = 17,
    ANTSRL_S_PHERO_C1 = 18,
    ANTSRL_S_PHERO_C2 = 19,
    ANTSRL_S_PHERO_C3 = 20,
    ANTSRL_S_COUNT_
};

int antsrl_abi_version(void);

size_t antsrl_cfg_size(void);

const char *antsrl_last_error(void);

int antsrl_workspace_bytes(const AntsCfg *cfg, size_t *bytes);

int antsrl_create(const AntsCfg *cfg, void *workspace, size_t workspace_bytes, AntsHandle **out);

int antsrl_workspace_bytes2(const AntsCfg *cfg, size_t *state_bytes, size_t *record_bytes);
int antsrl_create2(const AntsCfg *cfg, void *state_ws, size_t state_bytes, void *record_ws, size_t record_bytes,
                   AntsHandle **out);

typedef struct AntsWsArray {
    char name[24];
    int32_t block, _pad;
    uint64_t offset, bytes;
} AntsWsArray;
int antsrl_workspace_map(const AntsCfg *cfg, int split, AntsWsArray *entries, int32_t cap, int32_t *count);

void antsrl_destroy(AntsHandle *h);

int antsrl_reset(AntsHandle *h, const AntsInit *init, void *stream);

int antsrl_generate(AntsHandle *h, const AntsGen *gen, uint64_t episode_seed, void *stream);

int antsrl_step(AntsHandle *h, const int8_t *rotation, const int8_t *phero, float *obs,
                float *agent_state, float *reward, uint8_t *done, void *stream);

int antsrl_observe(AntsHandle *h, float *obs, float *agent_state, float *reward, void *stream);

int antsrl_update(AntsHandle *h, const double *wall_jitter, void *stream);

enum { ANTSRL_PHASE_WALLS = 0, ANTSRL_PHASE_ROCKS_PHEROMONE = 1, ANTSRL_PHASE_ANTS = 2, ANTSRL_PHASE_ANTHILL = 3 };
int antsrl_update_phase(AntsHandle *h, int phase, const double *wall_jitter, void *stream);

int antsrl_flush(AntsHandle *h, void *stream);

int antsrl_step_update(AntsHandle *h, const int8_t *rotation, const int8_t *phero,
                       const double *wall_jitter, float *obs, float *agent_state, float *reward,
                       uint8_t *done, void *stream);

#define ANTSRL_TIMING_EVENTS 5
int antsrl_set_timing_events(AntsHandle *h, void *const *events);

enum {
    ANTSRL_Q_CELL_META = 0,
    ANTSRL_Q_SCALED_UNITS = 1,
    ANTSRL_Q_INTERLEAVED = 2,
    ANTSRL_Q_FILTER_SEPARABLE = 3,
    ANTSRL_Q_PERCEIVE_RUN = 4,
    ANTSRL_Q_TIMESTEP = 5,
    ANTSRL_Q_DEFERRED_UPDATE = 6,
    ANTSRL_Q_PERCEIVE_FAST = 7,
    ANTSRL_Q_COUNT_
};
int antsrl_query(const AntsHandle *h, int what, long long *value);

int antsrl_bench_copy(void *dst, const void *src, size_t bytes, void *stream);

#define ANTSRL_MEM_PIECE_BYTES ((size_t)16 << 20)
int antsrl_mem_alloc(size_t bytes, int device, void **ptr);
int antsrl_mem_free(void *ptr);
int antsrl_mem_trim(void);
int antsrl_mem_stats(size_t *live_bytes, size_t *pooled_bytes, size_t *reserved_va_bytes, size_t *retired_va_bytes);

#define ANTSRL_OBS_F32 0
#define ANTSRL_OBS_BF16 1
int antsrl_set_obs_format(AntsHandle *h, int format);

int antsrl_set_obs_row_stride(AntsHandle *h, int32_t stride_elems);

#define ANTSRL_PERCEIVE_AUTO 0
#define ANTSRL_PERCEIVE_GENERIC 1
int antsrl_set_perceive_path(AntsHandle *h, int path);

int antsrl_set_activation(AntsHandle *h, const float *act, double new_deposit_strength,
                          void *stream);

int antsrl_policy_mlp(AntsHandle *h, const float *obs, const float *agent_state, int64_t n_ants, int32_t n_features,
                      const float *w1, const float *b1, const float *w2, const float *b2, const float *w3,
                      const float *b3, int8_t *rotation, int8_t *pheromone, float *logits, void *stream);

int antsrl_set_inloop_policy(AntsHandle *h, int32_t n_features, const float *w1, const float *b1, const float *w2,
                             const float *b2, const float *w3, const float *b3, int8_t *rotation_next,
                             int8_t *pheromone_next, void *stream);

typedef struct AntsMemNetShape {
    int32_t n_features, agent_dim, mem_size, h1, h2, h3, n_rot, n_ph;
} AntsMemNetShape;

int antsrl_memnet_packed_bytes(const AntsMemNetShape *s, size_t *bytes);

int antsrl_memnet_pack(const AntsMemNetShape *s, const float *const *params, void *packed, void *stream);

int antsrl_policy_memory(const AntsMemNetShape *s, const void *packed, const void *obs, int obs_format,
                         const float *agent_state, const float *mem_in, int64_t n_ants, float *mem_out, int8_t *rotation,
                         int8_t *pheromone, float *q_out, void *stream);

#define ANTSRL_MEMNET_BF16 0
#define ANTSRL_MEMNET_FP32 1

int antsrl_memnet_packed_bytes_ex(const AntsMemNetShape *s, int precision, size_t *bytes);

int antsrl_memnet_pack_ex(const AntsMemNetShape *s, int precision, const float *const *params, void *packed, void *stream);

int antsrl_policy_memory_ex(const AntsMemNetShape *s, int precision, const void *packed, const void *obs, int obs_format,
                            const float *agent_state, const float *mem_in, int64_t n_ants, float *mem_out,
                            int8_t *rotation, int8_t *pheromone, float *q_out, void *stream);

int antsrl_policy_memory_tiles(const AntsMemNetShape *s, int precision, const void *packed, const void *obs, int obs_format,
                               const float *agent_state, const float *mem_in, int64_t n_ants, float *mem_out,
                               int8_t *rotation, int8_t *pheromone, float *q_out, const int32_t *tiles,
                               const int32_t *n_live, void *stream);

int antsrl_memtrain_sizes(const AntsMemNetShape *s, int64_t B, size_t *params_floats, size_t *trained_floats,
                          size_t *state_bytes, size_t *workspace_bytes);

int antsrl_memtrain_init(const AntsMemNetShape *s, const float *const *params, void *state, void *stream);

int antsrl_memtrain_unpack(const AntsMemNetShape *s, const void *state, float *const *params, void *stream);

int antsrl_memtrain_copy(const AntsMemNetShape *s, const void *src_state, void *dst_state, void *stream);

int antsrl_memtrain_grad(const AntsMemNetShape *s, const void *state, const void *target_state, const float *states,
                         const float *agent_states, const int64_t *actions, const float *rewards, const float *new_states,
                         const float *new_agent_states, const uint8_t *dones, const int64_t *idx, int64_t B,
                         float discount, float *grads, float *loss_out, void *workspace, void *stream);

int antsrl_memtrain_apply(const AntsMemNetShape *s, void *state, const float *grads, int64_t step, double lr,
                          double beta1, double beta2, double eps, void *stream);

#define ANTSRL_DRAW_EXPLORE 0x45584C4FULL
#define ANTSRL_DRAW_ROTATION 0x524F5441ULL
#define ANTSRL_DRAW_PHEROMONE 0x50484552ULL
#define ANTSRL_DRAW_SAMPLE 0x53414D50ULL

int antsrl_agent_select(uint64_t seed, uint64_t step, int32_t env_id_base, int32_t n_envs, int32_t n_ants, double epsilon,
                        int32_t n_rot, int32_t n_ph, int32_t mem_size, int8_t *rotation, int8_t *pheromone,
                        const float *mem_old, float *mem_next, uint8_t *explored, void *stream);

int antsrl_agent_plan(uint64_t seed, uint64_t step, int32_t env_id_base, int32_t n_envs, int32_t n_ants, double epsilon,
                      int32_t *tiles, int32_t *n_live, void *stream);

typedef struct AntsRecordSpec {
    int32_t n_envs, n_ants, env_id_base;
    int32_t n_features, agent_dim, mem_size, n_rot;
    int32_t obs_format;
    int32_t obs_pitch;
    int32_t reserved;
    int64_t K, head, max_len;
    uint64_t seed, step;
} AntsRecordSpec;

int antsrl_replay_record_pre(const AntsRecordSpec *r, const void *obs, const float *agent_state, const float *memory,
                             const int8_t *rotation, const int8_t *pheromone, float *states, float *agent_states,
                             int64_t *actions, void *stream);
int antsrl_replay_record_post(const AntsRecordSpec *r, const void *obs, const float *agent_state, const float *memory,
                              const float *reward, const uint8_t *done, float *rewards, float *new_states,
                              float *new_agent_states, uint8_t *dones, void *stream);

int antsrl_agent_select_actions(uint64_t seed, uint64_t step, int32_t env_id_base, int32_t n_envs, int32_t n_ants,
                                double epsilon, int32_t n_rot, int32_t n_ph, int8_t *rotation, int8_t *pheromone,
                                uint8_t *explored, void *stream);
int antsrl_replay_record_pre_plain(const AntsRecordSpec *r, const void *obs, const float *agent_state,
                                   const int8_t *rotation, const int8_t *pheromone, float *states, float *agent_states,
                                   int64_t *actions, void *stream);
int antsrl_replay_record_post_plain(const AntsRecordSpec *r, const void *obs, const float *agent_state, const float *reward,
                                    const uint8_t *done, float *rewards, float *new_states, float *new_agent_states,
                                    uint8_t *dones, void *stream);

int antsrl_lintrain_sizes(int32_t n_features, int64_t B, size_t *trained_floats, size_t *workspace_bytes, int32_t *launches);
int antsrl_lintrain_grad(int32_t n_features, const float *w1, const float *b1, const float *heads, const float *target_l3,
                         const float *states, const float *agent_states, const int64_t *actions, const float *rewards,
                         const float *new_states, const float *new_agent_states, const uint8_t *dones, int64_t n_rows,
                         const int64_t *idx, int64_t B, float discount, float *grads, float *loss, void *workspace,
                         void *stream);
int antsrl_lintrain_apply(float *heads, float *adam_m, float *adam_v, const float *grads, int64_t step, double lr,
                          double beta1, double beta2, double eps, void *stream);
int antsrl_lintrain_step(int32_t n_features, const float *w1, const float *b1, float *heads, const float *target_l3,
                         float *adam_m, float *adam_v, const float *states, const float *agent_states,
                         const int64_t *actions, const float *rewards, const float *new_states,
                         const float *new_agent_states, const uint8_t *dones, int64_t n_rows, const int64_t *idx, int64_t B,
                         float discount, int64_t step, double lr, double beta1, double beta2, double eps, float *grads,
                         float *loss, void *workspace, void *stream);

int antsrl_exptrain_sizes(int32_t n_features, int64_t B, size_t *trained_floats, size_t *workspace_bytes, int32_t *launches);
int antsrl_exptrain_grad(int32_t n_features, const float *model, const float *target, const float *states,
                         const float *agent_states, const int64_t *actions, const float *rewards, const float *new_states,
                         const float *new_agent_states, const uint8_t *dones, int64_t n_rows, const int64_t *idx, int64_t B,
                         float discount, float *grads, float *loss, void *workspace, void *stream);
int antsrl_exptrain_apply(int32_t n_features, float *model, float *adam_m, float *adam_v, const float *grads, int64_t step,
                          double lr, double beta1, double beta2, double eps, void *stream);
int antsrl_exptrain_step(int32_t n_features, float *model, const float *target, float *adam_m, float *adam_v,
                         const float *states, const float *agent_states, const int64_t *actions, const float *rewards,
                         const float *new_states, const float *new_agent_states, const uint8_t *dones, int64_t n_rows,
                         const int64_t *idx, int64_t B, float discount, int64_t step, double lr, double beta1, double beta2,
                         double eps, float *grads, float *loss, void *workspace, void *stream);

typedef struct AntsReworkShape {
    int32_t n_features, agent_dim,
            g1, g2, g3,
            r1, r2, r3,
            p1,
            n_rot, n_ph;
} AntsReworkShape;

int antsrl_rework_collapsed_bytes(const AntsReworkShape *s, size_t *bytes);

int antsrl_rework_collapse(const AntsReworkShape *s, const float *const *params, void *collapsed, void *stream);

int antsrl_policy_rework(const AntsReworkShape *s, const void *collapsed, const void *obs, int obs_format,
                         const float *agent_state, int64_t n_ants, int8_t *rotation, int8_t *pheromone, float *q_out,
                         void *stream);

int antsrl_policy_rework_select(const AntsReworkShape *s, const void *collapsed, const void *obs, int obs_format,
                                const float *agent_state, uint64_t seed, uint64_t step, int32_t env_id_base,
                                int32_t n_envs, int32_t n_ants, double epsilon, int8_t *rotation, int8_t *pheromone,
                                uint8_t *explored, float *q_out, void *stream);

int antsrl_reworktrain_sizes(const AntsReworkShape *s, int64_t B, size_t *params_floats, size_t *workspace_bytes,
                             int32_t *launches);
int antsrl_reworktrain_grad(const AntsReworkShape *s, const float *model, const float *target_collapsed, const float *states,
                            const float *agent_states, const int64_t *actions, const float *rewards, const float *new_states,
                            const float *new_agent_states, const uint8_t *dones, int64_t n_rows, const int64_t *idx,
                            int64_t B, float discount, float *grads, float *loss, void *workspace, void *stream);
int antsrl_reworktrain_apply(const AntsReworkShape *s, float *model, float *adam_m, float *adam_v, const float *grads,
                             int64_t step, double lr, double beta1, double beta2, double eps, void *stream);
int antsrl_reworktrain_step(const AntsReworkShape *s, float *model, const float *target_collapsed, float *adam_m,
                            float *adam_v, const float *states, const float *agent_states, const int64_t *actions,
                            const float *rewards, const float *new_states, const float *new_agent_states,
                            const uint8_t *dones, int64_t n_rows, const int64_t *idx, int64_t B, float discount,
                            int64_t step, double lr, double beta1, double beta2, double eps, float *grads, float *loss,
                            void *workspace, void *stream);

int antsrl_monitor_sizes(int32_t n_envs, int32_t n_ants, int32_t max_reports, int32_t max_episodes, size_t *bytes);
int antsrl_monitor_init(void *state, int32_t n_envs, int32_t n_ants, int32_t max_reports, int32_t max_episodes,
                        void *stream);
int antsrl_monitor_step(void *state, int32_t n_envs, int32_t n_ants, int32_t max_reports, int32_t max_episodes,
                        const float *reward, const float *loss_dev, double loss_host, int has_loss, int report_slot,
                        void *stream);
int antsrl_monitor_end_episode(void *state, int32_t n_envs, int32_t n_ants, int32_t max_reports, int32_t max_episodes,
                               int episode_slot, int last_report_slot, void *stream);

#define ANTSRL_RECORDER_MAX_ENVS 8
int antsrl_recorder_sizes(const AntsHandle *h, int32_t n_sel, int32_t max_frames, int32_t with_heatmap,
                          size_t *static_bytes, size_t *frame_bytes, size_t *bytes);
int antsrl_recorder_begin(AntsHandle *h, void *block, const int32_t *env_indices, int32_t n_sel,
                          int32_t max_frames, int32_t with_heatmap, void *stream);
int antsrl_recorder_frame(AntsHandle *h, void *block, const int32_t *env_indices, int32_t n_sel,
                          int32_t max_frames, int32_t with_heatmap, int32_t frame, void *stream);

#define ANTSRL_RENDER_MAX_ZOOM 8
#define ANTSRL_RENDER_MAX_ANT_RADIUS 1024
#define ANTSRL_RENDER_VIEW_ALL 63
typedef struct {
    int32_t zoom, view_mask, ant_radius, layer_only;
    double phero_max_val;
    uint8_t phero_colors[4][3];
} AntsRenderOpts;
int antsrl_render_sizes(const AntsHandle *h, int32_t n_sel, const AntsRenderOpts *o,
                        size_t *frame_env_bytes, size_t *scratch_bytes_per_frame);
int antsrl_render_frames(AntsHandle *h, const void *block, int32_t n_sel, int32_t max_frames, int32_t with_heatmap,
                         int32_t first, int32_t count, const AntsRenderOpts *o, void *out, void *scratch, void *stream);

int antsrl_read_state(AntsHandle *h, int which, void *dst, void *stream);

int antsrl_perceptive_field(AntsHandle *h, uint8_t *dst, void *stream);

int antsrl_state_bytes(const AntsHandle *h, int which, size_t *bytes);

#ifdef __cplusplus
}
#endif
#endif
```

Measured before the change: 2.741 billion.

## Skip perception of fully explored tiles using a periodic explored-tile bitmap summary

```diff
diff --git a/antsrl_amd/_lib.py b/antsrl_amd/_lib.py
--- a/antsrl_amd/_lib.py
+++ b/antsrl_amd/_lib.py
@@ -12,7 +12,7 @@
            "antsrl_workspace_map",
            "antsrl_destroy", "antsrl_reset", "antsrl_generate", "antsrl_step", "antsrl_observe", "antsrl_update", "antsrl_flush",
            "antsrl_step_update", "antsrl_set_timing_events", "antsrl_set_activation", "antsrl_policy_mlp", "antsrl_read_state", "antsrl_state_bytes",
-           "antsrl_set_obs_format", "antsrl_query", "antsrl_bench_copy", "antsrl_set_inloop_policy", "antsrl_set_obs_row_stride", "antsrl_set_perceive_path", "antsrl_mem_alloc", "antsrl_mem_free",
+           "antsrl_set_obs_format", "antsrl_query", "antsrl_bench_copy", "antsrl_set_inloop_policy", "antsrl_set_obs_row_stride", "antsrl_set_perceive_path", "antsrl_refresh_explored_summary", "antsrl_mem_alloc", "antsrl_mem_free",
            "antsrl_mem_trim", "antsrl_mem_stats", "antsrl_update_phase",
            "antsrl_perceptive_field", "antsrl_memnet_packed_bytes", "antsrl_memnet_pack", "antsrl_policy_memory",
            "antsrl_memtrain_sizes", "antsrl_memtrain_init", "antsrl_memtrain_unpack", "antsrl_memtrain_copy",
@@ -96,6 +96,7 @@
     lib.antsrl_bench_copy.argtypes = [vp, vp, C.c_size_t, vp]
     lib.antsrl_set_obs_row_stride.argtypes = [vp, i32]
     lib.antsrl_set_perceive_path.argtypes = [vp, i32]
+    lib.antsrl_refresh_explored_summary.argtypes = [vp, vp]
     lib.antsrl_mem_alloc.argtypes = [C.c_size_t, i32, C.POINTER(vp)]
     lib.antsrl_mem_free.argtypes = [vp]
     lib.antsrl_mem_trim.argtypes = []
diff --git a/antsrl_amd/batched.py b/antsrl_amd/batched.py
--- a/antsrl_amd/batched.py
+++ b/antsrl_amd/batched.py
@@ -477,6 +477,10 @@
     def set_perceive_path(self, path: int) -> None:
         _lib.check(self.lib.antsrl_set_perceive_path(self._h, int(path)), "set_perceive_path")
 
+    def refresh_explored_summary(self) -> None:
+        with self._on_device():
+            _lib.check(self.lib.antsrl_refresh_explored_summary(self._h, self._stream()), "refresh_explored_summary")
+
     def set_activation(self, act, new_deposit_strength: float = 0.0) -> None:
         c = self.cfg
         a = self._dev(act, torch.float32, (c.n_envs, c.n_ants, c.n_phero))
diff --git a/antsrl_amd/config.py b/antsrl_amd/config.py
--- a/antsrl_amd/config.py
+++ b/antsrl_amd/config.py
@@ -19,8 +19,8 @@
 PHERO_AUTO, PHERO_EXPLICIT_SWEEP = 0, 1
 ACT_AUTO, ACT_CELL_META, ACT_SINGLE_KERNEL = 0, 1, 2
 TIMING_EVENTS = 5
-Q_CELL_META, Q_SCALED_UNITS, Q_INTERLEAVED, Q_FILTER_SEPARABLE, Q_PERCEIVE_RUN, Q_TIMESTEP, Q_DEFERRED_UPDATE, Q_PERCEIVE_FAST = range(8)
-PERCEIVE_AUTO, PERCEIVE_GENERIC = 0, 1
+Q_CELL_META, Q_SCALED_UNITS, Q_INTERLEAVED, Q_FILTER_SEPARABLE, Q_PERCEIVE_RUN, Q_TIMESTEP, Q_DEFERRED_UPDATE, Q_PERCEIVE_FAST, Q_EXPLORED_SUMMARY = range(9)
+PERCEIVE_AUTO, PERCEIVE_GENERIC, PERCEIVE_FAST_NOSKIP = 0, 1, 2
 
 (S_ANTS_XYT, S_PREV_XY, S_HOLDING, S_MANDIBLES, S_ACTIVATION, S_PHERO, S_FOOD, S_EXPLORED,
  S_ANTHILL_FOOD, S_ROCK_CENTERS, S_TIMESTEP, S_REWARD_STATE, S_WALLS, S_ANTHILL_AREA,
diff --git a/antsrl_amd/csrc/antsrl_capi.hip b/antsrl_amd/csrc/antsrl_capi.hip
--- a/antsrl_amd/csrc/antsrl_capi.hip
+++ b/antsrl_amd/csrc/antsrl_capi.hip
@@ -35,6 +35,8 @@
 hipError_t antsrl_launch_policy_pack(unsigned char *pack, const float *w1, const float *b1, const float *w2, const float *b2,
                                      const float *w3, const float *b3, int F, hipStream_t st);
 hipError_t antsrl_launch_meta_rebase(const KP &p, hipStream_t st);
+bool antsrl_explored_summary_supported(const KP &p, bool with_policy);
+hipError_t antsrl_launch_explored_summary(const KP &p, hipStream_t st);
 bool antsrl_update_move_supported(const KP &p);
 hipError_t antsrl_launch_update_move(const KP &p, int out_buf, double g_dep, double inv_g_dep, const int8_t *rot,
                                      const int8_t *ph, uint8_t *done, uint32_t seq, hipStream_t st, bool with_frames);
@@ -58,6 +60,10 @@
     bool obs_bf16;
     uint32_t obs_pitch;
     bool prc_generic;
+    bool prc_noskip;
+    uint32_t sum_obs;
+    bool sum_due;
+    bool sum_live;
     bool need_wall_clear;
     hipEvent_t ev[ANTSRL_TIMING_EVENTS];
     bool ev_armed;
@@ -355,7 +361,7 @@
     h->pol = PolArgs{};
     h->sweeps = 0; h->need_wall_clear = false;
     h->has_gen = false; h->episode_seed = 0; h->host_timestep = 1; h->obs_bf16 = false; h->obs_pitch = 0;
-    h->prc_generic = false;
+    h->prc_generic = false; h->prc_noskip = false; h->sum_obs = 0; h->sum_due = false; h->sum_live = false;
     h->ws_bytes[0] = need[0]; h->ws_bytes[1] = need[1];
     h->ev_armed = false;
     h->obs_seq = 0;
@@ -420,7 +426,7 @@
     h->p.deposit_strength = h->cfg.deposit_strength;
     h->cur = 0; h->steps_since_update = 0; h->need_full_collect = true; h->is_reset = true; h->episode_over = false;
     h->sweeps = 0; h->need_wall_clear = h->p.scaled && init->phero != nullptr;
-    h->host_timestep = 1; h->obs_seq = 0;
+    h->host_timestep = 1; h->obs_seq = 0; h->sum_obs = 0; h->sum_due = false; h->sum_live = false;
     set_decay(h);
     return ANTSRL_OK;
 }
@@ -444,7 +450,7 @@
     if (e != hipSuccess) return hip_fail(e, "generate");
     h->p.deposit_strength = h->cfg.deposit_strength;
     h->cur = 0; h->steps_since_update = 0; h->need_full_collect = true; h->is_reset = true; h->episode_over = false;
-    h->sweeps = 0; h->need_wall_clear = false; h->host_timestep = 1; h->obs_seq = 0;
+    h->sweeps = 0; h->need_wall_clear = false; h->host_timestep = 1; h->obs_seq = 0; h->sum_obs = 0; h->sum_due = false; h->sum_live = false;
     h->episode_seed = seed;
     set_decay(h);
     return ANTSRL_OK;
@@ -522,9 +528,22 @@
 extern "C" int antsrl_set_perceive_path(AntsHandle *h, int path)
 {
     if (!h) return fail(ANTSRL_E_INVALID, "NULL handle");
-    if (path != ANTSRL_PERCEIVE_AUTO && path != ANTSRL_PERCEIVE_GENERIC) return fail(ANTSRL_E_INVALID, "bad perceive path %d", path);
+    if (path != ANTSRL_PERCEIVE_AUTO && path != ANTSRL_PERCEIVE_GENERIC && path != ANTSRL_PERCEIVE_FAST_NOSKIP)
+        return fail(ANTSRL_E_INVALID, "bad perceive path %d", path);
     h->prc_generic = path == ANTSRL_PERCEIVE_GENERIC;
-    return ANTSRL_OK;
+    h->prc_noskip = path == ANTSRL_PERCEIVE_FAST_NOSKIP;
+    return ANTSRL_OK;
+}
+
+static bool summary_on(const AntsHandle *h)
+{
+    return !h->prc_generic && !h->prc_noskip && antsrl_explored_summary_supported(h->p, h->pol.pack != nullptr && h->obs_bf16);
+}
+#define SUMMARY_FIRST 256u
+#define SUMMARY_STEADY 1024u
+static bool summary_cadence(uint32_t n)
+{
+    return n >= SUMMARY_FIRST && (n <= SUMMARY_STEADY ? (n & (n - 1u)) == 0u : n % SUMMARY_STEADY == 0u);
 }
 
 static int flush_pending(AntsHandle *h, hipStream_t st)
@@ -576,11 +595,23 @@
     if (timed) (void)hipEventRecord(h->ev[2], st);
     e = antsrl_launch_perceive(h->p, h->cur, obs, agent_state, reward,
                                (stepping ? ACT_STEP : 0) | (obs ? ACT_HAS_OBS : 0) | (frames ? ACT_FRAMES : 0) |
-                                   ((obs || h->pol.pack) && h->obs_bf16 ? ACT_OBS_BF16 : 0),
+                                   ((obs || h->pol.pack) && h->obs_bf16 ? ACT_OBS_BF16 : 0) |
+                                   (h->sum_live && summary_on(h) ? ACT_SUMMARY : 0),
                                h->obs_seq, st, &h->pol, h->obs_pitch, h->prc_generic);
     if (e == hipErrorNotSupported)
         return fail(ANTSRL_E_UNSUPPORTED, "a padded observation row stride and the in-loop policy exclude each other (the net reads a dense tile image)");
     if (e != hipSuccess) return hip_fail(e, "perceive");
+    if (summary_cadence(++h->sum_obs) && summary_on(h)) h->sum_due = true;
+    return ANTSRL_OK;
+}
+
+static int summary_refresh_due(AntsHandle *h, hipStream_t st)
+{
+    if (!h->sum_due) return ANTSRL_OK;
+    h->sum_due = false;
+    h->sum_live = true;
+    hipError_t e = antsrl_launch_explored_summary(h->p, st);
+    if (e != hipSuccess) return hip_fail(e, "explored summary");
     return ANTSRL_OK;
 }
 
@@ -657,7 +688,8 @@
     if (!h->is_reset) return not_reset(h);
     if (h->phase_next) return mid_update(h);
     if (!agent_state || !reward || !done) return fail(ANTSRL_E_INVALID, "agent_state, reward, done are required");
-    return do_step(h, rotation, phero, obs, agent_state, reward, done, (hipStream_t)stream);
+    int rc = do_step(h, rotation, phero, obs, agent_state, reward, done, (hipStream_t)stream);
+    return rc ? rc : summary_refresh_due(h, (hipStream_t)stream);
 }
 
 extern "C" int antsrl_observe(AntsHandle *h, float *obs, float *agent_state, float *reward, void *stream)
@@ -665,8 +697,10 @@
     if (!h) return fail(ANTSRL_E_INVALID, "NULL handle");
     if (!h->is_reset) return not_reset(h);
     if (h->phase_next) return mid_update(h);
-    if (h->p.meta)
-        return meta_observe(h, nullptr, nullptr, obs, agent_state, reward, nullptr, false, (hipStream_t)stream, false);
+    if (h->p.meta) {
+        int rc = meta_observe(h, nullptr, nullptr, obs, agent_state, reward, nullptr, false, (hipStream_t)stream, false);
+        return rc ? rc : summary_refresh_due(h, (hipStream_t)stream);
+    }
     if (obs && h->obs_pitch) return fail(ANTSRL_E_UNSUPPORTED, "antsrl_set_obs_row_stride needs the cell-meta path (ANTSRL_Q_CELL_META)");
     hipError_t e = antsrl_launch_act(h->p, nullptr, nullptr, h->cur, obs, agent_state, reward, nullptr,
                                      obs ? ACT_HAS_OBS | (h->obs_bf16 ? ACT_OBS_BF16 : 0) : 0, (hipStream_t)stream);
@@ -747,6 +781,20 @@
     return ANTSRL_OK;
 }
 
+extern "C" int antsrl_refresh_explored_summary(AntsHandle *h, void *stream)
+{
+    if (!h) return fail(ANTSRL_E_INVALID, "NULL handle");
+    if (!h->is_reset) return not_reset(h);
+    if (h->phase_next) return mid_update(h);
+    if (!summary_on(h)) return ANTSRL_OK;
+    int frc = flush_pending(h, (hipStream_t)stream);
+    if (frc) return frc;
+    h->sum_live = true;
+    hipError_t e = antsrl_launch_explored_summary(h->p, (hipStream_t)stream);
+    if (e != hipSuccess) return hip_fail(e, "explored summary");
+    return ANTSRL_OK;
+}
+
 extern "C" int antsrl_flush(AntsHandle *h, void *stream)
 {
     if (!h) return fail(ANTSRL_E_INVALID, "NULL handle");
@@ -774,6 +822,8 @@
     int rc = do_step(h, rotation, phero, obs, agent_state, reward, done, st, timed);
     if (rc) return rc;
     if (timed) (void)hipEventRecord(h->ev[3], st);
+    rc = summary_refresh_due(h, st);
+    if (rc) return rc;
     if (sweep_late) {
         hipError_t e = antsrl_launch_sweep(h->p, h->cur, st);
         if (e != hipSuccess) return hip_fail(e, "pheromone sweep");
@@ -805,6 +855,7 @@
     case ANTSRL_Q_TIMESTEP: *value = h->host_timestep; break;
     case ANTSRL_Q_DEFERRED_UPDATE: *value = antsrl_update_move_supported(h->p); break;
     case ANTSRL_Q_PERCEIVE_FAST: *value = h->p.meta && !h->prc_generic && antsrl_perceive_fast(h->p); break;
+    case ANTSRL_Q_EXPLORED_SUMMARY: *value = summary_on(h); break;
     default: return fail(ANTSRL_E_INVALID, "bad query selector %d", what);
     }
     return ANTSRL_OK;
diff --git a/antsrl_amd/csrc/antsrl_device.h b/antsrl_amd/csrc/antsrl_device.h
--- a/antsrl_amd/csrc/antsrl_device.h
+++ b/antsrl_amd/csrc/antsrl_device.h
@@ -91,4 +91,5 @@
 #define ACT_STEP 1
 #define ACT_HAS_OBS 2
 #define ACT_OBS_BF16 8
+#define ACT_SUMMARY 32
 #define ACT_FRAMES 16
diff --git a/antsrl_amd/csrc/antsrl_explored.h b/antsrl_amd/csrc/antsrl_explored.h
--- /dev/null
+++ b/antsrl_amd/csrc/antsrl_explored.h
@@ -0,0 +1,110 @@
+#pragma once
+#include <stdint.h>
+
+#if !defined(__HIPCC__) && !defined(__host__)
+#define __host__
+#define __device__
+#endif
+
+#define EXPL_TILE_SHIFT 3
+
+__host__ __device__ inline bool explored_tiles_ok(const int W, const int H)
+{
+    return W >= (1 << EXPL_TILE_SHIFT) && H >= (1 << EXPL_TILE_SHIFT) && (W & (W - 1)) == 0 && (H & (H - 1)) == 0;
+}
+
+__host__ __device__ inline uint32_t explored_tile_count(const int W, const int H)
+{
+    return (uint32_t)(W >> EXPL_TILE_SHIFT) * (uint32_t)(H >> EXPL_TILE_SHIFT);
+}
+__host__ __device__ inline uint32_t explored_tile_index(const int x, const int y, const int H)
+{
+    return (uint32_t)((x >> EXPL_TILE_SHIFT) * (H >> EXPL_TILE_SHIFT) + (y >> EXPL_TILE_SHIFT));
+}
+__host__ __device__ inline uint32_t explored_tile_word(const uint32_t t) { return t >> 5; }
+__host__ __device__ inline uint32_t explored_tile_bit(const uint32_t t) { return t & 31u; }
+
+struct ExplBox {
+    int tx0, ntx, ty0, nty;
+};
+
+__host__ __device__ inline double explored_box_margin(const int r, const double delta)
+{
+    return (double)r * delta * 1.4142135623730951 + 0.5;
+}
+
+__host__ __device__ inline int expl_floor_i(const double v)
+{
+    const int i = (int)v;
+    return (double)i > v ? i - 1 : i;
+}
+__host__ __device__ inline int expl_ceil_i(const double v)
+{
+    const int i = (int)v;
+    return (double)i < v ? i + 1 : i;
+}
+
+__host__ __device__ inline ExplBox explored_box(const double cx, const double cy, const double margin, const int W, const int H)
+{
+    ExplBox b;
+    const int tw = W >> EXPL_TILE_SHIFT, th = H >> EXPL_TILE_SHIFT;
+    const int x0 = expl_floor_i(cx - margin) >> EXPL_TILE_SHIFT, x1 = expl_ceil_i(cx + margin) >> EXPL_TILE_SHIFT;
+    const int y0 = expl_floor_i(cy - margin) >> EXPL_TILE_SHIFT, y1 = expl_ceil_i(cy + margin) >> EXPL_TILE_SHIFT;
+    b.tx0 = x0;
+    b.ntx = x1 - x0 + 1 < tw ? x1 - x0 + 1 : tw;
+    b.ty0 = y0;
+    b.nty = y1 - y0 + 1 < th ? y1 - y0 + 1 : th;
+    return b;
+}
+
+__host__ __device__ inline bool explored_box_small(const ExplBox b) { return b.ntx <= 3 && b.nty <= 32; }
+
+__host__ __device__ inline bool explored_box_full_small(const uint32_t *bits, const ExplBox b, const int W, const int H)
+{
+    const int tw = W >> EXPL_TILE_SHIFT, th = H >> EXPL_TILE_SHIFT;
+    const uint32_t t_first = (uint32_t)(b.ty0 & (th - 1)), t_last = (uint32_t)((b.ty0 + b.nty - 1) & (th - 1));
+    uint32_t wa[3], wb[3], va[3], vb[3];
+    for (int i = 0; i < 3; ++i) {
+        const uint32_t base = (uint32_t)((b.tx0 + (i < b.ntx ? i : b.ntx - 1)) & (tw - 1)) * (uint32_t)th;
+        wa[i] = explored_tile_word(base + t_first);
+        wb[i] = explored_tile_word(base + t_last);
+    }
+    for (int i = 0; i < 3; ++i) {
+        va[i] = bits[wa[i]];
+        vb[i] = bits[wb[i]];
+    }
+    bool ok = true;
+    for (int i = 0; i < 3; ++i) {
+        const uint32_t base = (uint32_t)((b.tx0 + (i < b.ntx ? i : b.ntx - 1)) & (tw - 1)) * (uint32_t)th;
+        uint32_t ma = 0u, mb = 0u;
+        for (int j = 0; j < b.nty; ++j) {
+            const uint32_t t = base + (uint32_t)((b.ty0 + j) & (th - 1)), m = 1u << explored_tile_bit(t);
+            if (explored_tile_word(t) == wa[i]) ma |= m;
+            else mb |= m;
+        }
+        ok = ok & ((va[i] & ma) == ma) & ((vb[i] & mb) == mb);
+    }
+    return ok;
+}
+
+__host__ __device__ inline bool explored_box_full(const uint32_t *bits, const ExplBox b, const int W, const int H)
+{
+    const int tw = W >> EXPL_TILE_SHIFT, th = H >> EXPL_TILE_SHIFT;
+    bool ok = true;
+    for (int i = 0; i < b.ntx; ++i) {
+        const uint32_t base = (uint32_t)((b.tx0 + i) & (tw - 1)) * (uint32_t)th;
+        int ty = b.ty0 & (th - 1), n = b.nty;
+        while (n > 0) {
+            const uint32_t t = base + (uint32_t)ty, pos = explored_tile_bit(t);
+            int take = n;
+            if (take > 32 - (int)pos) take = 32 - (int)pos;
+            if (take > th - ty) take = th - ty;
+            const uint32_t m = (take >= 32 ? ~0u : (1u << take) - 1u) << pos;
+            const bool full = (bits[explored_tile_word(t)] & m) == m;
+            ok = ok & full;
+            ty = (ty + take) & (th - 1);
+            n -= take;
+        }
+    }
+    return ok;
+}
diff --git a/antsrl_amd/csrc/antsrl_perceive.hip b/antsrl_amd/csrc/antsrl_perceive.hip
--- a/antsrl_amd/csrc/antsrl_perceive.hip
+++ b/antsrl_amd/csrc/antsrl_perceive.hip
@@ -1,6 +1,7 @@
 #include "antsrl_util.h"
 #include "antsrl_flush.h"
 #include "antsrl_update_one.h"
+#include "antsrl_explored.h"
 #include <type_traits>
 
 #define PRC_UNROLL 2
@@ -321,6 +322,7 @@
     static_assert(!POLICY || OBS16, "the in-loop policy reads bfloat16 rows");
     static_assert(!PAD || (HAS_OBS && !POLICY), "padded rows: an observation tensor, no in-loop policy image");
     static_assert(!FAST || ILV, "the fast path reads interleaved records");
+    constexpr bool SKIP = FAST && LAYOUT == PLAYOUT_DEFAULT_ROCKS && !POLICY;
     extern __shared__ __align__(16) unsigned char smem[];
     constexpr int C = 2;
     const int tid = threadIdx.x;
@@ -378,6 +380,7 @@
     const float pre_hold = p.s.holding[a_pre];
     const float pre_seed = (agent_state || POLICY) ? p.s.seed[a_pre] : 0.0f;
     uint32_t rm_lane = 0u;
+    bool skip_lane = false;
     {
         const uint32_t wsel = (blockIdx.x >> 3) + (blockIdx.x >> 8);
         const int w_pro = (POLICY && nwaves > 1) ? 1 + (int)(wsel % (nwaves > 1 ? nwaves - 1 : 1)) : (int)(wsel % nwaves);
@@ -434,10 +437,17 @@
                     if (border || dx * dx + dy * dy < rr * rr) rm |= 1u << q;
                 }
             }
-            if constexpr (FAST) rm_lane = rm;
-            else if (R > 0) rmask[lane] = rm;
-        }
-    }
+            if constexpr (FAST) {
+                rm_lane = rm;
+                if (SKIP && (flags & ACT_SUMMARY)) {
+                    const uint32_t *sum = p.s.explored_bits + (size_t)e * p.words;
+                    const ExplBox bx = explored_box(frames[lane].cx, frames[lane].cy, explored_box_margin(p.r, p.delta), W, H);
+                    skip_lane = explored_box_small(bx) ? explored_box_full_small(sum, bx, W, H) : explored_box_full(sum, bx, W, H);
+                }
+            } else if (R > 0) rmask[lane] = rm;
+        }
+    }
+    const unsigned long long skip_ants = SKIP ? __ballot(skip_lane) : 0ull;
     const bool wave_rocks = FAST && LAYOUT == PLAYOUT_DEFAULT_ROCKS && __ballot(rm_lane != 0u) != 0ull;
     (void)wave_rocks;
     wave_lds_sync();
@@ -469,6 +479,9 @@
     const bool own = mask_q || explore;
     const unsigned long long need_mask = __ballot(own);
     const int src_lane = own ? lane : (need_mask ? __builtin_ctzll(need_mask) : 0);
+    const unsigned long long unmasked = __ballot(mask_q);
+    const int donor = __builtin_amdgcn_readfirstlane(unmasked ? __builtin_ctzll(unmasked) : 0);
+    (void)donor;
 
     const bool tiled = FAST || p.tiled != 0, ftile = !FAST && p.ftile != 0;
 #define PRC_SLOT(ix, iy) (tiled ? tiled_slot((ix), (iy), H) : ftile ? tiled44_slot((ix), (iy), H) : (uint32_t)((ix) * H + (iy)))
@@ -496,7 +509,12 @@
         }                                                                                                \
         _Pragma("unroll") for (int u = 0; u < PRC_UNROLL; ++u)                                           \
         {                                                                                                \
-            const uint32_t gc_ = (PERM) ? (uint32_t)__shfl((int)GRP.cell[u], src_lane) : GRP.cell[u]; \
+            uint32_t gc_ = (PERM) ? (uint32_t)__shfl((int)GRP.cell[u], src_lane) : GRP.cell[u];       \
+            if (SKIP && !(PERM)) {  \
+                const int j_ = min((G0) + u, n_run - 1);                                                 \
+                const uint32_t dc_ = (uint32_t)__builtin_amdgcn_readlane((int)GRP.cell[u], donor);       \
+                gc_ = (((skip_ants >> j_) & 1ull) && !mask_q) ? dc_ : gc_;                               \
+            }                                                                                            \
             if (ILV) {      \
                 const stream_f4 t = PRC_LOAD4(ph + (size_t)gc_ * 4);                                     \
                 GRP.pv[u][0] = t.x; GRP.pv[u][1] = t.y; GRP.fd[u] = t.z; GRP.mt[u] = __float_as_uint(t.w); \
@@ -539,7 +557,8 @@
             const int j = min(j0 + u, n_run - 1);
             const bool real = (j0 + u < n_run) && lane < PP;
             const uint32_t mt = g.mt[u];
-            const bool unexp = real && explore && (mt >> META_STAMP_SHIFT) >= seq;
+            const bool skipping = SKIP && !mask_q && ((skip_ants >> j) & 1ull) != 0ull;
+            const bool unexp = real && explore && !skipping && (mt >> META_STAMP_SHIFT) >= seq;
             const uint32_t n_un = (uint32_t)__popcll(__ballot(unexp));
             cntv = (lane == j0 + u) ? n_un : cntv;
             if (unexp)
@@ -743,6 +762,52 @@
     }
 }
 
+__global__ void __launch_bounds__(256) k_explored_summary(const KP p)
+{
+    const int lane = threadIdx.x & 63;
+    const int th = p.H >> EXPL_TILE_SHIFT, th_sh = __builtin_ctz((unsigned)th);
+    const uint32_t nt = explored_tile_count(p.W, p.H), nw = (nt + 31u) >> 5;
+    const size_t gw = (size_t)blockIdx.x * (blockDim.x >> 6) + (threadIdx.x >> 6);
+    if (gw >= (size_t)p.E * nw) return;
+    const uint32_t e = (uint32_t)(gw / nw), w = (uint32_t)(gw % nw);
+    uint32_t *sum = p.s.explored_bits + (size_t)e * p.words + w;
+    const uint32_t have = *sum;
+    const uint32_t left = nt - 32u * w, valid = left >= 32u ? ~0u : (1u << left) - 1u;
+    uint32_t todo = valid & ~have;
+    if (!todo) return;
+    const uint32_t *meta = reinterpret_cast<const uint32_t *>(p.s.food) + (size_t)e * p.W * p.H * p.fs + 1;
+    const size_t FS = (size_t)p.fs;
+    {
+        uint32_t m = META_NEVER << META_STAMP_SHIFT;
+        if (lane < 32 && ((todo >> lane) & 1u)) {
+            const uint32_t t = 32u * w + (uint32_t)lane;
+            const int x = (int)(t >> th_sh) * 8 + 3, y = (int)(t & (uint32_t)(th - 1)) * 8 + 3;
+            m = meta[(size_t)frec_xy(p, x, y) * FS];
+        }
+        todo &= (uint32_t)__ballot((m >> META_STAMP_SHIFT) != META_NEVER);
+    }
+    uint32_t add = 0u;
+    while (todo) {
+        uint32_t b[4], m[4];
+#pragma unroll
+        for (int k = 0; k < 4; ++k) {
+            b[k] = (uint32_t)__builtin_ctz(todo);
+            const uint32_t rest = todo & (todo - 1u);
+            todo = (rest || k == 3) ? rest : todo;
+        }
+#pragma unroll
+        for (int k = 0; k < 4; ++k) {
+            const uint32_t t = 32u * w + b[k];
+            const int x = (int)(t >> th_sh) * 8 + (lane >> 3), y = (int)(t & (uint32_t)(th - 1)) * 8 + (lane & 7);
+            m[k] = meta[(size_t)frec_xy(p, x, y) * FS];
+        }
+#pragma unroll
+        for (int k = 0; k < 4; ++k)
+            if (__ballot((m[k] >> META_STAMP_SHIFT) == META_NEVER) == 0ull) add |= 1u << b[k];
+    }
+    if (add && lane == 0) *sum = have | add;
+}
+
 static int prc_layout(const KP &p)
 {
     static const int def[7] = {ANTSRL_CH_ANTS, ANTSRL_CH_PHERO, ANTSRL_CH_PHERO, ANTSRL_CH_ANTHILL,
@@ -881,6 +946,22 @@
     return hipErrorInvalidValue;
 }
 
+bool antsrl_explored_summary_supported(const KP &p, bool with_policy)
+{
+    if (with_policy || prc_layout(p) != PLAYOUT_DEFAULT_ROCKS) return false;
+    if (!p.meta || !antsrl_perceive_fast(p) || !p.explore_on || !explored_tiles_ok(p.W, p.H)) return false;
+    for (int q = 0; q < p.PP; ++q)
+        if (!p.mask[q]) return true;
+    return false;
+}
+
+hipError_t antsrl_launch_explored_summary(const KP &p, hipStream_t st)
+{
+    const size_t waves = (size_t)p.E * ((explored_tile_count(p.W, p.H) + 31u) >> 5);
+    hipLaunchKernelGGL(k_explored_summary, dim3((unsigned)((waves + 3) / 4)), dim3(256), 0, st, p);
+    return hipGetLastError();
+}
+
 hipError_t antsrl_launch_meta_rebase(const KP &p, hipStream_t st)
 {
     hipLaunchKernelGGL(k_meta_rebase, dim3(grid_for((size_t)p.E * p.W * p.H)), dim3(256), 0, st, p);
diff --git a/include/antsrl.h b/include/antsrl.h
--- a/include/antsrl.h
+++ b/include/antsrl.h
@@ -199,6 +199,7 @@
     ANTSRL_Q_TIMESTEP = 5,
     ANTSRL_Q_DEFERRED_UPDATE = 6,
     ANTSRL_Q_PERCEIVE_FAST = 7,
+    ANTSRL_Q_EXPLORED_SUMMARY = 8,
     ANTSRL_Q_COUNT_
 };
 int antsrl_query(const AntsHandle *h, int what, long long *value);
@@ -219,7 +220,10 @@
 
 #define ANTSRL_PERCEIVE_AUTO 0
 #define ANTSRL_PERCEIVE_GENERIC 1
+#define ANTSRL_PERCEIVE_FAST_NOSKIP 2
 int antsrl_set_perceive_path(AntsHandle *h, int path);
+
+int antsrl_refresh_explored_summary(AntsHandle *h, void *stream);
 
 int antsrl_set_activation(AntsHandle *h, const float *act, double new_deposit_strength,
                           void *stream);
diff --git a/profiles/r08/skip_ab.py b/profiles/r08/skip_ab.py
--- /dev/null
+++ b/profiles/r08/skip_ab.py
@@ -0,0 +1,73 @@
+#!/usr/bin/env python3
+import argparse
+import os
+import sys
+
+sys.path.insert(0, os.path.dirname(os.path.dirname(os.path.dirname(os.path.abspath(__file__)))))
+
+SHAPES = {"c3": dict(E=1024, N=512, W=256, H=256, R=8), "c2": dict(E=256, N=256, W=256, H=256, R=0)}
+
+
+def main():
+    ap = argparse.ArgumentParser()
+    ap.add_argument("--config", default="c3", choices=sorted(SHAPES))
+    ap.add_argument("--rounds", type=int, default=5)
+    ap.add_argument("--age", type=int, default=400)
+    ap.add_argument("--warmup", type=int, default=20)
+    ap.add_argument("--steps", type=int, default=200)
+    ap.add_argument("--refresh-cost", action="store_true")
+    args = ap.parse_args()
+    import torch
+    from antsrl_amd import config as cm
+    from antsrl_amd.batched import BatchedAntsEnv
+    from antsrl_amd.synth import synth_init
+    s = SHAPES[args.config]
+    dev = torch.device("cuda:0")
+    cfg = cm.make_cfg(s["E"], s["N"], s["W"], s["H"], n_rocks=s["R"], deposit_strength=256.0, max_time=1 << 30)
+    env = BatchedAntsEnv(cfg, dev)
+    env.tune_placement()
+    init = synth_init(cfg, seed=1234)
+    g = torch.Generator(device=dev)
+    g.manual_seed(99)
+    rot = torch.randint(-1, 2, (8, s["E"], s["N"]), generator=g, device=dev, dtype=torch.int8)
+    ph = torch.randint(0, 3, (8, s["E"], s["N"]), generator=g, device=dev, dtype=torch.int8)
+    e0, e1 = torch.cuda.Event(enable_timing=True), torch.cuda.Event(enable_timing=True)
+
+    def episode(path, age):
+        env.set_perceive_path(path)
+        env.reset(init)
+        for t in range(age):
+            env.step_update(rot[t % 8], ph[t % 8], None)
+
+    def timed(n, t0):
+        e0.record()
+        for t in range(t0, t0 + n):
+            env.step_update(rot[t % 8], ph[t % 8], None)
+        e1.record()
+        e1.synchronize()
+        return e0.elapsed_time(e1) / n
+
+    names = {cm.PERCEIVE_AUTO: "auto  ", cm.PERCEIVE_FAST_NOSKIP: "noskip"}
+    for r in range(args.rounds):
+        order = (cm.PERCEIVE_FAST_NOSKIP, cm.PERCEIVE_AUTO) if r % 2 == 0 else (cm.PERCEIVE_AUTO, cm.PERCEIVE_FAST_NOSKIP)
+        for path in order:
+            episode(path, args.age + args.warmup)
+            print("%s r%d %s %.5f" % (args.config, r + 1, names[path], timed(args.steps, args.age + args.warmup)), flush=True)
+    if args.refresh_cost:
+        for age in sorted({64, args.age}):
+            episode(cm.PERCEIVE_AUTO, age - 1)
+            torch.cuda.synchronize()
+            e0.record()
+            env.refresh_explored_summary()
+            e1.record()
+            e1.synchronize()
+            first = e0.elapsed_time(e1)
+            e0.record()
+            env.refresh_explored_summary()
+            e1.record()
+            e1.synchronize()
+            print("%s refresh at age %d: %.4f ms, again right behind it: %.4f ms" % (args.config, age - 1, first, e0.elapsed_time(e1)), flush=True)
+
+
+if __name__ == "__main__":
+    main()
```

Measured after the change: 2.830 billion, median of 6. 1.03x the previous value.
